# Frojdholm/rayrs

Measured on AMD Instinct MI355X. Metric: Mray/s (primary+secondary) on 1M-tri scene @1024spp, higher is better.
Workload: dtype f64

## Files before the change

### rayrs_amd/_ffi.py

```python
import ctypes as C
import os

_HERE = os.path.dirname(os.path.abspath(__file__))
LIB_PATH = os.environ.get("RAYRS_HIP_LIB") or os.path.join(_HERE, "librayrs_hip.so")

SYMBOLS = [
    "rayrs_strerror", "rayrs_last_error",
    "rayrs_objects_create", "rayrs_objects_destroy", "rayrs_objects_len",
    "rayrs_object_sphere", "rayrs_object_plane", "rayrs_object_triangle",
    "rayrs_object_from_triangles_f32", "rayrs_object_from_triangles_f64",
    "rayrs_object_from_spheres", "rayrs_object_box_geom",
    "rayrs_scene_new", "rayrs_scene_destroy", "rayrs_scene_info", "rayrs_scene_export_bvh",
    "rayrs_scene_export_wide", "rayrs_scene_export_gate_tree", "rayrs_scene_export_hot_tree", "rayrs_scene_clone_to_device", "rayrs_scene_device", "rayrs_scene_set_tuning",
    "rayrs_camera_new",
    "rayrs_frame_sample_chunk", "rayrs_render", "rayrs_render_launch", "rayrs_render_finish", "rayrs_render_multi",
    "rayrs_film_create", "rayrs_film_destroy", "rayrs_film_render", "rayrs_film_read", "rayrs_film_status_get",
    "rayrs_film_state_bytes", "rayrs_film_state_get", "rayrs_film_state_set",
    "rayrs_film_render_adaptive", "rayrs_film_tile_samples",
    "rayrs_render_features", "rayrs_film_features", "rayrs_film_denoise", "rayrs_image_denoise",
    "rayrs_film_noise", "rayrs_film_denoise_guided", "rayrs_image_denoise_guided",
    "rayrs_abi_layout", "rayrs_abi_version",
    "rayrs_io_last_error", "rayrs_buffer_free", "rayrs_ply_load", "rayrs_ply_save", "rayrs_obj_load", "rayrs_obj_load_spheres",
    "rayrs_hdr_load", "rayrs_hdr_save", "rayrs_image_to_bytes", "rayrs_ppm_save", "rayrs_png_save",
]


PRIVATE_SYMBOLS = ["rayrs_test_math", "rayrs_test_rng", "rayrs_test_intersect", "rayrs_test_trace", "rayrs_test_path_trace", "rayrs_test_material", "rayrs_test_background",
                   "rayrs_lab_set", "rayrs_lab_round_ms", "rayrs_lab_multi_rehearse"]


class MaterialDesc(C.Structure):
    _fields_ = [("kind", C.c_int32), ("metallic", C.c_int32), ("color", C.c_double * 3),
                ("spec_color", C.c_double * 3), ("alpha", C.c_double), ("ior", C.c_double),
                ("r0", C.c_double * 3)]


class EmissionDesc(C.Structure):
    _fields_ = [("emissive", C.c_int32), ("pad", C.c_int32), ("strength", C.c_double),
                ("color", C.c_double * 3)]


class CameraDesc(C.Structure):
    _fields_ = [("origin", C.c_double * 3), ("e_x", C.c_double * 3), ("e_y", C.c_double * 3),
                ("z", C.c_double * 3), ("width", C.c_double), ("height", C.c_double),
                ("ppc", C.c_uint32), ("x_pixels", C.c_uint32), ("y_pixels", C.c_uint32)]


class SceneInfo(C.Structure):
    _fields_ = [("n_objects", C.c_uint64), ("n_interior", C.c_uint32), ("n_prims", C.c_uint32),
                ("root_ref", C.c_uint32), ("depth", C.c_uint32), ("compact", C.c_uint32),
                ("n_surfaces", C.c_uint32), ("node_bytes", C.c_uint32), ("prim_bytes", C.c_uint32),
                ("device_bytes", C.c_uint64), ("root_box", C.c_double * 6),
                ("build_seconds", C.c_double), ("n_wide", C.c_uint32), ("wide_root_ref", C.c_uint32),
                ("wide_depth", C.c_uint32), ("local_pool", C.c_uint32), ("gate_n_wide", C.c_uint32),
                ("gate_root_ref", C.c_uint32), ("gate_depth", C.c_uint32),
                ("hot_n_wide", C.c_uint32), ("hot_root_ref", C.c_uint32), ("hot_depth", C.c_uint32),
                ("hot_first", C.c_uint32), ("hot_count", C.c_uint32), ("hot_pad", C.c_uint32),
                ("hot_box", C.c_double * 6)]


class RenderParams(C.Structure):
    _fields_ = [("spp", C.c_uint32), ("max_bounces", C.c_uint32), ("seed", C.c_uint64),
                ("sample_chunk", C.c_uint32), ("tile_rank", C.c_uint32), ("tile_ranks", C.c_uint32),
                ("out_format", C.c_uint32), ("count_work", C.c_uint32), ("fast_traversal", C.c_uint32)]


class RenderStats(C.Structure):
    _fields_ = [("rays", C.c_uint64), ("paths", C.c_uint64), ("nan_pixels", C.c_uint64),
                ("neg_pixels", C.c_uint64), ("interior_visits", C.c_uint64), ("tri_tests", C.c_uint64),
                ("sphere_tests", C.c_uint64), ("plane_tests", C.c_uint64), ("escaped_paths", C.c_uint64),
                ("step_wave", C.c_uint64), ("step_lane", C.c_uint64), ("inner_wave", C.c_uint64),
                ("leaf_wave", C.c_uint64), ("interior_ticks", C.c_uint64), ("leaf_ticks", C.c_uint64),
                ("kernel_ms", C.c_double), ("total_ms", C.c_double), ("kernel_launches", C.c_uint64),
                ("trace_ms", C.c_double), ("refill_ticks", C.c_uint64),
                ("surface_hits", C.c_uint64 * 8), ("direct_rays", C.c_uint64), ("hit_ms", C.c_double), ("miss_ms", C.c_double),
                ("local_pool", C.c_uint32), ("exact_walk", C.c_uint32), ("hot_group", C.c_uint32),
                ("stats_pad", C.c_uint32), ("pre_rays", C.c_uint64), ("pre_root_records", C.c_uint64), ("hot_lane", C.c_uint64),
                ("hot_prim_tests", C.c_uint64), ("hot_tri_divided", C.c_uint64)]

    def as_dict(self):
        d = {n: getattr(self, n) for n, _ in self._fields_}
        d["surface_hits"] = list(self.surface_hits)
        return d


class Tuning(C.Structure):
    _fields_ = [("pool_slots", C.c_uint32), ("local_pool", C.c_uint32)]


class FilmParams(C.Structure):
    _fields_ = [("sample_chunk", C.c_uint32), ("max_bounces", C.c_uint32), ("seed", C.c_uint64),
                ("tile_rank", C.c_uint32), ("tile_ranks", C.c_uint32), ("fast_traversal", C.c_uint32), ("pad", C.c_uint32)]


class FilmStatus(C.Structure):
    _fields_ = [("samples", C.c_uint64), ("full_chunks", C.c_uint64), ("rays", C.c_uint64), ("paths", C.c_uint64),
                ("nan_pixels", C.c_uint64), ("neg_pixels", C.c_uint64), ("unconverged", C.c_uint64),
                ("nonfinite", C.c_uint64), ("closed", C.c_uint32), ("pad", C.c_uint32)]

    def as_dict(self):
        return {n: getattr(self, n) for n, _ in self._fields_ if n != "pad"}


class LabTuning(C.Structure):
    _fields_ = [("refill_min", C.c_uint32), ("leaf_min", C.c_uint32), ("static_pct", C.c_uint32),
                ("stack_lds", C.c_uint32), ("hot_records", C.c_uint32), ("trav_blocks_per_cu", C.c_uint32),
                ("eager_light", C.c_uint32), ("local_reserve", C.c_uint32), ("local_segment_items", C.c_uint32),
                ("force_rccl", C.c_uint32), ("gate_tree", C.c_uint32), ("hot_group", C.c_uint32), ("leaf_wait", C.c_uint32), ("flat_blocks_per_cu", C.c_uint32)]


ABI_VERSION = 7

ABI_STRUCTS = [MaterialDesc, EmissionDesc, CameraDesc, SceneInfo, RenderParams, RenderStats, Tuning, FilmParams, FilmStatus]

_lib = None


def lib():
    global _lib
    if _lib is not None:
        return _lib
    if not os.path.exists(LIB_PATH):
        raise RuntimeError(
            f"{LIB_PATH} is missing: build it with `python -c 'import __graft_entry__ as g; g.build()'` "
            "(make -C rayrs_amd/csrc). There is no CPU fallback.")
    L = C.CDLL(LIB_PATH)
    L.rayrs_abi_version.argtypes = []
    L.rayrs_abi_version.restype = C.c_uint32
    if L.rayrs_abi_version() != ABI_VERSION:
        raise RuntimeError(f"{LIB_PATH} has RAYRS_ABI_VERSION {L.rayrs_abi_version()}, this binding was written against "
                           f"{ABI_VERSION}: rebuild the library (make -C rayrs_amd/csrc)")
    dp = C.POINTER(C.c_double)
    vp = C.c_void_p
    L.rayrs_strerror.restype = C.c_char_p
    L.rayrs_strerror.argtypes = [C.c_int]
    L.rayrs_last_error.restype = C.c_char_p
    L.rayrs_objects_create.argtypes = [C.POINTER(vp)]
    L.rayrs_objects_destroy.argtypes = [vp]
    L.rayrs_objects_destroy.restype = None
    L.rayrs_objects_len.argtypes = [vp]
    L.rayrs_objects_len.restype = C.c_uint64
    mp, ep = C.POINTER(MaterialDesc), C.POINTER(EmissionDesc)
    L.rayrs_object_sphere.argtypes = [vp, C.c_double, dp, mp, ep]
    L.rayrs_object_plane.argtypes = [vp, C.c_int] + [C.c_double] * 5 + [mp, ep]
    L.rayrs_object_triangle.argtypes = [vp, dp, dp, dp, mp, ep]
    L.rayrs_object_from_triangles_f32.argtypes = [vp, vp, C.c_uint32, vp, C.c_uint32, mp, ep]
    L.rayrs_object_from_triangles_f64.argtypes = [vp, vp, C.c_uint32, vp, C.c_uint32, mp, ep]
    L.rayrs_object_from_spheres.argtypes = [vp, C.c_double, vp, C.c_uint32, mp, ep]
    L.rayrs_object_box_geom.argtypes = [vp, dp, dp, mp, ep]
    L.rayrs_scene_new.argtypes = [vp, C.c_double, C.c_double, C.c_int, C.c_uint32, C.c_uint32, C.c_uint32, vp,
                                  C.c_int, C.POINTER(vp)]
    L.rayrs_scene_destroy.argtypes = [vp]
    L.rayrs_scene_destroy.restype = None
    L.rayrs_scene_info.argtypes = [vp, C.POINTER(SceneInfo)]
    L.rayrs_scene_export_bvh.argtypes = [vp, vp, vp, vp]
    L.rayrs_scene_export_wide.argtypes = [vp, vp, vp]
    L.rayrs_scene_export_gate_tree.argtypes = [vp, vp, vp]
    L.rayrs_scene_export_hot_tree.argtypes = [vp, vp, vp]
    L.rayrs_scene_clone_to_device.argtypes = [vp, C.c_int, C.POINTER(vp)]
    L.rayrs_scene_device.argtypes = [vp]
    L.rayrs_scene_set_tuning.argtypes = [vp, C.POINTER(Tuning)]
    L.rayrs_lab_set.argtypes = [vp, C.POINTER(LabTuning)]
    L.rayrs_lab_set.restype = C.c_int
    L.rayrs_lab_multi_rehearse.argtypes = [vp, C.c_uint32, C.c_uint32, C.c_int, C.c_char_p, C.c_uint32]
    L.rayrs_lab_multi_rehearse.restype = C.c_int
    L.rayrs_frame_sample_chunk.argtypes = [C.c_uint32] * 4
    L.rayrs_frame_sample_chunk.restype = C.c_uint32
    L.rayrs_abi_layout.argtypes = [vp, C.c_uint32]
    L.rayrs_abi_layout.restype = C.c_uint32
    L.rayrs_abi_version.argtypes = []
    L.rayrs_abi_version.restype = C.c_uint32
    L.rayrs_render_multi.argtypes = [C.POINTER(vp), C.c_uint32, C.POINTER(CameraDesc), C.POINTER(RenderParams), vp,
                                     C.POINTER(RenderStats)]
    L.rayrs_camera_new.argtypes = [dp, dp, dp, C.c_double, C.c_double, C.c_double, C.c_uint32,
                                   C.POINTER(CameraDesc)]
    L.rayrs_render.argtypes = [vp, C.POINTER(CameraDesc), C.POINTER(RenderParams), vp, C.POINTER(RenderStats)]
    L.rayrs_render_launch.argtypes = [vp, C.POINTER(CameraDesc), C.POINTER(RenderParams), vp, vp]
    L.rayrs_render_finish.argtypes = [vp, C.POINTER(RenderStats)]
    L.rayrs_film_create.argtypes = [vp, C.POINTER(CameraDesc), C.POINTER(FilmParams), C.POINTER(vp)]
    L.rayrs_film_destroy.argtypes = [vp]
    L.rayrs_film_destroy.restype = None
    L.rayrs_film_render.argtypes = [vp, C.c_uint32, C.POINTER(RenderStats)]
    L.rayrs_film_read.argtypes = [vp, C.c_uint32, vp]
    L.rayrs_film_status_get.argtypes = [vp, C.c_double, C.POINTER(FilmStatus)]
    L.rayrs_film_state_bytes.argtypes = [vp]
    L.rayrs_film_state_bytes.restype = C.c_uint64
    L.rayrs_film_state_get.argtypes = [vp, vp, C.c_uint64]
    L.rayrs_film_state_set.argtypes = [vp, vp, C.c_uint64]
    L.rayrs_film_render_adaptive.argtypes = [vp, C.c_uint32, C.c_double, C.c_uint32, C.POINTER(C.c_uint64), C.POINTER(RenderStats)]
    L.rayrs_film_tile_samples.argtypes = [vp, vp, C.c_uint64]
    L.rayrs_film_tile_samples.restype = C.c_uint64
    for name, args in (("rayrs_render_features", [vp, C.POINTER(CameraDesc), C.c_uint32, C.c_uint64, C.c_uint32, C.c_uint32, C.c_uint32,
                                                  vp, vp, vp, vp, vp]),
                       ("rayrs_film_features", [vp, C.c_uint32, vp, vp, vp, vp, vp]),
                       ("rayrs_film_denoise", [vp, C.c_uint32, C.c_uint32] + [C.c_double] * 4 + [C.c_uint32, vp]),
                       ("rayrs_image_denoise", [C.c_int, C.c_uint32, C.c_uint32, vp, vp, vp, vp, C.c_uint32] + [C.c_double] * 4 + [vp]),
                       ("rayrs_film_noise", [vp, vp]),
                       ("rayrs_film_denoise_guided", [vp, C.c_uint32, C.c_uint32] + [C.c_double] * 4 + [C.c_uint32, vp, vp]),
                       ("rayrs_image_denoise_guided", [C.c_int, C.c_uint32, C.c_uint32, vp, vp, vp, vp, vp, C.c_uint32] + [C.c_double] * 4
                        + [vp, vp])):
        if hasattr(L, name) or "RAYRS_HIP_LIB" not in os.environ:
            getattr(L, name).argtypes = args
    L.rayrs_test_math.argtypes = [C.c_int, C.c_int, vp, vp, C.c_uint64, vp]
    L.rayrs_test_rng.argtypes = [C.c_int, C.c_uint64, vp, vp, vp, C.c_uint64, vp]
    L.rayrs_test_intersect.argtypes = [vp, vp, vp, C.c_uint64, C.c_int, vp, vp]
    L.rayrs_test_trace.argtypes = [vp, vp, vp, C.c_uint64, C.c_int, vp, vp, vp]
    L.rayrs_test_path_trace.argtypes = [vp, C.POINTER(CameraDesc), C.c_uint64, C.c_uint32, vp, vp, C.c_uint64, C.c_int, C.c_uint32,
                                        vp, vp, vp, vp, vp, vp]
    L.rayrs_test_material.argtypes = [C.c_int, mp, vp, vp, vp, C.c_uint64, vp, vp, vp, vp]
    L.rayrs_test_background.argtypes = [vp, vp, C.c_uint64, vp]
    L.rayrs_io_last_error.restype = C.c_char_p
    L.rayrs_buffer_free.argtypes = [vp]
    L.rayrs_buffer_free.restype = None
    u32p = C.POINTER(C.c_uint32)
    L.rayrs_ply_load.argtypes = [C.c_char_p, C.POINTER(vp), u32p, C.POINTER(vp), u32p]
    L.rayrs_ply_save.argtypes = [C.c_char_p, vp, C.c_uint32, vp, C.c_uint32, C.c_int]
    L.rayrs_obj_load.argtypes = [C.c_char_p, C.POINTER(vp), u32p, C.POINTER(vp), u32p]
    L.rayrs_obj_load_spheres.argtypes = [C.c_char_p, C.POINTER(vp), u32p]
    L.rayrs_hdr_load.argtypes = [C.c_char_p, C.POINTER(vp), u32p, u32p]
    L.rayrs_hdr_save.argtypes = [C.c_char_p, vp, C.c_uint32, C.c_uint32]
    L.rayrs_image_to_bytes.argtypes = [vp, C.c_uint32, C.c_uint32, C.c_double, vp, C.POINTER(C.c_uint64)]
    L.rayrs_ppm_save.argtypes = [C.c_char_p, vp, C.c_uint32, C.c_uint32]
    L.rayrs_png_save.argtypes = [C.c_char_p, vp, C.c_uint32, C.c_uint32]
    for name in SYMBOLS:
        if not hasattr(L, name) and "RAYRS_HIP_LIB" in os.environ:
            continue
        fn = getattr(L, name)
        if fn.restype is C.c_int and name not in ("rayrs_strerror",):
            fn.restype = C.c_int
    _lib = L
    return L


class RayrsError(RuntimeError):
    def __init__(self, status, where):
        L = lib()
        msg = L.rayrs_strerror(status).decode()
        extra = L.rayrs_last_error().decode() if status != -6 else L.rayrs_io_last_error().decode()
        super().__init__(f"{where}: {msg} ({status})" + (f" [{extra}]" if extra else ""))
        self.status = status


def check(status, where):
    if status != 0:
        raise RayrsError(status, where)
```

### rayrs_amd/api.py

```python
import ctypes as C
from dataclasses import dataclass, field
from typing import List, Optional, Sequence, Tuple

import numpy as np

from . import _ffi

Vec = Tuple[float, float, float]


class Axis:
    X, XRev, Y, YRev, Z, ZRev = range(6)


class BvhHeuristic:
    Midpoint = ("midpoint", 0)

    @staticmethod
    def Sah(splits: int):
        return ("sah", int(splits))


MAT_LAMBERTIAN, MAT_REFLECT, MAT_REFRACT, MAT_GLASS, MAT_COOK_TORRANCE, MAT_COOK_TORRANCE_REFRACT, \
    MAT_COOK_TORRANCE_GLASS, MAT_PLASTIC, MAT_NO_REFLECT = range(9)
# ... 191 lines not shown
        return int(self.desc.x_pixels)

    def y_pixels(self) -> int:
        return int(self.desc.y_pixels)


class Scene:

    def __init__(self, objects, z_near, z_far, heuristic, hdri, device: int = 0):
        L = _ffi.lib()
        self._L = L
        self._h = None
        objs = C.c_void_p()
        _ffi.check(L.rayrs_objects_create(C.byref(objs)), "rayrs_objects_create")
        try:
            for o in flatten_objects(objects):
                m, e = o.mat.desc(), o.emission.desc()
                if o.kind == "sphere":
                    st = L.rayrs_object_sphere(objs, o.radius, _d3(o.origin), C.byref(m), C.byref(e))
                elif o.kind == "plane":
                    st = L.rayrs_object_plane(objs, o.axis, o.umin, o.umax, o.vmin, o.vmax, o.pos, C.byref(m),
                                              C.byref(e))
                elif o.kind == "triangle":
                    st = L.rayrs_object_triangle(objs, _d3(o.p[0]), _d3(o.p[1]), _d3(o.p[2]), C.byref(m),
                                                 C.byref(e))
                elif o.kind == "mesh":
                    fn = (L.rayrs_object_from_triangles_f32 if o.verts.dtype == np.float32
                          else L.rayrs_object_from_triangles_f64)
                    st = fn(objs, o.verts.ctypes.data, o.verts.shape[0], o.idx.ctypes.data, o.idx.shape[0],
                            C.byref(m), C.byref(e))
                else:
                    raise ValueError(f"unknown object kind {o.kind}")
                if st == -1:
                    raise ValueError(f"Object::{o.kind}: invalid argument (a reference assert! would fire)")
                _ffi.check(st, f"rayrs_object_{o.kind}")
            hdri = np.ascontiguousarray(hdri, dtype=np.float32)
            if hdri.ndim != 3 or hdri.shape[2] != 3:
                raise ValueError("hdri must be (H, W, 3)")
            kind, splits = heuristic
            h = C.c_void_p()
            st = L.rayrs_scene_new(objs, float(z_near), float(z_far), 1 if kind == "sah" else 0, int(splits),
                                   hdri.shape[1], hdri.shape[0], hdri.ctypes.data, int(device), C.byref(h))
            if st == -1:
                raise ValueError("Scene::new: invalid argument (lib.rs:234-235, bvh.rs:229)")
            _ffi.check(st, "rayrs_scene_new")
            self._h = h
            self.device = int(device)
        finally:
            L.rayrs_objects_destroy(objs)

    @classmethod
    def _from_handle(cls, L, h, device):
        self = cls.__new__(cls)
        self._L, self._h, self.device = L, h, int(device)
        return self

    def clone_to_device(self, device: int) -> "Scene":
        h = C.c_void_p()
        _ffi.check(self._L.rayrs_scene_clone_to_device(self._h, int(device), C.byref(h)), "rayrs_scene_clone_to_device")
        return Scene._from_handle(self._L, h, device)

    def set_tuning(self, **kw):
        t = _ffi.Tuning()
        for k, v in kw.items():
            if k not in dict(_ffi.Tuning._fields_):
                raise ValueError(f"unknown tuning field {k}")
            setattr(t, k, int(v))
        _ffi.check(self._L.rayrs_scene_set_tuning(self._h, C.byref(t)), "rayrs_scene_set_tuning")

    def lab_set(self, **kw):
        t = _ffi.LabTuning()
        for k, v in kw.items():
            if k not in dict(_ffi.LabTuning._fields_):
                raise ValueError(f"unknown lab field {k}")
            setattr(t, k, int(v))
        _ffi.check(self._L.rayrs_lab_set(self._h, C.byref(t)), "rayrs_lab_set")

    def info(self) -> dict:
        i = _ffi.SceneInfo()
        _ffi.check(self._L.rayrs_scene_info(self._h, C.byref(i)), "rayrs_scene_info")
        d = {n: getattr(i, n) for n, _ in i._fields_ if n not in ("root_box", "hot_box")}
        d["root_box"] = list(i.root_box)
        d["hot_box"] = list(i.hot_box)
        return d

    def export_bvh(self):
        i = self.info()
        box = np.zeros((max(i["n_interior"], 1), 2, 6), dtype=np.float64)
        ref = np.zeros((max(i["n_interior"], 1), 2), dtype=np.uint32)
        prim = np.zeros(max(i["n_prims"], 1), dtype=np.uint32)
        _ffi.check(self._L.rayrs_scene_export_bvh(self._h, box.ctypes.data, ref.ctypes.data, prim.ctypes.data),
                   "rayrs_scene_export_bvh")
        return box[:i["n_interior"]], ref[:i["n_interior"]], prim[:i["n_prims"]]

    def export_wide(self):
        i = self.info()
        box = np.zeros((max(i["n_wide"], 1), 4, 6), dtype=np.float64)
        ref = np.zeros((max(i["n_wide"], 1), 4), dtype=np.uint32)
        _ffi.check(self._L.rayrs_scene_export_wide(self._h, box.ctypes.data, ref.ctypes.data),
                   "rayrs_scene_export_wide")
        return box[:i["n_wide"]], ref[:i["n_wide"]]

    def export_gate_tree(self):
        i = self.info()
        box = np.zeros((max(i["gate_n_wide"], 1), 4, 6), dtype=np.float64)
        ref = np.zeros((max(i["gate_n_wide"], 1), 4), dtype=np.uint32)
        _ffi.check(self._L.rayrs_scene_export_gate_tree(self._h, box.ctypes.data, ref.ctypes.data),
                   "rayrs_scene_export_gate_tree")
        return box[:i["gate_n_wide"]], ref[:i["gate_n_wide"]]

    def export_hot_tree(self):
        i = self.info()
        box = np.zeros((max(i["hot_n_wide"], 1), 4, 6), dtype=np.float64)
        ref = np.zeros((max(i["hot_n_wide"], 1), 4), dtype=np.uint32)
        _ffi.check(self._L.rayrs_scene_export_hot_tree(self._h, box.ctypes.data, ref.ctypes.data),
                   "rayrs_scene_export_hot_tree")
        return box[:i["hot_n_wide"]], ref[:i["hot_n_wide"]]

    def close(self):
        if self._h is not None:
            self._L.rayrs_scene_destroy(self._h)
            self._h = None

    def __del__(self):
        try:
            self.close()
        except Exception:
            pass


def frame_sample_chunk(width: int, height: int, spp: int, requested: int = 4) -> int:
    return int(_ffi.lib().rayrs_frame_sample_chunk(int(width), int(height), int(spp), int(requested)))


def make_params(spp, max_bounces=50, seed=0x5EED, sample_chunk=0, tile_rank=0, tile_ranks=1, out_f64=False,
                count_work=False, exact_traversal=True, fast_traversal=None) -> _ffi.RenderParams:
    p = _ffi.RenderParams()
    p.spp, p.max_bounces, p.seed = int(spp), int(max_bounces), int(seed)
    p.sample_chunk, p.tile_rank, p.tile_ranks = int(sample_chunk), int(tile_rank), int(tile_ranks)
    p.out_format = 1 if out_f64 else 0
    p.count_work = 1 if count_work else 0
    fast = (not exact_traversal) if fast_traversal is None else bool(fast_traversal)
    p.fast_traversal = 1 if fast else 0
    return p


def render(scene: Scene, camera: Camera, spp: int, max_bounces: int = 50, seed: int = 0x5EED, sample_chunk: int = 0,
           tile_rank: int = 0, tile_ranks: int = 1, out_f64: bool = False, count_work: bool = False, out=None,
           exact_traversal: bool = True, fast_traversal=None):
    L = scene._L
    H, W = camera.y_pixels(), camera.x_pixels()
    dt = np.float64 if out_f64 else np.float32
    if out is None:
        out = np.zeros((H, W, 3), dtype=dt)
    assert out.shape == (H, W, 3) and out.dtype == dt and out.flags.c_contiguous
    p = make_params(spp, max_bounces, seed, sample_chunk, tile_rank, tile_ranks, out_f64, count_work, exact_traversal,
                    fast_traversal)
    st = _ffi.RenderStats()
    _ffi.check(L.rayrs_render(scene._h, C.byref(camera.desc), C.byref(p), out.ctypes.data, C.byref(st)),
               "rayrs_render")
    return out, st.as_dict()


def render_multi(scene_list, camera: Camera, spp: int, max_bounces: int = 50, seed: int = 0x5EED,
                 sample_chunk: int = 0, out_f64: bool = False):
    L = scene_list[0]._L
    H, W = camera.y_pixels(), camera.x_pixels()
# ... 268 lines not shown
```

### rayrs_amd/csrc/abi.cpp

```cpp
#include <hip/hip_runtime.h>

#include <cmath>
#include <cstddef>
#include <cstdlib>
#include <cstring>
#include <memory>
#include <new>
#include <stdexcept>
#include <string>
#include <vector>

#include "../../include/rayrs_hip.h"
#include "film.h"
#include "kernels.h"
#include "local_pool.h"
#include "rayrs_lab.h"
#include "scene_host.hpp"
#include "scene_internal.hpp"
#include "wavefront.h"

using namespace rayrs;

namespace {
thread_local std::string g_last_error;
// ... 103 lines not shown
    RAYRS_GUARDED({
    if (!objs) return RAYRS_INVALID_ARG;
    if (!(umin < umax && vmin < vmax)) return RAYRS_INVALID_ARG;
    if (axis < 0 || axis > 5) return RAYRS_INVALID_ARG;
    const int surf = objs->list.add_surface(mat, emission);
    if (surf < 0) return surf;
    Object o;
    std::memset(&o, 0, sizeof(o));
    o.geom.kind = PRIM_PLANE;
    o.geom.axis = (uint32_t)axis;
    o.geom.u0 = umin, o.geom.u1 = umax, o.geom.v0 = vmin, o.geom.v1 = vmax, o.geom.pos = pos;
    o.surface = (uint32_t)surf;
    objs->list.objs.push_back(o);
    return RAYRS_OK;
    })
}

int rayrs_object_triangle(rayrs_objects* objs, const double p1[3], const double p2[3], const double p3[3],
                          const rayrs_material* mat, const rayrs_emission* emission) {
    RAYRS_GUARDED({
    if (!objs || !p1 || !p2 || !p3) return RAYRS_INVALID_ARG;
    const int surf = objs->list.add_surface(mat, emission);
    if (surf < 0) return surf;
    push_triangle(objs->list, {p1[0], p1[1], p1[2]}, {p2[0], p2[1], p2[2]}, {p3[0], p3[1], p3[2]}, (uint32_t)surf);
    return RAYRS_OK;
    })
}

int rayrs_object_from_triangles_f32(rayrs_objects* objs, const float* verts, uint32_t nverts, const uint32_t* idx,
                                    uint32_t ntris, const rayrs_material* mat, const rayrs_emission* emission) {
    RAYRS_GUARDED({
    return from_triangles<float>(objs, verts, nverts, idx, ntris, mat, emission);
    })
}

int rayrs_object_from_triangles_f64(rayrs_objects* objs, const double* verts, uint32_t nverts, const uint32_t* idx,
                                    uint32_t ntris, const rayrs_material* mat, const rayrs_emission* emission) {
    RAYRS_GUARDED({
    return from_triangles<double>(objs, verts, nverts, idx, ntris, mat, emission);
    })
}

int rayrs_object_from_spheres(rayrs_objects* objs, double radius, const double* centers, uint32_t n,
                              const rayrs_material* mat, const rayrs_emission* emission) {
    if (!objs || (!centers && n)) return RAYRS_INVALID_ARG;
    for (uint32_t i = 0; i < n; i++) RAYRS_TRY(rayrs_object_sphere(objs, radius, centers + 3 * (size_t)i, mat, emission));
    return RAYRS_OK;
}

int rayrs_object_box_geom(rayrs_objects* objs, const double ll[3], const double ur[3], const rayrs_material* mat,
                          const rayrs_emission* emission) {
    if (!objs || !ll || !ur) return RAYRS_INVALID_ARG;
    const struct {
        int axis;
        double u0, u1, v0, v1, pos;
    } faces[6] = {
        {RAYRS_AXIS_X, ll[1], ur[1], ll[2], ur[2], ll[0]},    {RAYRS_AXIS_XREV, ll[1], ur[1], ll[2], ur[2], ur[0]},
        {RAYRS_AXIS_ZREV, ll[0], ur[0], ll[1], ur[1], ll[2]}, {RAYRS_AXIS_Z, ll[0], ur[0], ll[1], ur[1], ur[2]},
        {RAYRS_AXIS_YREV, ll[0], ur[0], ll[2], ur[2], ll[1]}, {RAYRS_AXIS_Y, ll[0], ur[0], ll[2], ur[2], ll[1]},
    };
    for (const auto& f : faces) RAYRS_TRY(rayrs_object_plane(objs, f.axis, f.u0, f.u1, f.v0, f.v1, f.pos, mat, emission));
    return RAYRS_OK;
}


void rayrs_scene_destroy(rayrs_scene* scene) { delete scene; }

static int scene_configure_traversal(rayrs_scene* s) {
    const FlatScene& f = s->flat;
    for (int x = 0; x < 3; x++) {
        if (x == 2 && !f.has_hot) continue;
        const WalkTree& t = s->tree(x);
        rayrs_scene::Walk& w = s->trav[x];
        const uint32_t depth = t.depth ? t.depth : 1;
        w.leafq = x == 0 ? 0u : TRAV_LEAFQ;
        uint32_t want = s->lab.stack_lds ? s->lab.stack_lds : (w.leafq ? TRAV_STACK_LDS_DEFER : TRAV_STACK_LDS);
        w.stack_lds = want < depth ? want : depth;
        const uint32_t rec_bytes = f.compact ? (uint32_t)sizeof(Node4F32) + 16u : (uint32_t)sizeof(Node4F64) + 16u;
        uint32_t hot = (w.leafq ? TRAV_HOT_BYTES_DEFER : TRAV_HOT_BYTES) / rec_bytes;
        if (s->lab.hot_records == 0xffffffffu) hot = 0;
        else if (s->lab.hot_records) hot = s->lab.hot_records < WIDE_FRONT ? s->lab.hot_records : WIDE_FRONT;
        w.hot_records = hot < t.n() ? hot : t.n();
        const uint32_t lds = wf_trav_lds_bytes(f.compact, w.stack_lds, w.leafq, w.hot_records);
        HIP_TRY(wf_trav_raise_lds(f.compact, lds));
        HIP_TRY(wf_trav_occupancy(f.compact, lds, &w.blocks_per_cu));
        if (w.blocks_per_cu < 1) w.blocks_per_cu = 1;
    }
    return RAYRS_OK;
}

constexpr uint32_t LOCAL_SEGMENT_ITEMS = 1u << 27;
constexpr uint32_t LOCAL_MAX_SEGMENTS = 64;
static void scene_configure_local(rayrs_scene* s) {
    const FlatScene& f = s->flat;
    LocalScene& ls = s->local;
    std::memset(&ls, 0, sizeof(ls));
    s->local_ok = false;
    const WalkTree& t = f.gate;
    if (t.n() > 1 || f.n_prims() == 0 || f.n_prims() > LP_MAX_PRIMS || s->surfaces.size() > LP_MAX_PRIMS) return;
    auto add_gate = [&](const double* box, uint32_t ref) {
        if ((ref >> 30) != REF_RANGE) return false;
        const uint32_t g = ls.n_gates++;
        for (int i = 0; i < 6; i++) ls.box[g][i] = box[i];
        ls.first[g] = (ref & 0x3fffffffu) >> 2;
        ls.count[g] = (ref & 3u) + 1u;
        return true;
    };
    if (t.n() == 0) {
        if (!add_gate(f.root_box, t.root_ref)) return;
    } else {
        if ((t.root_ref >> 30) != REF_INTERIOR) return;
        for (uint32_t k = 0; k < 4; k++) {
            const uint32_t ref = t.ref[k];
            if ((ref >> 30) == REF_NONE) continue;
            if (!add_gate(&t.box[(size_t)k * 6], ref)) return;
        }
    }
    uint32_t covered = 0;
    for (uint32_t g = 0; g < ls.n_gates; g++) covered += ls.count[g];
    if (covered != f.n_prims()) return;
    ls.n_records = t.n();
    ls.n_prims = f.n_prims();
    for (const SurfaceDev& sf : s->surfaces) ls.kind_mask |= 1u << (uint32_t)sf.kind;
    s->local_ok = true;
}

extern "C++" int rayrs::scene_upload(rayrs_scene* s) {
    HIP_TRY(hipSetDevice(s->device));
    hipDeviceProp_t prop;
    HIP_TRY(hipGetDeviceProperties(&prop, s->device));
    s->cu_count = prop.multiProcessorCount;
    const FlatScene& f = s->flat;
    for (int x = 0; x < 3; x++) {
        const WalkTree& t = s->tree(x);
        if (x == 2 && !f.has_hot) continue;
        HIP_TRY(s->trav[x].d_nodes.upload(t.node_bytes.data(), t.node_bytes.size()));
    }
    if (f.has_hot) HIP_TRY(s->d_hot.upload(&f.hot, sizeof(HotGroupDev)));
    HIP_TRY(s->d_prims.upload(f.prim_bytes.data(), f.prim_bytes.size()));
    HIP_TRY(s->d_surfaces.upload(s->surfaces.data(), s->surfaces.size() * sizeof(SurfaceDev)));
    HIP_TRY(s->d_hdri.upload(f.hdri_quads.data(), f.hdri_quads.size() * sizeof(float)));
    HIP_TRY(s->d_counters.reserve(sizeof(Counters)));
    for (auto& e : s->ev) HIP_TRY(e.create());
    s->device_bytes = f.walk.node_bytes.size() + f.gate.node_bytes.size() + (f.has_hot ? f.gate_hot.node_bytes.size() : 0) + f.prim_bytes.size() + s->surfaces.size() * sizeof(SurfaceDev) +
                      f.hdri_quads.size() * sizeof(float);
    RAYRS_TRY(scene_configure_traversal(s));
    HIP_TRY(s->pool.d_ctl.reserve(sizeof(WfCtl)));
    HIP_TRY(s->pool.h_live.alloc(2 * sizeof(uint32_t)));
    for (auto& e : s->pool.ev_batch) HIP_TRY(e.create());
    HIP_TRY(s->d_next_item.reserve(sizeof(unsigned long long)));
    if (s->local_ok) {
        HIP_TRY(lp_configure());
        HIP_TRY(lp_occupancy(s->flat.compact, s->local.n_prims, (uint32_t)s->surfaces.size(), &s->local_blocks_per_cu));
        if (s->local_blocks_per_cu < 1) s->local_blocks_per_cu = 1;
        if (s->local_blocks_per_cu > (int)LP_WPS) s->local_blocks_per_cu = (int)LP_WPS;
        HIP_TRY(s->d_local_items.reserve(LOCAL_MAX_SEGMENTS * sizeof(unsigned long long)));
    }
    return RAYRS_OK;
}

int rayrs_scene_new(const rayrs_objects* objs, double z_near, double z_far, int heuristic, uint32_t splits,
                    uint32_t hdri_w, uint32_t hdri_h, const float* hdri_rgb, int device, rayrs_scene** out) {
    RAYRS_GUARDED({
    if (!objs || !out) return RAYRS_INVALID_ARG;
    *out = nullptr;
    std::unique_ptr<rayrs_scene> s(new rayrs_scene());
    RAYRS_TRY(build_flat_scene(objs->list, z_near, z_far, heuristic, splits, hdri_w, hdri_h, hdri_rgb, &s->flat));
    if (std::max(s->flat.walk.depth, s->flat.gate.depth) > 4096u) {
        g_last_error = "walk tree needs " + std::to_string(std::max(s->flat.walk.depth, s->flat.gate.depth)) + " stack entries (limit 4096)";
        return RAYRS_UNSUPPORTED;
    }
    s->surfaces = objs->list.surfaces;
    s->n_objects = objs->list.objs.size();
    s->device = device;
    scene_configure_local(s.get());
    if (device >= 0) RAYRS_TRY(scene_upload(s.get()));
    *out = s.release();
    return RAYRS_OK;
    })
}

int rayrs_scene_info(const rayrs_scene* scene, rayrs_scene_info_t* info) {
    if (!scene || !info) return RAYRS_INVALID_ARG;
    const FlatScene& f = scene->flat;
    std::memset(info, 0, sizeof(*info));
    info->n_objects = scene->n_objects;
    info->n_interior = f.n_interior();
    info->n_prims = f.n_prims();
    info->root_ref = f.root_ref;
    info->depth = f.depth;
    info->compact = f.compact ? 1u : 0u;
    info->n_surfaces = (uint32_t)scene->surfaces.size();
    info->node_bytes = f.compact ? (uint32_t)sizeof(Node4F32) : (uint32_t)sizeof(Node4F64);
    info->n_wide = f.walk.n();
    info->wide_root_ref = f.walk.root_ref;
    info->wide_depth = f.walk.depth;
    info->gate_n_wide = f.gate.n();
    info->gate_root_ref = f.gate.root_ref;
    info->gate_depth = f.gate.depth;
    if (f.has_hot) {
        info->hot_n_wide = f.gate_hot.n();
        info->hot_root_ref = f.gate_hot.root_ref;
        info->hot_depth = f.gate_hot.depth;
        info->hot_first = f.hot.first;
        info->hot_count = f.hot.count;
        for (int i = 0; i < 6; i++) info->hot_box[i] = f.hot.box[i];
    }
    info->local_pool = (scene->local_ok && scene->tuning.local_pool != 1u) ? 1u : 0u;
    info->prim_bytes = 4u * (f.compact ? PRIM_DWORDS_COMPACT : PRIM_DWORDS_FULL);
    info->device_bytes = scene->device_bytes;
    for (int i = 0; i < 6; i++) info->root_box[i] = f.root_box[i];
    info->build_seconds = f.build_seconds;
    return RAYRS_OK;
}

int rayrs_scene_export_bvh(const rayrs_scene* scene, double* child_box, uint32_t* child_ref, uint32_t* prim_object) {
    if (!scene) return RAYRS_INVALID_ARG;
    const FlatScene& f = scene->flat;
    if (child_box && !f.child_box.empty()) std::memcpy(child_box, f.child_box.data(), f.child_box.size() * 8);
    if (child_ref && !f.child_ref.empty()) std::memcpy(child_ref, f.child_ref.data(), f.child_ref.size() * 4);
    if (prim_object && !f.prim_object.empty())
        std::memcpy(prim_object, f.prim_object.data(), f.prim_object.size() * 4);
    return RAYRS_OK;
}

static int export_tree(const WalkTree& t, double* wide_box, uint32_t* wide_ref) {
    if (wide_box && !t.box.empty()) std::memcpy(wide_box, t.box.data(), t.box.size() * 8);
    if (wide_ref && !t.ref.empty()) std::memcpy(wide_ref, t.ref.data(), t.ref.size() * 4);
// ... 12 lines not shown
    return scene && scene->flat.has_hot ? export_tree(scene->flat.gate_hot, wide_box, wide_ref) : RAYRS_INVALID_ARG;
}

int rayrs_scene_clone_to_device(const rayrs_scene* scene, int device, rayrs_scene** out) {
    RAYRS_GUARDED({
        if (!scene || !out || device < 0) return RAYRS_INVALID_ARG;
        *out = nullptr;
        std::unique_ptr<rayrs_scene> s(new rayrs_scene());
        s->flat = scene->flat;
        s->surfaces = scene->surfaces;
        s->n_objects = scene->n_objects;
        s->tuning = scene->tuning;
        s->lab = scene->lab;
        s->device = device;
        scene_configure_local(s.get());
        RAYRS_TRY(scene_upload(s.get()));
        *out = s.release();
        return RAYRS_OK;
    })
}

int rayrs_scene_device(const rayrs_scene* scene) { return scene ? scene->device : -1; }

static int scene_quiesce(rayrs_scene* scene) {
    return scene->device >= 0 ? scene_settle(scene) : RAYRS_OK;
}

rayrs_scene::~rayrs_scene() {
    if (device < 0) return;
    (void)hipSetDevice(device);
    if (pending && last_stream) (void)hipStreamSynchronize(last_stream);
}

int rayrs_scene_set_tuning(rayrs_scene* scene, const rayrs_tuning* tuning) {
    if (!scene || !tuning) return RAYRS_INVALID_ARG;
    if (tuning->local_pool > 1u) return RAYRS_INVALID_ARG;
    RAYRS_TRY(scene_quiesce(scene));
    scene->tuning = *tuning;
    return RAYRS_OK;
}

#ifdef RAYRS_LAB_TICKS
extern "C" int rayrs_lab_ticks(rayrs_scene* scene, uint64_t out[16]) {
    if (!scene || !out || scene->device < 0) return RAYRS_INVALID_ARG;
    HIP_TRY(hipSetDevice(scene->device));
    Counters c;
    HIP_TRY(scene->d_counters.download(&c, sizeof(c)));
    for (int i = 0; i < 16; i++) out[i] = c.lab_ticks[i];
    return RAYRS_OK;
}
#endif

static int round_event(rayrs_scene::Pool& pl, uint32_t r, uint32_t k, hipStream_t stream) {
    while (pl.ev_round.size() < 4 * (size_t)(r + 1)) {
        Event e;
        HIP_TRY(e.create());
        pl.ev_round.push_back(std::move(e));
    }
    HIP_TRY(hipEventRecord(pl.ev_round[4 * (size_t)r + k], stream));
    return RAYRS_OK;
}

static int round_ms(const rayrs_scene* scene, uint32_t r, float ms[3]) {
    const Event* e = &scene->pool.ev_round[4 * (size_t)r];
    ms[1] = ms[2] = 0.f;
    HIP_TRY(hipEventElapsedTime(&ms[0], e[0], e[1]));
    if (scene->last_local) return RAYRS_OK;
    HIP_TRY(hipEventElapsedTime(&ms[1], e[1], e[2]));
    HIP_TRY(hipEventElapsedTime(&ms[2], e[2], e[3]));
    return RAYRS_OK;
}

extern "C" int rayrs_lab_round_ms(rayrs_scene* scene, float* out, uint32_t cap_rounds) {
    if (!scene || scene->device < 0 || scene->pending) return RAYRS_INVALID_ARG;
    HIP_TRY(hipSetDevice(scene->device));
    for (uint32_t r = 0; r < scene->pool.timed_rounds && r < cap_rounds && out; r++) RAYRS_TRY(round_ms(scene, r, out + 3 * r));
    return (int)scene->pool.timed_rounds;
}

int rayrs_lab_set(rayrs_scene* scene, const rayrs_lab_tuning* lab) {
    if (!scene || !lab) return RAYRS_INVALID_ARG;
    if (lab->stack_lds > 64u) return RAYRS_INVALID_ARG;
    if (lab->hot_group != 0u && lab->hot_group != 0xffffffffu) return RAYRS_INVALID_ARG;
    if (lab->static_pct > 100u || lab->refill_min > 64u || lab->leaf_min > 64u || lab->leaf_wait > 64u || lab->flat_blocks_per_cu > 64u || lab->eager_light > 1u || lab->force_rccl > 1u || lab->gate_tree > 1u)
        return RAYRS_INVALID_ARG;
    if (lab->local_reserve != 0u && (lab->local_reserve < 8u || lab->local_reserve > 4096u)) return RAYRS_INVALID_ARG;
    if (lab->local_segment_items != 0u && lab->local_segment_items < 65536u) return RAYRS_INVALID_ARG;
    RAYRS_TRY(scene_quiesce(scene));
    scene->lab = *lab;
    if (scene->device >= 0) return scene_configure_traversal(scene);
    return RAYRS_OK;
}

uint32_t rayrs_frame_sample_chunk(uint32_t x_pixels, uint32_t y_pixels, uint32_t spp, uint32_t requested) {
    if (spp == 0) return 0;
    uint64_t chunk = requested ? requested : 4u;
    const uint64_t pixels = (uint64_t)((x_pixels + 7u) / 8u) * ((y_pixels + 7u) / 8u) * 64u;
    while (chunk < spp && pixels * ((spp + chunk - 1) / chunk) > (1ull << 30)) chunk *= 2;
    return chunk >= spp ? 0u : (uint32_t)chunk;
}

uint32_t rayrs_abi_version(void) { return RAYRS_ABI_VERSION; }

uint32_t rayrs_abi_layout(uint32_t* out, uint32_t cap) {
    std::vector<uint32_t> t;
    t.push_back(RAYRS_ABI_VERSION);
#define RAYRS_STRUCT(T, N) t.push_back((uint32_t)sizeof(T)), t.push_back(N)
#define RAYRS_FIELD(T, F) t.push_back((uint32_t)offsetof(T, F))
    RAYRS_STRUCT(rayrs_material, 7);
    RAYRS_FIELD(rayrs_material, kind), RAYRS_FIELD(rayrs_material, metallic), RAYRS_FIELD(rayrs_material, color);
    RAYRS_FIELD(rayrs_material, spec_color), RAYRS_FIELD(rayrs_material, alpha), RAYRS_FIELD(rayrs_material, ior);
    RAYRS_FIELD(rayrs_material, r0);
    RAYRS_STRUCT(rayrs_emission, 4);
    RAYRS_FIELD(rayrs_emission, emissive), RAYRS_FIELD(rayrs_emission, pad), RAYRS_FIELD(rayrs_emission, strength);
    RAYRS_FIELD(rayrs_emission, color);
    RAYRS_STRUCT(rayrs_camera, 9);
    RAYRS_FIELD(rayrs_camera, origin), RAYRS_FIELD(rayrs_camera, e_x), RAYRS_FIELD(rayrs_camera, e_y);
    RAYRS_FIELD(rayrs_camera, z), RAYRS_FIELD(rayrs_camera, width), RAYRS_FIELD(rayrs_camera, height);
    RAYRS_FIELD(rayrs_camera, ppc), RAYRS_FIELD(rayrs_camera, x_pixels), RAYRS_FIELD(rayrs_camera, y_pixels);
    RAYRS_STRUCT(rayrs_scene_info_t, 26);
    RAYRS_FIELD(rayrs_scene_info_t, n_objects), RAYRS_FIELD(rayrs_scene_info_t, n_interior);
    RAYRS_FIELD(rayrs_scene_info_t, n_prims), RAYRS_FIELD(rayrs_scene_info_t, root_ref);
    RAYRS_FIELD(rayrs_scene_info_t, depth), RAYRS_FIELD(rayrs_scene_info_t, compact);
    RAYRS_FIELD(rayrs_scene_info_t, n_surfaces), RAYRS_FIELD(rayrs_scene_info_t, node_bytes);
    RAYRS_FIELD(rayrs_scene_info_t, prim_bytes), RAYRS_FIELD(rayrs_scene_info_t, device_bytes);
    RAYRS_FIELD(rayrs_scene_info_t, root_box), RAYRS_FIELD(rayrs_scene_info_t, build_seconds);
    RAYRS_FIELD(rayrs_scene_info_t, n_wide), RAYRS_FIELD(rayrs_scene_info_t, wide_root_ref);
    RAYRS_FIELD(rayrs_scene_info_t, wide_depth), RAYRS_FIELD(rayrs_scene_info_t, local_pool);
    RAYRS_FIELD(rayrs_scene_info_t, gate_n_wide), RAYRS_FIELD(rayrs_scene_info_t, gate_root_ref);
    RAYRS_FIELD(rayrs_scene_info_t, gate_depth);
    RAYRS_FIELD(rayrs_scene_info_t, hot_n_wide), RAYRS_FIELD(rayrs_scene_info_t, hot_root_ref);
    RAYRS_FIELD(rayrs_scene_info_t, hot_depth), RAYRS_FIELD(rayrs_scene_info_t, hot_first);
    RAYRS_FIELD(rayrs_scene_info_t, hot_count), RAYRS_FIELD(rayrs_scene_info_t, hot_pad);
    RAYRS_FIELD(rayrs_scene_info_t, hot_box);
    RAYRS_STRUCT(rayrs_render_params, 9);
    RAYRS_FIELD(rayrs_render_params, spp), RAYRS_FIELD(rayrs_render_params, max_bounces);
    RAYRS_FIELD(rayrs_render_params, seed), RAYRS_FIELD(rayrs_render_params, sample_chunk);
    RAYRS_FIELD(rayrs_render_params, tile_rank), RAYRS_FIELD(rayrs_render_params, tile_ranks);
    RAYRS_FIELD(rayrs_render_params, out_format), RAYRS_FIELD(rayrs_render_params, count_work);
    RAYRS_FIELD(rayrs_render_params, fast_traversal);
    RAYRS_STRUCT(rayrs_render_stats, 33);
    RAYRS_FIELD(rayrs_render_stats, rays), RAYRS_FIELD(rayrs_render_stats, paths);
    RAYRS_FIELD(rayrs_render_stats, nan_pixels), RAYRS_FIELD(rayrs_render_stats, neg_pixels);
    RAYRS_FIELD(rayrs_render_stats, interior_visits), RAYRS_FIELD(rayrs_render_stats, tri_tests);
    RAYRS_FIELD(rayrs_render_stats, sphere_tests), RAYRS_FIELD(rayrs_render_stats, plane_tests);
    RAYRS_FIELD(rayrs_render_stats, escaped_paths), RAYRS_FIELD(rayrs_render_stats, step_wave);
    RAYRS_FIELD(rayrs_render_stats, step_lane), RAYRS_FIELD(rayrs_render_stats, inner_wave);
    RAYRS_FIELD(rayrs_render_stats, leaf_wave), RAYRS_FIELD(rayrs_render_stats, interior_ticks);
    RAYRS_FIELD(rayrs_render_stats, leaf_ticks), RAYRS_FIELD(rayrs_render_stats, kernel_ms);
    RAYRS_FIELD(rayrs_render_stats, total_ms), RAYRS_FIELD(rayrs_render_stats, kernel_launches);
    RAYRS_FIELD(rayrs_render_stats, trace_ms), RAYRS_FIELD(rayrs_render_stats, refill_ticks);
    RAYRS_FIELD(rayrs_render_stats, surface_hits), RAYRS_FIELD(rayrs_render_stats, direct_rays);
    RAYRS_FIELD(rayrs_render_stats, hit_ms), RAYRS_FIELD(rayrs_render_stats, miss_ms);
    RAYRS_FIELD(rayrs_render_stats, local_pool), RAYRS_FIELD(rayrs_render_stats, exact_walk);
    RAYRS_FIELD(rayrs_render_stats, hot_group), RAYRS_FIELD(rayrs_render_stats, stats_pad);
    RAYRS_FIELD(rayrs_render_stats, pre_rays), RAYRS_FIELD(rayrs_render_stats, pre_root_records);
    RAYRS_FIELD(rayrs_render_stats, hot_lane);
    RAYRS_FIELD(rayrs_render_stats, hot_prim_tests), RAYRS_FIELD(rayrs_render_stats, hot_tri_divided);
    RAYRS_STRUCT(rayrs_tuning, 2);
    RAYRS_FIELD(rayrs_tuning, pool_slots), RAYRS_FIELD(rayrs_tuning, local_pool);
    RAYRS_STRUCT(rayrs_film_params, 7);
    RAYRS_FIELD(rayrs_film_params, sample_chunk), RAYRS_FIELD(rayrs_film_params, max_bounces);
    RAYRS_FIELD(rayrs_film_params, seed), RAYRS_FIELD(rayrs_film_params, tile_rank);
    RAYRS_FIELD(rayrs_film_params, tile_ranks), RAYRS_FIELD(rayrs_film_params, fast_traversal);
    RAYRS_FIELD(rayrs_film_params, pad);
    RAYRS_STRUCT(rayrs_film_status, 10);
    RAYRS_FIELD(rayrs_film_status, samples), RAYRS_FIELD(rayrs_film_status, full_chunks);
    RAYRS_FIELD(rayrs_film_status, rays), RAYRS_FIELD(rayrs_film_status, paths);
    RAYRS_FIELD(rayrs_film_status, nan_pixels), RAYRS_FIELD(rayrs_film_status, neg_pixels);
    RAYRS_FIELD(rayrs_film_status, unconverged), RAYRS_FIELD(rayrs_film_status, nonfinite);
    RAYRS_FIELD(rayrs_film_status, closed), RAYRS_FIELD(rayrs_film_status, pad);
#undef RAYRS_STRUCT
#undef RAYRS_FIELD
    for (uint32_t i = 0; i < cap && i < t.size(); i++) out[i] = t[i];
    return (uint32_t)t.size();
}


int rayrs_camera_new(const double origin[3], const double up[3], const double lookat[3], double fov, double width,
                     double height, uint32_t ppi, rayrs_camera* out) {
    return camera_new(origin, up, lookat, fov, width, height, ppi, out);
}


extern "C++" SceneDev rayrs::make_scene_dev(const rayrs_scene* s, bool exact) {
    SceneDev sc;
    std::memset(&sc, 0, sizeof(sc));
    const int which = s->walk_index(exact);
    const WalkTree& t = s->tree(which);
    const rayrs_scene::Walk& w = s->trav[which];
    sc.hot = which == 2 ? s->d_hot.as<HotGroupDev>() : nullptr;
    sc.nodes = w.d_nodes.as<>();
    sc.prims = s->d_prims.as<>();
    sc.surfaces = s->d_surfaces.as<SurfaceDev>();
    sc.hdri = s->d_hdri.as<float>();
    sc.hdri_w = s->flat.hdri_w;
    sc.hdri_h = s->flat.hdri_h;
    sc.hdri_wm1 = (double)(s->flat.hdri_w - 1u);
    sc.hdri_hm1 = (double)(s->flat.hdri_h - 1u);
    sc.root_ref = t.root_ref;
    sc.stack_depth = t.depth ? t.depth : 1;
    sc.stack_lds = w.stack_lds;
    sc.hot_records = w.hot_records;
    sc.leafq = w.leafq;
    sc.n_surfaces = (uint32_t)s->surfaces.size();
    for (int i = 0; i < 6; i++) sc.root_box[i] = s->flat.root_box[i];
    sc.t0 = s->flat.t0;
    sc.t1 = s->flat.t1;
    sc.exact = exact ? 1u : 0u;
    return sc;
}

constexpr double RAYRS_FAR_DIAGONALS = 8.0;
constexpr double RAYRS_FAR_PRIMITIVES = 4096.0;
extern "C++" bool rayrs::camera_is_far(const rayrs_scene* s, const rayrs_camera* c) {
    const double* b = s->flat.root_box;
    double d2 = 0.0, e2 = 0.0;
    for (int a = 0; a < 3; a++) {
        const double lo = b[2 * a], hi = b[2 * a + 1], o = c->origin[a];
        const double out = o < lo ? lo - o : (o > hi ? o - hi : 0.0);
        d2 += out * out;
        e2 += (hi - lo) * (hi - lo);
    }
    const double small = s->flat.small_extent;
    return d2 > RAYRS_FAR_DIAGONALS * RAYRS_FAR_DIAGONALS * e2 || (small > 0.0 && d2 > RAYRS_FAR_PRIMITIVES * RAYRS_FAR_PRIMITIVES * small * small);
}

extern "C++" CameraDev rayrs::make_camera_dev(const rayrs_camera* c) {
    CameraDev cam;
    std::memset(&cam, 0, sizeof(cam));
    for (int i = 0; i < 3; i++) {
        cam.origin[i] = c->origin[i];
        cam.e_x[i] = c->e_x[i];
        cam.e_y[i] = c->e_y[i];
        cam.z[i] = c->z[i];
    }
    cam.width = c->width;
    cam.height = c->height;
    cam.ppc = (double)c->ppc;
    cam.W = c->x_pixels;
    cam.H = c->y_pixels;
    return cam;
}

extern "C++" uint32_t rayrs::trav_settings(const rayrs_scene* s, bool exact, uint32_t np, RenderDev& rp) {
    const rayrs_lab_tuning& lab = s->lab;
    rp.refill_min = lab.refill_min ? lab.refill_min : 52u;
    rp.leaf_min = lab.leaf_min ? lab.leaf_min : (exact ? 48u : lab.gate_tree ? 32u : 24u);
    rp.leaf_wait = lab.leaf_wait ? lab.leaf_wait : 16u;
    uint32_t trav_bpc = (uint32_t)s->trav[s->walk_index(exact)].blocks_per_cu;
    if (lab.trav_blocks_per_cu && lab.trav_blocks_per_cu < trav_bpc) trav_bpc = lab.trav_blocks_per_cu;
    const uint32_t blocks = (uint32_t)s->cu_count * trav_bpc;
    const uint32_t static_pct = lab.static_pct ? lab.static_pct : 50u;
    const uint64_t n_waves = (uint64_t)blocks * 4u;
    rp.static_windows = (uint32_t)((uint64_t)(np / wf_window_slots()) * static_pct / 100u / n_waves * n_waves);
    return blocks;
}

extern "C++" WfDev rayrs::pool_wf(const DevBuf& block, uint32_t np, const DevBuf& ctl, uint32_t trav_blocks, const DevBuf& spill) {
    WfDev wf;
    std::memset(&wf, 0, sizeof(wf));
    wf.slots = block.as<PathSlot>();
    wf.light = reinterpret_cast<double*>(wf.slots + np);
    wf.state = reinterpret_cast<uint8_t*>(wf.light + (size_t)np * 4u);
    wf.ctl = ctl.as<WfCtl>();
    wf.np = np;
    wf.trav_threads = trav_blocks * 256u;
    wf.stack_spill = spill.as<uint32_t>();
    return wf;
}

struct FramePlan {
    SceneDev sc;
    CameraDev cam;
    RenderDev rp;
    bool exact, eager_light, use_local;
    uint64_t partial_need;
    uint64_t tile_items, seg_tiles, seg_items;
    uint32_t local_blocks;
    uint64_t live_total;
    uint32_t np, trav_blocks, flat_blocks;
    size_t spill_words;
    bool is_film;
    FilmPassDev film;
};

static RenderDev make_render_dev(const rayrs_scene* scene, const rayrs_camera* camera, const rayrs_render_params* params, uint32_t sample0,
                                 const FilmPassDev* film, void* out_device) {
    RenderDev rp;
    std::memset(&rp, 0, sizeof(rp));
    rp.spp = params->spp;
    rp.sample0 = sample0;
    rp.max_bounces = params->max_bounces;
    rp.seed = params->seed;
    rp.chunk = (params->sample_chunk == 0 || params->sample_chunk >= params->spp) ? params->spp : params->sample_chunk;
// ... 36 lines not shown
    p.local_blocks = (uint32_t)scene->cu_count * (uint32_t)scene->local_blocks_per_cu;
    const uint64_t most_items = rp.total_items < p.seg_items ? rp.total_items : p.seg_items;
    const uint64_t want_blocks = (most_items + 4u * LP_PATHS_PER_WAVE - 1) / (4u * LP_PATHS_PER_WAVE);
    if (want_blocks < p.local_blocks) p.local_blocks = (uint32_t)(want_blocks ? want_blocks : 1);
    if (!p.use_local || rp.total_items == 0) p.local_blocks = 0;

    p.exact = params->fast_traversal == 0u || camera_is_far(scene, camera);
    p.sc = make_scene_dev(scene, p.exact);
    p.cam = make_camera_dev(camera);

    constexpr uint64_t POOL_MAX_SLOTS = 1ull << 28;
    uint64_t np64 = rp.total_items;
    if (np64 > POOL_MAX_SLOTS) np64 = POOL_MAX_SLOTS;
    {
        const uint64_t samples = rp.n_local_tiles * 64ull * rp.spp;
        const uint64_t by_work = samples / 12u > (1ull << 20) ? samples / 12u : (1ull << 20);
        if (np64 > by_work) np64 = by_work;
    }
    if (scene->tuning.pool_slots) np64 = scene->tuning.pool_slots;
    if (np64 > rp.total_items) np64 = rp.total_items;
    p.live_total = np64;
    const bool streaming = !p.use_local && rp.total_items > 0;
    p.np = streaming ? (uint32_t)((p.live_total + 1023ull) & ~1023ull) : 0u;
    p.trav_blocks = trav_settings(scene, p.exact, p.np, rp);
    p.spill_words = streaming ? (size_t)(p.sc.stack_depth - p.sc.stack_lds) * p.trav_blocks * 256u : 0;

    p.eager_light = lab.eager_light != 0u;
    for (const SurfaceDev& sf : scene->surfaces)
        if (sf.emit[0] != 0.0 || sf.emit[1] != 0.0 || sf.emit[2] != 0.0) p.eager_light = true;

    const uint32_t n_windows = p.np / wf_window_slots();
    p.flat_blocks = (n_windows + 3u) / 4u;
    uint32_t per_cu = lab.flat_blocks_per_cu;
    if (!per_cu) {
        per_cu = n_windows / (36u * (uint32_t)scene->cu_count);
        per_cu = per_cu < FLAT_BLOCKS_PER_CU_MIN ? FLAT_BLOCKS_PER_CU_MIN : per_cu > FLAT_BLOCKS_PER_CU_MAX ? FLAT_BLOCKS_PER_CU_MAX : per_cu;
    }
    const uint32_t flat_cap = (uint32_t)scene->cu_count * per_cu;
    if (p.flat_blocks > flat_cap) p.flat_blocks = flat_cap;
    return RAYRS_OK;
}

static int enqueue_local(rayrs_scene* scene, const FramePlan& p, hipStream_t stream) {
    rayrs_scene::Pool& pl = scene->pool;
    const RenderDev& rp = p.rp;
    const uint64_t n_seg = (rp.total_items + p.seg_items - 1) / p.seg_items;
    for (uint64_t seg = 0; seg < n_seg; seg++) {
        LocalDev lp;
        lp.light = scene->d_local_light.as<double>();
        lp.next_item = scene->d_local_items.as<unsigned long long>() + seg;
        lp.item_base = seg * p.seg_items;
        lp.item_count = rp.total_items - lp.item_base < p.seg_items ? rp.total_items - lp.item_base : p.seg_items;
        RenderDev rseg = rp;
        rseg.partial_item0 = lp.item_base;
        const uint64_t share = lp.item_count / ((uint64_t)p.local_blocks * 4u * 16u);
        lp.reserve = (uint32_t)(share < 8u ? 8u : share > 256u ? 256u : share);
        if (scene->lab.local_reserve) lp.reserve = scene->lab.local_reserve;
        lp.pad = 0;
        RAYRS_TRY(round_event(pl, (uint32_t)seg, 0, stream));
        HIP_TRY(lp_launch(scene->flat.compact, rp.count_work != 0u, p.sc, scene->local, p.cam, rseg, lp, p.local_blocks, stream));
        RAYRS_TRY(round_event(pl, (uint32_t)seg, 1, stream));
        const uint32_t seg_lt0 = (uint32_t)(seg * p.seg_tiles), seg_n_lt = (uint32_t)(lp.item_count / p.tile_items);
        HIP_TRY(p.is_film ? launch_film_accumulate(p.cam, rseg, p.film, seg_lt0, seg_n_lt, stream) : launch_resolve(p.cam, rseg, seg_lt0, seg_n_lt, stream));
        pl.timed_rounds = (uint32_t)seg + 1;
    }
    scene->rounds = (uint32_t)n_seg;
    return RAYRS_OK;
}

static int enqueue_streaming(rayrs_scene* scene, const FramePlan& p, const WfDev& wf, hipStream_t stream) {
    rayrs_scene::Pool& pl = scene->pool;
    const RenderDev& rp = p.rp;
    uint32_t* h_live = pl.h_live.as<uint32_t>();
    HIP_TRY(wf_launch_init(wf, (uint32_t)p.live_total, stream));
    HIP_TRY(wf_launch_gen(scene->flat.compact, p.sc, p.cam, rp, wf, p.flat_blocks, stream));
    h_live[0] = h_live[1] = (uint32_t)p.live_total;
    constexpr uint32_t MAX_TIMED = 8192;
    uint32_t it = 0;
    uint32_t batch = 16;
    for (uint32_t b = 0;; b++) {
        for (uint32_t k = 0; k < batch; k++, it++) {
            const bool timed = it < MAX_TIMED;
            if (timed) RAYRS_TRY(round_event(pl, it, 0, stream));
            HIP_TRY(wf_launch_trav(scene->flat.compact, rp.count_work != 0u, p.sc, rp, wf, p.trav_blocks, stream));
            if (timed) RAYRS_TRY(round_event(pl, it, 1, stream));
            HIP_TRY(wf_launch_hit(scene->flat.compact, p.eager_light, p.sc, p.cam, rp, wf, p.flat_blocks, stream));
            if (timed) RAYRS_TRY(round_event(pl, it, 2, stream));
            HIP_TRY(wf_launch_miss(scene->flat.compact, p.eager_light, p.sc, p.cam, rp, wf, p.flat_blocks, stream));
            if (timed) {
                RAYRS_TRY(round_event(pl, it, 3, stream));
                pl.timed_rounds = it + 1;
            }
        }
        HIP_TRY(hipMemcpyAsync(&h_live[b & 1u], &wf.ctl->live_slots, sizeof(uint32_t), hipMemcpyDeviceToHost, stream));
        HIP_TRY(hipEventRecord(pl.ev_batch[b & 1u], stream));
        if (b > 0) {
            HIP_TRY(hipEventSynchronize(pl.ev_batch[(b - 1u) & 1u]));
            const uint64_t seen = h_live[(b - 1u) & 1u];
            if (seen == 0u) break;
            batch = seen * 8u < p.live_total ? 4u : 16u;
        }
        if (it > (1u << 26)) {
            g_last_error = "path rounds did not terminate";
            return RAYRS_HIP_ERROR;
        }
    }
    scene->rounds = it;
    return RAYRS_OK;
}

extern "C++" int rayrs::render_enqueue(rayrs_scene* scene, const rayrs_camera* camera, const rayrs_render_params* params, uint32_t sample0,
                                       const FilmPassDev* film, void* out_device, void* hip_stream) {
    RAYRS_GUARDED({
    if (!scene || !camera || !params || (!out_device && !film)) return RAYRS_INVALID_ARG;
    if (scene->device < 0) return RAYRS_NO_DEVICE;
    if (params->spp == 0 || camera->x_pixels == 0 || camera->y_pixels == 0) return RAYRS_INVALID_ARG;
    if (camera->x_pixels > 65535u || camera->y_pixels > 65535u) return RAYRS_UNSUPPORTED;
    if (params->max_bounces > 8000u) return RAYRS_UNSUPPORTED;
    if (params->spp > SLOT_SAMPLE_MASK || sample0 > SLOT_SAMPLE_MASK - params->spp) return RAYRS_UNSUPPORTED;
    if (params->tile_ranks == 0 || params->tile_rank >= params->tile_ranks) return RAYRS_INVALID_ARG;
    if (params->out_format != RAYRS_OUT_F32 && params->out_format != RAYRS_OUT_F64) return RAYRS_INVALID_ARG;
    if (params->fast_traversal > 1u) return RAYRS_INVALID_ARG;
    HIP_TRY(hipSetDevice(scene->device));
    hipStream_t stream = reinterpret_cast<hipStream_t>(hip_stream);
    if (scene->pending) {
        HIP_TRY(hipStreamSynchronize(scene->last_stream));
        scene->pending = false;
    }

    FramePlan p;
    RAYRS_TRY(plan_frame(scene, camera, params, sample0, film, out_device, p));
    p.is_film = film != nullptr;
    p.film = film ? *film : FilmPassDev{};
    scene->last_exact = p.exact;

    rayrs_scene::Pool& pl = scene->pool;
    HIP_TRY(scene->d_partial.reserve((size_t)p.partial_need * 3 * sizeof(double)));
    p.rp.partial = scene->d_partial.as<double>();
    HIP_TRY(scene->d_local_light.reserve((size_t)p.local_blocks * 4u * LP_PATHS_PER_WAVE * 4 * sizeof(double)));
    HIP_TRY(pl.block.reserve((size_t)p.np * POOL_SLOT_BYTES));
    HIP_TRY(pl.d_wave_items.reserve((size_t)p.flat_blocks * 4u * 2 * sizeof(unsigned long long)));
    HIP_TRY(pl.d_stack_spill.reserve(p.spill_words * sizeof(uint32_t)));
    WfDev wf = pool_wf(pl.block, p.np, pl.d_ctl, p.trav_blocks, pl.d_stack_spill);
    wf.n_flat_waves = p.flat_blocks * 4u;
    wf.wave_items = pl.d_wave_items.as<unsigned long long>();

    pl.timed_rounds = 0;
    HIP_TRY(hipMemsetAsync(p.rp.counters, 0, sizeof(Counters), stream));
    HIP_TRY(hipMemsetAsync(p.rp.next_item, 0, sizeof(unsigned long long), stream));
    if (p.use_local) HIP_TRY(hipMemsetAsync(scene->d_local_items.as<>(), 0, LOCAL_MAX_SEGMENTS * sizeof(unsigned long long), stream));
    HIP_TRY(hipEventRecord(scene->ev[0], stream));
    scene->rounds = 0;
    scene->last_local = p.use_local;
    if (p.rp.total_items > 0) RAYRS_TRY(p.use_local ? enqueue_local(scene, p, stream) : enqueue_streaming(scene, p, wf, stream));
    HIP_TRY(hipEventRecord(scene->ev[1], stream));
    if (!p.use_local) HIP_TRY(p.is_film ? launch_film_accumulate(p.cam, p.rp, p.film, 0u, p.rp.n_local_tiles, stream) : launch_resolve(p.cam, p.rp, 0u, p.rp.n_local_tiles, stream));
    HIP_TRY(hipEventRecord(scene->ev[2], stream));
    scene->last_stream = stream;
    scene->pending = true;
    return RAYRS_OK;
    })
}

int rayrs_render_launch(rayrs_scene* scene, const rayrs_camera* camera, const rayrs_render_params* params,
                        void* out_device, void* hip_stream) {
    if (!out_device) return RAYRS_INVALID_ARG;
    return render_enqueue(scene, camera, params, 0u, nullptr, out_device, hip_stream);
// ... 71 lines not shown
```

### rayrs_amd/csrc/rayrs_lab.h

```cpp
#ifndef RAYRS_LAB_H
#define RAYRS_LAB_H

#include <stdint.h>

#include "../../include/rayrs_hip.h"

#ifdef __cplusplus
extern "C" {
#endif

typedef struct {
    uint32_t refill_min;
    uint32_t leaf_min;
    uint32_t static_pct;
    uint32_t stack_lds;
    uint32_t hot_records;
    uint32_t trav_blocks_per_cu;
    uint32_t eager_light;
    uint32_t local_reserve;
    uint32_t local_segment_items;
    uint32_t force_rccl;
    uint32_t gate_tree;
    uint32_t hot_group;
    uint32_t leaf_wait;
    uint32_t flat_blocks_per_cu;
} rayrs_lab_tuning;

int rayrs_lab_set(rayrs_scene* scene, const rayrs_lab_tuning* lab);

int rayrs_lab_round_ms(rayrs_scene* scene, float* out, uint32_t cap_rounds);

int rayrs_lab_multi_rehearse(const int* rank_devices, uint32_t n, uint32_t rounds, int fail_reduce_at, char* log, uint32_t cap);

#ifdef __cplusplus
}
#endif
#endif
```

### rayrs_amd/csrc/rayrs_selftest.h

```cpp
#ifndef RAYRS_SELFTEST_H
#define RAYRS_SELFTEST_H

#include <stdint.h>

#include "../../include/rayrs_hip.h"

#ifdef __cplusplus
extern "C" {
#endif

int rayrs_test_math(int device, int fn, const double* x, const double* y, uint64_t n, double* out);
int rayrs_test_rng(int device, uint64_t seed, const uint64_t* pixel, const uint64_t* sample, const uint32_t* draw,
                   uint64_t n, uint64_t* out_bits);
int rayrs_test_intersect(rayrs_scene* scene, const double* o, const double* d, uint64_t n, int exact, double* t,
                         int64_t* object);
int rayrs_test_trace(rayrs_scene* scene, const double* o, const double* d, uint64_t n, int exact, double* t, int64_t* object,
                     uint64_t* pre_answered);
int rayrs_test_path_trace(rayrs_scene* scene, const rayrs_camera* camera, uint64_t seed, uint32_t max_bounces,
                          const uint32_t* pixel, const uint32_t* sample, uint64_t n, int exact, uint32_t cap,
                          uint32_t* n_queries, int64_t* object, double* t, double* throughput, uint32_t* draw, double* rgb);
int rayrs_test_material(int device, const rayrs_material* mat, const double* normal, const double* view,
                        const uint64_t* key, uint64_t n, int32_t* scattered, double* color, double* dir,
                        uint32_t* draws);
int rayrs_test_background(rayrs_scene* scene, const double* dir, uint64_t n, double* rgb);

#ifdef __cplusplus
}
#endif
#endif
```

### rayrs_amd/csrc/scene_host.cpp

```cpp
#include "scene_host.hpp"

#include <algorithm>
#include <chrono>
#include <cmath>
#include <cstddef>
#include <cstdlib>
#include <cstring>
#include <limits>

#include "../../include/rayrs_numeric.h"

namespace rayrs {


static bool in01(const double* c) {
    return c[0] >= 0.0 && c[0] <= 1.0 && c[1] >= 0.0 && c[1] <= 1.0 && c[2] >= 0.0 && c[2] <= 1.0;
}

int ObjectList::add_surface(const rayrs_material* m, const rayrs_emission* e) {
    if (!m) return RAYRS_INVALID_ARG;
    SurfaceDev s;
    std::memset(&s, 0, sizeof(s));
    s.kind = m->kind;
    if (m->kind < 0 || m->kind > RAYRS_MAT_NO_REFLECT) return RAYRS_INVALID_ARG;
    if (m->kind != RAYRS_MAT_NO_REFLECT) {
        if (!in01(m->color)) return RAYRS_INVALID_ARG;
        for (int i = 0; i < 3; i++) s.color[i] = m->color[i];
        const bool needs_ior = m->kind == RAYRS_MAT_REFRACT || m->kind == RAYRS_MAT_GLASS ||
                               m->kind == RAYRS_MAT_COOK_TORRANCE_REFRACT ||
                               m->kind == RAYRS_MAT_COOK_TORRANCE_GLASS || m->kind == RAYRS_MAT_PLASTIC;
        if (needs_ior && !(m->ior > 0.0 && std::isfinite(m->ior))) return RAYRS_INVALID_ARG;
        s.ior = m->ior;
        if (m->kind >= RAYRS_MAT_COOK_TORRANCE && m->kind <= RAYRS_MAT_PLASTIC) {
            if (!(m->alpha > 0.0 && std::isfinite(m->alpha))) return RAYRS_INVALID_ARG;
            s.ct_alpha2 = m->alpha * m->alpha;
            for (int i = 0; i < 3; i++) s.ct_color[i] = m->color[i];
            if (m->kind == RAYRS_MAT_COOK_TORRANCE) {
                s.metallic = m->metallic ? 1 : 0;
                if (s.metallic) {
                    for (int i = 0; i < 3; i++) s.ct_r0[i] = m->r0[i];
                } else {
                    s.ct_ior = m->ior;
                }
            } else {
                s.metallic = 0;
                s.ct_ior = m->ior;
                if (m->kind == RAYRS_MAT_PLASTIC) {
                    if (!in01(m->spec_color)) return RAYRS_INVALID_ARG;
                    for (int i = 0; i < 3; i++) s.ct_color[i] = m->spec_color[i];
                }
            }
        }
    }
    if (e && e->emissive) {
        if (!(e->strength >= 0.0) || !in01(e->color)) return RAYRS_INVALID_ARG;
        s.emissive = 1;
        for (int i = 0; i < 3; i++) s.emit[i] = e->strength * e->color[i];
    }
    for (size_t i = 0; i < surfaces.size(); i++)
        if (std::memcmp(&surfaces[i], &s, sizeof(s)) == 0) return (int)i;
    surfaces.push_back(s);
    return (int)surfaces.size() - 1;
}


Aabb shape_bbox(const Shape& s) {
    Aabb b;
    if (s.kind == PRIM_SPHERE) {
        const double radius = rr_sqrt(s.radius2);
        b.xmin = s.origin.x - radius;
        b.xmax = s.origin.x + radius;
        b.ymin = s.origin.y - radius;
        b.ymax = s.origin.y + radius;
        b.zmin = s.origin.z - radius;
        b.zmax = s.origin.z + radius;
    } else if (s.kind == PRIM_PLANE) {
        if (s.axis == RAYRS_AXIS_X || s.axis == RAYRS_AXIS_XREV) {
            b = {s.pos, s.pos, s.u0, s.u1, s.v0, s.v1};
        } else if (s.axis == RAYRS_AXIS_Y || s.axis == RAYRS_AXIS_YREV) {
            b = {s.u0, s.u1, s.pos, s.pos, s.v0, s.v1};
        } else {
            b = {s.u0, s.u1, s.v0, s.v1, s.pos, s.pos};
        }
    } else {
        b.xmin = rr_min(s.p1.x, rr_min(s.p2.x, s.p3.x));
        b.ymin = rr_min(s.p1.y, rr_min(s.p2.y, s.p3.y));
        b.zmin = rr_min(s.p1.z, rr_min(s.p2.z, s.p3.z));
        b.xmax = rr_max(s.p1.x, rr_max(s.p2.x, s.p3.x));
        b.ymax = rr_max(s.p1.y, rr_max(s.p2.y, s.p3.y));
        b.zmax = rr_max(s.p1.z, rr_max(s.p2.z, s.p3.z));
    }
    return b;
}
// ... 436 lines not shown
void tight_box(const Aabb& b, const double* gate, double* out) {
    const double pb[6] = {b.xmin, b.xmax, b.ymin, b.ymax, b.zmin, b.zmax};
    double ext = 0.0;
    for (int a = 0; a < 3; a++) ext = std::max(ext, pb[2 * a + 1] - pb[2 * a]);
    const double m = ext * LEAF_MARGIN;
    for (int a = 0; a < 3; a++) {
        double lo = pb[2 * a] - m, hi = pb[2 * a + 1] + m;
        float lf = (float)lo, hf = (float)hi;
        if ((double)lf > lo) lf = std::nextafterf(lf, -std::numeric_limits<float>::infinity());
        if ((double)hf < hi) hf = std::nextafterf(hf, std::numeric_limits<float>::infinity());
        lo = (double)lf, hi = (double)hf;
        out[2 * a] = lo > gate[2 * a] ? lo : gate[2 * a];
        out[2 * a + 1] = hi < gate[2 * a + 1] ? hi : gate[2 * a + 1];
    }
}

void split_groups(const std::vector<WalkGroup>& groups, const std::vector<Aabb>& prim_box, std::vector<WalkGroup>& out) {
    out.reserve(groups.size() * 3);
    for (const WalkGroup& g : groups) {
        const uint32_t first = (g.ref & 0x3fffffffu) >> 2, count = (g.ref & 3u) + 1u;
        for (uint32_t i = 0; i < count; i++) {
            WalkGroup r;
            tight_box(prim_box[first + i], g.box, r.box);
            r.ref = (REF_RANGE << 30) | ((first + i) << 2);
            out.push_back(r);
        }
    }
}

void build_tree_over(const std::vector<WalkGroup>& leaves, WalkTree& t) {
    WalkBuilder b(leaves);
    b.build();
    t.box.reserve(leaves.size() * 12);
    t.ref.reserve(leaves.size() * 2);
    const WideCollapse wc(b.nodes);
    t.root_ref = emit_wide(t, wc, 0, &t.depth);
    front_largest(t);
}

constexpr double HOT_MIN_AREA = 0.25;
constexpr size_t HOT_MIN_GROUPS = 8;

void pick_hot_group(FlatScene& f, const std::vector<WalkGroup>& groups) {
    f.has_hot = false;
    f.gate_hot = WalkTree();
    std::memset(&f.hot, 0, sizeof(f.hot));
    if (groups.size() < HOT_MIN_GROUPS) return;
    size_t best = 0;
    double best_area = -1.0;
    for (size_t i = 0; i < groups.size(); i++) {
        const double a = box_area(groups[i].box);
        if (a > best_area) best_area = a, best = i;
    }
    const double root_area = box_area(f.root_box);
    if (!(best_area >= HOT_MIN_AREA * root_area) || !std::isfinite(best_area)) return;
    std::vector<WalkGroup> rest;
    rest.reserve(groups.size() - 1);
    for (size_t i = 0; i < groups.size(); i++)
        if (i != best) rest.push_back(groups[i]);
    build_tree_over(rest, f.gate_hot);
    const WalkGroup& g = groups[best];
    for (int k = 0; k < 6; k++) f.hot.box[k] = g.box[k];
    f.hot.first = (g.ref & 0x3fffffffu) >> 2;
    f.hot.count = (g.ref & 3u) + 1u;
    f.has_hot = true;
}

void build_walk_trees(FlatScene& f, const std::vector<Aabb>& prim_box) {
    f.walk = WalkTree();
    f.gate = WalkTree();
    if ((f.root_ref >> 30) != REF_INTERIOR) {
        f.walk.root_ref = f.gate.root_ref = f.root_ref;
        return;
    }
    std::vector<WalkGroup> groups;
    collect_groups(f, f.root_ref & 0x3fffffffu, f.root_box, groups);
    build_tree_over(groups, f.gate);
    pick_hot_group(f, groups);
    std::vector<WalkGroup> singles;
    split_groups(groups, prim_box, singles);
    build_tree_over(singles, f.walk);
}

inline bool boxes_f32_exact(const WalkTree& t) {
    for (size_t r = 0; r < t.ref.size(); r++) {
        if ((t.ref[r] >> 30) == REF_NONE) continue;
        for (int k = 0; k < 6; k++)
            if (!f32_exact(t.box[r * 6 + k])) return false;
    }
    return true;
}

template <typename NODE, typename F>
void fill_nodes(WalkTree& t) {
    const uint32_t n = t.n();
    const double inf = std::numeric_limits<double>::infinity();
    t.node_bytes.assign((size_t)std::max(n, 1u) * sizeof(NODE), 0);
    NODE* nodes = reinterpret_cast<NODE*>(t.node_bytes.data());
    for (uint32_t r = 0; r < n; r++)
        for (int ch = 0; ch < 4; ch++) {
            const uint32_t ref = t.ref[(size_t)r * 4 + ch];
            nodes[r].ref[ch] = ref;
            for (int k = 0; k < 6; k++)
                nodes[r].box[ch][k] = (ref >> 30) == REF_NONE ? ((k & 1) ? (F)-inf : (F)inf) : (F)t.box[((size_t)r * 4 + ch) * 6 + k];
        }
}

void put_f64(uint32_t* dst, double v) { std::memcpy(dst, &v, 8); }
void put_f32(uint32_t* dst, float v) { std::memcpy(dst, &v, 4); }

}

int build_flat_scene(const ObjectList& objs, double z_near, double z_far, int heuristic, uint32_t splits,
                     uint32_t hdri_w, uint32_t hdri_h, const float* hdri_rgb, FlatScene* out) {
    if (!(z_near >= 0.0) || !(z_far > z_near)) return RAYRS_INVALID_ARG;
    if (objs.objs.empty()) return RAYRS_INVALID_ARG;
    if (heuristic != RAYRS_BVH_MIDPOINT && heuristic != RAYRS_BVH_SAH) return RAYRS_INVALID_ARG;
    if (heuristic == RAYRS_BVH_SAH && splits < 2) return RAYRS_INVALID_ARG;
    if (hdri_w < 2 || hdri_h < 2 || !hdri_rgb) return RAYRS_INVALID_ARG;
    if (objs.objs.size() >= (1u << 28)) return RAYRS_UNSUPPORTED;

    const auto t_begin = std::chrono::steady_clock::now();
    FlatScene& f = *out;
    f = FlatScene();
    f.t0 = z_near;
    f.t1 = z_far;

    Builder b(objs, f, heuristic == RAYRS_BVH_SAH, splits);
    Aabb root;
    const size_t n = objs.objs.size();
    if (n == 1) {
        root = b.boxes[0];
        f.prim_object[0] = 0;
        b.next_prim = 1;
        f.root_ref = (REF_RANGE << 30) | 0u;
    } else {
        f.root_ref = b.build(0, n, 0, &root);
    }
    f.root_box[0] = root.xmin, f.root_box[1] = root.xmax, f.root_box[2] = root.ymin;
    f.root_box[3] = root.ymax, f.root_box[4] = root.zmin, f.root_box[5] = root.zmax;

    {
        std::vector<Aabb> prim_box(n);
        for (size_t p = 0; p < n; p++) prim_box[p] = b.boxes[f.prim_object[p]];
        build_walk_trees(f, prim_box);
        std::vector<double> ext(n);
        for (size_t p = 0; p < n; p++) {
            const Aabb& pb = prim_box[p];
            const double e = std::max(pb.xmax - pb.xmin, std::max(pb.ymax - pb.ymin, pb.zmax - pb.zmin));
            ext[p] = e > 0.0 ? e : std::numeric_limits<double>::infinity();
        }
        std::nth_element(ext.begin(), ext.begin() + (std::ptrdiff_t)(n / 20), ext.end());
        f.small_extent = std::isfinite(ext[n / 20]) ? ext[n / 20] : 0.0;
    }

    bool compact = boxes_f32_exact(f.gate) && boxes_f32_exact(f.walk) && boxes_f32_exact(f.gate_hot);
    for (size_t i = 0; i < n && compact; i++) {
        const Shape& s = objs.objs[i].geom;
        if (s.kind != PRIM_TRIANGLE) continue;
        const double v[9] = {s.p1.x, s.p1.y, s.p1.z, s.p2.x, s.p2.y, s.p2.z, s.p3.x, s.p3.y, s.p3.z};
        for (double c : v)
            if (!f32_exact(c)) {
                compact = false;
                break;
            }
    }
    f.compact = compact;
    for (WalkTree* t : {&f.gate, &f.walk, &f.gate_hot}) {
        if (compact) fill_nodes<Node4F32, float>(*t);
        else fill_nodes<Node4F64, double>(*t);
    }

    const uint32_t dw = compact ? PRIM_DWORDS_COMPACT : PRIM_DWORDS_FULL;
    f.prim_bytes.assign((size_t)n * dw * 4, 0);
    uint32_t* prims = reinterpret_cast<uint32_t*>(f.prim_bytes.data());
    for (size_t p = 0; p < n; p++) {
        const Object& o = objs.objs[f.prim_object[p]];
        const Shape& s = o.geom;
        uint32_t* rec = prims + p * dw;
        if (s.kind == PRIM_SPHERE) {
            put_f64(rec + 0, s.radius2);
            put_f64(rec + 2, s.origin.x);
            put_f64(rec + 4, s.origin.y);
            put_f64(rec + 6, s.origin.z);
        } else if (s.kind == PRIM_PLANE) {
            put_f64(rec + 0, s.u0);
            put_f64(rec + 2, s.u1);
            put_f64(rec + 4, s.v0);
            put_f64(rec + 6, s.v1);
            put_f64(rec + 8, s.pos);
        } else {
            const double v[9] = {s.p1.x, s.p1.y, s.p1.z, s.p2.x, s.p2.y, s.p2.z, s.p3.x, s.p3.y, s.p3.z};
            for (int k = 0; k < 9; k++) {
                if (compact)
                    put_f32(rec + k, (float)v[k]);
                else
                    put_f64(rec + 2 * k, v[k]);
            }
        }
        rec[dw - 1] = s.kind | (s.axis << 2) | (o.surface << 8);
    }

    if (f.has_hot) {
        for (uint32_t k = 0; k < f.hot.count; k++) {
            const Object& o = objs.objs[f.prim_object[f.hot.first + k]];
            const Shape& s = o.geom;
            HotPrim& hp = f.hot.prim[k];
            if (s.kind == PRIM_SPHERE) {
                hp.v[0] = s.radius2, hp.v[1] = s.origin.x, hp.v[2] = s.origin.y, hp.v[3] = s.origin.z;
            } else if (s.kind == PRIM_PLANE) {
                hp.v[0] = s.u0, hp.v[1] = s.u1, hp.v[2] = s.v0, hp.v[3] = s.v1, hp.v[4] = s.pos;
            } else {
                hp.v[0] = s.p1.x, hp.v[1] = s.p1.y, hp.v[2] = s.p1.z;
                hp.v[3] = s.p2.x - s.p1.x, hp.v[4] = s.p2.y - s.p1.y, hp.v[5] = s.p2.z - s.p1.z;
                hp.v[6] = s.p3.x - s.p1.x, hp.v[7] = s.p3.y - s.p1.y, hp.v[8] = s.p3.z - s.p1.z;
            }
            hp.tag = s.kind | (s.axis << 2) | (o.surface << 8);
            if (s.kind == PRIM_SPHERE) f.hot.n_sphere++;
            else if (s.kind == PRIM_PLANE) f.hot.n_plane++;
            else f.hot.n_tri++;
        }
        const WalkTree& t = f.gate_hot;
        const uint32_t r = t.root_ref & 0x3fffffffu;
        const double inf = std::numeric_limits<double>::infinity();
        for (int ch = 0; ch < 4; ch++) {
            const uint32_t ref = t.ref[(size_t)r * 4 + ch];
            f.hot.root_ref[ch] = ref;
            for (int k = 0; k < 6; k++)
                f.hot.root_box[ch][k] = (ref >> 30) == REF_NONE ? ((k & 1) ? -inf : inf) : t.box[((size_t)r * 4 + ch) * 6 + k];
        }
    }

    f.hdri_w = hdri_w;
    f.hdri_h = hdri_h;
    {
        std::vector<float> rgb((size_t)hdri_w * hdri_h * 3);
        for (size_t t = 0; t < rgb.size(); t++) {
            const double v = rr_max(rr_min((double)hdri_rgb[t], 3.0), 0.0);
            rgb[t] = (float)v;
        }
        f.hdri_quads.assign((size_t)hdri_w * hdri_h * 16, 0.f);
        for (uint32_t i = 0; i < hdri_h; i++) {
            const uint32_t i1 = i + 1 < hdri_h ? i + 1 : hdri_h - 1;
            for (uint32_t j = 0; j < hdri_w; j++) {
                const uint32_t j1 = j + 1 < hdri_w ? j + 1 : hdri_w - 1;
                const size_t src[4] = {(size_t)i * hdri_w + j, (size_t)i1 * hdri_w + j, (size_t)i * hdri_w + j1,
                                       (size_t)i1 * hdri_w + j1};
                float* q = &f.hdri_quads[((size_t)i * hdri_w + j) * 16];
                for (int k = 0; k < 4; k++)
                    for (int c = 0; c < 3; c++) q[k * 4 + c] = rgb[src[k] * 3 + c];
            }
        }
    }

    f.build_seconds = std::chrono::duration<double>(std::chrono::steady_clock::now() - t_begin).count();
    return RAYRS_OK;
}


static inline Vec3 sub(Vec3 a, Vec3 b) { return {a.x - b.x, a.y - b.y, a.z - b.z}; }
static inline Vec3 cross(Vec3 a, Vec3 b) {
    return {a.y * b.z - a.z * b.y, a.z * b.x - a.x * b.z, a.x * b.y - a.y * b.x};
}
static inline Vec3 unit(Vec3 a) {
    const double inv = 1.0 / rr_sqrt(a.x * a.x + a.y * a.y + a.z * a.z);
    return {a.x * inv, a.y * inv, a.z * inv};
}

int camera_new(const double origin[3], const double up[3], const double lookat[3], double fov, double width,
               double height, uint32_t ppi, rayrs_camera* out) {
    if (!origin || !up || !lookat || !out) return RAYRS_INVALID_ARG;
    if (!(fov > 0. && fov < 180.)) return RAYRS_INVALID_ARG;
    if (!(width > 0.) || !(height > 0.)) return RAYRS_INVALID_ARG;
    const Vec3 o{origin[0], origin[1], origin[2]}, u{up[0], up[1], up[2]}, la{lookat[0], lookat[1], lookat[2]};
    if (o.x == la.x && o.y == la.y && o.z == la.z) return RAYRS_INVALID_ARG;
    const uint32_t ppc = (uint32_t)std::round((double)ppi * 2.54);
    const Vec3 z = unit(sub(la, o));
    const Vec3 x = unit(cross(u, z));
    const Vec3 y = unit(cross(z, x));
    const double rad = fov * (RR_PI / 180.0);
    const double focal = width / rr_tan(rad / 2.);
    out->origin[0] = o.x, out->origin[1] = o.y, out->origin[2] = o.z;
    out->e_x[0] = x.x, out->e_x[1] = x.y, out->e_x[2] = x.z;
    out->e_y[0] = y.x, out->e_y[1] = y.y, out->e_y[2] = y.z;
    out->z[0] = focal * z.x, out->z[1] = focal * z.y, out->z[2] = focal * z.z;
    out->width = width;
    out->height = height;
    out->ppc = ppc;
    out->x_pixels = (uint32_t)std::round(width * (double)ppc);
    out->y_pixels = (uint32_t)std::round(height * (double)ppc);
    return RAYRS_OK;
}

}
```

### rayrs_amd/csrc/scene_host.hpp

```cpp
#pragma once
#include <cstdint>
#include <string>
#include <vector>

#include "../../include/rayrs_hip.h"
#include "layout.h"

namespace rayrs {

struct Vec3 {
    double x, y, z;
};

struct Aabb {
    double xmin, xmax, ymin, ymax, zmin, zmax;
};

struct Shape {
    uint32_t kind;
    uint32_t axis;
    double radius2;
    Vec3 origin;
    double u0, u1, v0, v1, pos;
    Vec3 p1, p2, p3;
};

struct Object {
    Shape geom;
    uint32_t surface;
};

struct ObjectList {
    std::vector<Object> objs;
    std::vector<SurfaceDev> surfaces;

    int add_surface(const rayrs_material* m, const rayrs_emission* e);
};

Aabb shape_bbox(const Shape& s);

struct WalkTree {
    std::vector<double> box;
    std::vector<uint32_t> ref;
    uint32_t root_ref = 0;
    uint32_t depth = 0;
    std::vector<uint8_t> node_bytes;
    uint32_t n() const { return (uint32_t)(ref.size() / 4); }
};

struct FlatScene {
    std::vector<double> child_box;
    std::vector<uint32_t> child_ref;
    std::vector<uint32_t> prim_object;
    uint32_t root_ref = 0;
    uint32_t depth = 0;
    WalkTree walk, gate, gate_hot;
    bool has_hot = false;
    HotGroupDev hot = {};
    double root_box[6] = {0, 0, 0, 0, 0, 0};
    bool compact = false;
    std::vector<uint8_t> prim_bytes;
    std::vector<float> hdri_quads;
    uint32_t hdri_w = 0, hdri_h = 0;
    double t0 = 0, t1 = 0;
    double build_seconds = 0;
    double small_extent = 0;
    uint32_t n_interior() const { return (uint32_t)(child_ref.size() / 2); }
    uint32_t n_prims() const { return (uint32_t)prim_object.size(); }
};

int build_flat_scene(const ObjectList& objs, double z_near, double z_far, int heuristic, uint32_t splits,
                     uint32_t hdri_w, uint32_t hdri_h, const float* hdri_rgb, FlatScene* out);

int camera_new(const double origin[3], const double up[3], const double lookat[3], double fov, double width,
               double height, uint32_t ppi, rayrs_camera* out);

}
```

### rayrs_amd/csrc/scene_internal.hpp

```cpp
#pragma once
#include <hip/hip_runtime.h>

#include <cstdint>
#include <string>
#include <vector>

#include "../../include/rayrs_hip.h"
#include "device_mem.hpp"
#include "film.h"
#include "local_pool.h"
#include "rayrs_lab.h"
#include "scene_host.hpp"
#include "wavefront.h"

struct rayrs_objects {
    rayrs::ObjectList list;
};

struct rayrs_scene {
    rayrs::FlatScene flat;
    std::vector<rayrs::SurfaceDev> surfaces;
    uint64_t n_objects = 0;
    int device = -1;
    ~rayrs_scene();
    rayrs::DevBuf d_prims, d_surfaces, d_hdri, d_counters;
    rayrs::DevBuf d_partial;
    rayrs::Event ev[3];
    hipStream_t last_stream = nullptr;
    bool pending = false;
    int cu_count = 0;
    struct Walk {
        rayrs::DevBuf d_nodes;
        int blocks_per_cu = 0;
        uint32_t stack_lds = 1;
        uint32_t hot_records = 0;
        uint32_t leafq = 0;
    };
    Walk trav[3];
    const rayrs::WalkTree& tree(int which) const { return which == 2 ? flat.gate_hot : which == 1 ? flat.gate : flat.walk; }
    rayrs::DevBuf d_hot;
    int walk_index(bool exact) const {
        if (!exact) return lab.gate_tree ? 1 : 0;
        return (flat.has_hot && lab.hot_group != 0xffffffffu) ? 2 : 1;
    }
    uint64_t device_bytes = 0;
    struct Pool {
        rayrs::DevBuf block;
        rayrs::DevBuf d_ctl;
        rayrs::DevBuf d_wave_items;
        rayrs::DevBuf d_stack_spill;
        rayrs::PinnedBuf h_live;
        rayrs::Event ev_batch[2];
        std::vector<rayrs::Event> ev_round;
        uint32_t timed_rounds = 0;
    };
    Pool pool;
    rayrs::DevBuf d_next_item;
    uint32_t rounds = 0;
    bool local_ok = false;
    bool last_local = false;
    bool last_exact = false;
    rayrs::LocalScene local = {};
    int local_blocks_per_cu = 1;
    rayrs::DevBuf d_local_light;
    rayrs::DevBuf d_local_items;
    rayrs::Stream multi_stream;
    rayrs::DevBuf multi_out;
    rayrs_tuning tuning = {};
    rayrs_lab_tuning lab = {};
};

namespace rayrs {
void set_last_error(const std::string& text);
int hip_fail(hipError_t e, const char* what);
int scene_settle(rayrs_scene* s);
inline uint32_t rank_tiles(uint64_t n_tiles, uint32_t rank, uint32_t ranks) {
    return n_tiles > rank ? (uint32_t)((n_tiles - rank + ranks - 1) / ranks) : 0u;
}
inline size_t frame_bytes(uint32_t w, uint32_t h, uint32_t out_format) {
    return (size_t)w * h * 3 * (out_format == RAYRS_OUT_F64 ? 8 : 4);
}
int scene_upload(rayrs_scene* s);
SceneDev make_scene_dev(const rayrs_scene* s, bool exact);
CameraDev make_camera_dev(const rayrs_camera* c);
bool camera_is_far(const rayrs_scene* s, const rayrs_camera* c);
uint32_t trav_settings(const rayrs_scene* s, bool exact, uint32_t np, RenderDev& rp);
constexpr size_t POOL_SLOT_BYTES = sizeof(PathSlot) + 4 * sizeof(double) + 1u;
WfDev pool_wf(const DevBuf& block, uint32_t np, const DevBuf& ctl, uint32_t trav_blocks, const DevBuf& spill);
int render_enqueue(rayrs_scene* scene, const rayrs_camera* camera, const rayrs_render_params* params, uint32_t sample0,
                   const FilmPassDev* film, void* out_device, void* hip_stream);
}

#define HIP_TRY(expr)                                       \
    do {                                                    \
        hipError_t _e = (expr);                             \
        if (_e != hipSuccess) return rayrs::hip_fail(_e, #expr); \
    } while (0)

#define RAYRS_TRY(expr)                \
    do {                               \
        const int _s = (expr);         \
        if (_s != RAYRS_OK) return _s; \
    } while (0)

#define RAYRS_GUARDED(...)                                   \
    try {                                                    \
        __VA_ARGS__                                          \
    } catch (const std::bad_alloc&) {                        \
        rayrs::set_last_error("out of host memory");         \
        return RAYRS_OOM;                                    \
    } catch (const std::exception& e) {                      \
        rayrs::set_last_error(e.what());                     \
        return RAYRS_INVALID_ARG;                            \
    } catch (...) {                                          \
        rayrs::set_last_error("unknown exception");          \
        return RAYRS_INVALID_ARG;                            \
    }
```

### rayrs_amd/csrc/selftest.cpp

```cpp
#include <cstring>
#include <vector>

#include "kernels.h"
#include "rayrs_selftest.h"
#include "scene_internal.hpp"

using namespace rayrs;

static hipError_t alloc(DevBuf& b, size_t bytes) { return b.reserve(bytes ? bytes : 8); }

extern "C" {

int rayrs_test_math(int device, int fn, const double* x, const double* y, uint64_t n, double* out) {
    if (!x || !out) return RAYRS_INVALID_ARG;
    HIP_TRY(hipSetDevice(device));
    DevBuf dx, dy, dout;
    HIP_TRY(dx.upload(x, n * 8));
    if (y) HIP_TRY(dy.upload(y, n * 8));
    HIP_TRY(alloc(dout, n * 8));
    if (n) HIP_TRY(launch_test_math(fn, dx.as<const double>(), y ? dy.as<const double>() : nullptr, n, dout.as<double>(), nullptr));
    HIP_TRY(hipDeviceSynchronize());
    HIP_TRY(dout.download(out, n * 8));
    return RAYRS_OK;
}

int rayrs_test_rng(int device, uint64_t seed, const uint64_t* pixel, const uint64_t* sample, const uint32_t* draw,
                   uint64_t n, uint64_t* out_bits) {
    if (!pixel || !sample || !draw || !out_bits) return RAYRS_INVALID_ARG;
    HIP_TRY(hipSetDevice(device));
    DevBuf dp, ds, dd, dout;
    HIP_TRY(dp.upload(pixel, n * 8));
    HIP_TRY(ds.upload(sample, n * 8));
    HIP_TRY(dd.upload(draw, n * 4));
    HIP_TRY(alloc(dout, n * 8));
    if (n)
        HIP_TRY(launch_test_rng(seed, dp.as<const uint64_t>(), ds.as<const uint64_t>(), dd.as<const uint32_t>(), n,
                                dout.as<uint64_t>(), nullptr));
    HIP_TRY(hipDeviceSynchronize());
    HIP_TRY(dout.download(out_bits, n * 8));
    return RAYRS_OK;
}

int rayrs_test_intersect(rayrs_scene* scene, const double* o, const double* d, uint64_t n, int exact, double* t,
                         int64_t* object) {
    if (!scene || !o || !d || !t || !object) return RAYRS_INVALID_ARG;
    if (scene->device < 0) return RAYRS_NO_DEVICE;
    HIP_TRY(hipSetDevice(scene->device));
    DevBuf dorg, ddir, dt, dprim;
    HIP_TRY(dorg.upload(o, n * 24));
    HIP_TRY(ddir.upload(d, n * 24));
    HIP_TRY(alloc(dt, n * 8));
    HIP_TRY(alloc(dprim, n * 8));
    const SceneDev sc = make_scene_dev(scene, exact != 0);
    DevBuf dspill;
    const uint64_t threads = (n + 255) / 256 * 256;
    if (sc.stack_depth > sc.stack_lds) HIP_TRY(alloc(dspill, (size_t)(sc.stack_depth - sc.stack_lds) * threads * 4));
    if (n)
        HIP_TRY(launch_test_intersect(scene->flat.compact, sc, dorg.as<const double>(), ddir.as<const double>(), n,
                                      dt.as<double>(), dprim.as<long long>(), dspill.as<uint32_t>(), nullptr));
    HIP_TRY(hipDeviceSynchronize());
    HIP_TRY(dt.download(t, n * 8));
    HIP_TRY(dprim.download(object, n * 8));
    for (uint64_t i = 0; i < n; i++)
        if (object[i] >= 0) object[i] = (int64_t)scene->flat.prim_object[(size_t)object[i]];
    return RAYRS_OK;
}

int rayrs_test_trace(rayrs_scene* scene, const double* o, const double* d, uint64_t n, int exact, double* t, int64_t* object,
                     uint64_t* pre_answered) {
    if (!scene || !o || !d || !t || !object) return RAYRS_INVALID_ARG;
    if (scene->device < 0) return RAYRS_NO_DEVICE;
    HIP_TRY(hipSetDevice(scene->device));
    const bool ex = exact != 0;
    const SceneDev sc = make_scene_dev(scene, ex);
    uint64_t np64 = scene->tuning.pool_slots ? scene->tuning.pool_slots : (n < (1u << 20) ? n : (1u << 20));
    np64 = np64 < 1024u ? 1024u : (np64 + 1023u) & ~1023ull;
    const uint32_t np = (uint32_t)np64;
    RenderDev rp;
    std::memset(&rp, 0, sizeof(rp));
    const uint32_t trav_blocks = trav_settings(scene, ex, np, rp);
    DevBuf dblock, dctl, dspill, dcount, dans, dorg, ddir;
    HIP_TRY(alloc(dblock, (size_t)np * POOL_SLOT_BYTES));
    HIP_TRY(alloc(dctl, sizeof(WfCtl)));
    HIP_TRY(alloc(dspill, (size_t)(sc.stack_depth - sc.stack_lds) * trav_blocks * 256u * 4u));
    HIP_TRY(alloc(dcount, sizeof(Counters)));
    HIP_TRY(alloc(dans, sizeof(unsigned long long)));
    HIP_TRY(alloc(dorg, (size_t)np * 24));
    HIP_TRY(alloc(ddir, (size_t)np * 24));
    HIP_TRY(hipMemset(dcount.as<>(), 0, sizeof(Counters)));
    HIP_TRY(hipMemset(dans.as<>(), 0, sizeof(unsigned long long)));
    const WfDev wf = pool_wf(dblock, np, dctl, trav_blocks, dspill);
    rp.counters = dcount.as<Counters>();
    std::vector<uint8_t> state(np);
    std::vector<PathSlot> slots(np);
    constexpr uint32_t MAX_ROUNDS = 64;
    for (uint64_t base = 0; base < n; base += np) {
        const uint32_t m = (uint32_t)(n - base < np ? n - base : np);
        HIP_TRY(hipMemcpy(dorg.as<>(), o + 3 * base, (size_t)m * 24, hipMemcpyHostToDevice));
        HIP_TRY(hipMemcpy(ddir.as<>(), d + 3 * base, (size_t)m * 24, hipMemcpyHostToDevice));
        HIP_TRY(wf_launch_intake(sc, wf, dorg.as<const double>(), ddir.as<const double>(), m, dans.as<unsigned long long>(), nullptr));
        uint32_t round = 0;
        for (;; round++) {
            WfCtl ctl;
            std::memset(&ctl, 0, sizeof(ctl));
            ctl.live_slots = m;
            HIP_TRY(hipMemcpy(dctl.as<>(), &ctl, sizeof(ctl), hipMemcpyHostToDevice));
            HIP_TRY(wf_launch_trav(scene->flat.compact, false, sc, rp, wf, trav_blocks, nullptr));
            HIP_TRY(hipDeviceSynchronize());
            HIP_TRY(hipMemcpy(state.data(), wf.state, np, hipMemcpyDeviceToHost));
            bool ready = false;
            for (uint32_t i = 0; i < m; i++) ready |= (state[i] & 7u) == WF_READY;
            if (!ready) break;
            if (round + 1 >= MAX_ROUNDS) {
                set_last_error("rayrs_test_trace: slots still READY after the traversal rounds");
                return RAYRS_HIP_ERROR;
            }
        }
        HIP_TRY(dblock.download(slots.data(), (size_t)m * sizeof(PathSlot)));
        for (uint32_t i = 0; i < m; i++) {
            if (state[i] == WF_HIT) {
                if (slots[i].ray.prim >= scene->flat.prim_object.size()) {
                    set_last_error("rayrs_test_trace: a HIT slot names no primitive");
                    return RAYRS_HIP_ERROR;
                }
                t[base + i] = slots[i].ray.t;
                object[base + i] = (int64_t)scene->flat.prim_object[slots[i].ray.prim];
            } else if (state[i] == WF_MISS) {
                t[base + i] = 0.0;
                object[base + i] = -1;
            } else {
                set_last_error("rayrs_test_trace: a slot left neither HIT nor MISS");
                return RAYRS_HIP_ERROR;
            }
        }
    }
    unsigned long long answered = 0;
    HIP_TRY(dans.download(&answered, sizeof(answered)));
    if (pre_answered) *pre_answered = answered;
    return RAYRS_OK;
}

int rayrs_test_path_trace(rayrs_scene* scene, const rayrs_camera* camera, uint64_t seed, uint32_t max_bounces,
                          const uint32_t* pixel, const uint32_t* sample, uint64_t n, int exact, uint32_t cap,
                          uint32_t* n_queries, int64_t* object, double* t, double* throughput, uint32_t* draw, double* rgb) {
    if (!scene || !camera || !pixel || !sample || !n_queries || !object || !t || !throughput || !draw || !rgb || cap == 0)
        return RAYRS_INVALID_ARG;
    if (scene->device < 0) return RAYRS_NO_DEVICE;
    for (uint64_t i = 0; i < n; i++)
        if ((pixel[i] >> 16) >= camera->y_pixels || (pixel[i] & 0xffffu) >= camera->x_pixels) return RAYRS_INVALID_ARG;
    HIP_TRY(hipSetDevice(scene->device));
    DevBuf dpix, dsam, dn, dprim, dt, dthr, ddraw, drgb, dspill;
    HIP_TRY(dpix.upload(pixel, n * 4));
    HIP_TRY(dsam.upload(sample, n * 4));
    HIP_TRY(alloc(dn, n * 4));
    HIP_TRY(alloc(dprim, n * cap * 4));
    HIP_TRY(alloc(dt, n * cap * 8));
    HIP_TRY(alloc(dthr, n * cap * 24));
    HIP_TRY(alloc(ddraw, n * cap * 4));
    HIP_TRY(alloc(drgb, n * 24));
    HIP_TRY(hipMemset(dprim.as<>(), 0xff, n * cap * 4));
    HIP_TRY(hipMemset(dt.as<>(), 0, n * cap * 8));
    HIP_TRY(hipMemset(dthr.as<>(), 0, n * cap * 24));
    HIP_TRY(hipMemset(ddraw.as<>(), 0, n * cap * 4));
    const SceneDev sc = make_scene_dev(scene, exact != 0);
    const CameraDev cam = make_camera_dev(camera);
    const uint64_t threads = (n + 255) / 256 * 256;
    if (sc.stack_depth > sc.stack_lds) HIP_TRY(alloc(dspill, (size_t)(sc.stack_depth - sc.stack_lds) * threads * 4));
    if (n)
        HIP_TRY(launch_test_path_trace(scene->flat.compact, sc, cam, seed, max_bounces, dpix.as<const uint32_t>(),
                                       dsam.as<const uint32_t>(), n, cap, dn.as<uint32_t>(), dprim.as<uint32_t>(), dt.as<double>(),
                                       dthr.as<double>(), ddraw.as<uint32_t>(), drgb.as<double>(), dspill.as<uint32_t>(), nullptr));
    HIP_TRY(hipDeviceSynchronize());
    std::vector<uint32_t> prim(n * cap);
    HIP_TRY(dn.download(n_queries, n * 4));
    HIP_TRY(dprim.download(prim.data(), n * cap * 4));
    HIP_TRY(dt.download(t, n * cap * 8));
    HIP_TRY(dthr.download(throughput, n * cap * 24));
    HIP_TRY(ddraw.download(draw, n * cap * 4));
    HIP_TRY(drgb.download(rgb, n * 24));
    for (uint64_t k = 0; k < n * cap; k++)
        object[k] = prim[k] == 0xffffffffu ? -1 : (int64_t)scene->flat.prim_object[prim[k]];
    return RAYRS_OK;
}

int rayrs_test_material(int device, const rayrs_material* mat, const double* normal, const double* view,
                        const uint64_t* key, uint64_t n, int32_t* scattered, double* color, double* dir,
                        uint32_t* draws) {
    RAYRS_GUARDED({
    if (!mat || !normal || !view || !key || !scattered || !color || !dir || !draws) return RAYRS_INVALID_ARG;
    ObjectList tmp;
    const int surf = tmp.add_surface(mat, nullptr);
    if (surf < 0) return surf;
    HIP_TRY(hipSetDevice(device));
    DevBuf ds, dn, dv, dk, dsc, dc, dd, ddr;
    HIP_TRY(ds.upload(&tmp.surfaces[0], sizeof(SurfaceDev)));
    HIP_TRY(dn.upload(normal, n * 24));
    HIP_TRY(dv.upload(view, n * 24));
    HIP_TRY(dk.upload(key, n * 8));
    HIP_TRY(alloc(dsc, n * 4));
    HIP_TRY(alloc(dc, n * 24));
    HIP_TRY(alloc(dd, n * 24));
    HIP_TRY(alloc(ddr, n * 4));
    if (n)
        HIP_TRY(launch_test_material(ds.as<const SurfaceDev>(), dn.as<const double>(), dv.as<const double>(),
                                     dk.as<const uint64_t>(), n, dsc.as<int32_t>(), dc.as<double>(), dd.as<double>(),
                                     ddr.as<uint32_t>(), nullptr));
    HIP_TRY(hipDeviceSynchronize());
    HIP_TRY(dsc.download(scattered, n * 4));
    HIP_TRY(dc.download(color, n * 24));
    HIP_TRY(dd.download(dir, n * 24));
    HIP_TRY(ddr.download(draws, n * 4));
    return RAYRS_OK;
    })
}

int rayrs_test_background(rayrs_scene* scene, const double* dir, uint64_t n, double* rgb) {
    if (!scene || !dir || !rgb) return RAYRS_INVALID_ARG;
    if (scene->device < 0) return RAYRS_NO_DEVICE;
    HIP_TRY(hipSetDevice(scene->device));
    DevBuf dd, dout;
    HIP_TRY(dd.upload(dir, n * 24));
    HIP_TRY(alloc(dout, n * 24));
    const SceneDev sc = make_scene_dev(scene, false);
    if (n) HIP_TRY(launch_test_background(sc, dd.as<const double>(), n, dout.as<double>(), nullptr));
// ... 7 lines not shown
```

### rayrs_amd/csrc/wavefront.h

```cpp
#pragma once
#include <hip/hip_runtime.h>

#include <cstddef>

#include "layout.h"

namespace rayrs {


struct RaySlot {
    double o[3];
    double d[3];
    double t;
    uint32_t prim;
    uint32_t bd;
};
static_assert(sizeof(RaySlot) == 64, "RaySlot");

struct TailSlot {
    double thr[3];
    double acc[3];
    uint32_t item;
    uint32_t s_cur;
    uint32_t s_end;
    uint32_t pix;
};
static_assert(sizeof(TailSlot) == 64, "TailSlot");

struct PathSlot {
    RaySlot ray;
    TailSlot tail;
};
static_assert(sizeof(PathSlot) == 128, "PathSlot");
constexpr uint32_t SLOT_ITEM_BIT = 1u << 31;
constexpr uint32_t SLOT_LIGHT_BIT = 1u << 30;
constexpr uint32_t SLOT_SAMPLE_MASK = (1u << 30) - 1u;

constexpr uint8_t WF_IDLE = 0;
constexpr uint8_t WF_READY = 1;
constexpr uint8_t WF_HIT = 2;
constexpr uint8_t WF_MISS = 3;
constexpr uint8_t WF_DEAD = 4;

struct alignas(128) WfCtl {
    uint32_t next_window;
    uint32_t pad0[31];
    uint32_t live_slots;
    uint32_t pad1[31];
};
static_assert(offsetof(WfCtl, live_slots) == 128 && sizeof(WfCtl) == 256, "WfCtl lines");

struct WfDev {
    PathSlot* slots;
    double* light;
    uint8_t* state;
    WfCtl* ctl;
    uint32_t np;
    unsigned long long* wave_items;
    uint32_t n_flat_waves;
    uint32_t trav_threads;
    uint32_t* stack_spill;
};

uint32_t wf_window_slots();
hipError_t wf_launch_init(const WfDev& wf, uint32_t live, hipStream_t stream);
hipError_t wf_launch_gen(bool compact, const SceneDev& sc, const CameraDev& cam, const RenderDev& rp, const WfDev& wf,
                         uint32_t blocks, hipStream_t stream);
hipError_t wf_launch_trav(bool compact, bool count, const SceneDev& sc, const RenderDev& rp, const WfDev& wf,
                          uint32_t blocks, hipStream_t stream);
uint32_t wf_trav_lds_bytes(bool compact, uint32_t stack_lds, uint32_t leafq, uint32_t hot_records);
hipError_t wf_trav_occupancy(bool compact, uint32_t lds, int* blocks_per_cu);
hipError_t wf_trav_raise_lds(bool compact, uint32_t lds);
hipError_t wf_launch_hit(bool compact, bool eager_light, const SceneDev& sc, const CameraDev& cam, const RenderDev& rp, const WfDev& wf,
                         uint32_t blocks, hipStream_t stream);
hipError_t wf_launch_miss(bool compact, bool eager_light, const SceneDev& sc, const CameraDev& cam, const RenderDev& rp, const WfDev& wf,
                          uint32_t blocks, hipStream_t stream);
hipError_t wf_launch_intake(const SceneDev& sc, const WfDev& wf, const double* o, const double* d, uint32_t n,
                            unsigned long long* answered, hipStream_t stream);

}
```

### rayrs_amd/csrc/wavefront.hip

```cpp
#include <hip/hip_runtime.h>

#include <map>
#include <mutex>

#include "device_path.h"
#include "kernels.h"
#include "lab_ticks.h"
#include "launch_dispatch.h"
#include "wavefront.h"

namespace rayrs {

constexpr uint32_t SPL = 8;
constexpr uint32_t WINDOW = 64 * SPL;
constexpr uint32_t HIT_SURFACES_LDS = 32;

static_assert(SPL == 8, "StateWords/BatchFeed assume two words per lane");
struct StateWords {
    uint32_t w[SPL / 4];
};

RR_DEV StateWords load_state_words(const WfDev& wf, uint32_t win) {
    const uint32_t* src = reinterpret_cast<const uint32_t*>(wf.state + win * WINDOW) + (threadIdx.x & 63u) * (SPL / 4);
    StateWords r;
#pragma unroll
    for (uint32_t k = 0; k < SPL / 4; k++) r.w[k] = src[k];
    return r;
}

RR_DEV uint32_t compact_words(const StateWords& sw, uint8_t want, uint16_t* list) {
    const uint32_t lane = threadIdx.x & 63u;
    const unsigned long long lanemask_lt = (1ull << lane) - 1ull;
    const uint32_t* words = sw.w;
    uint32_t count = 0;
#pragma unroll
    for (int j = 0; j < (int)SPL; j++) {
        const uint32_t s = (words[j >> 2] >> ((j & 3) * 8)) & 0xffu;
        const bool m = s == (uint32_t)want;
        const unsigned long long mask = __ballot(m);
        if (m) list[count + (uint32_t)__popcll(mask & lanemask_lt)] = (uint16_t)(lane * SPL + (uint32_t)j);
        count += (uint32_t)__popcll(mask);
    }
    return count;
}

RR_DEV uint32_t compact_window(const WfDev& wf, uint32_t win, uint8_t want, uint16_t* list) {
    return compact_words(load_state_words(wf, win), want, list);
}

RR_DEV uint8_t ready_state(V3 d) {
    const uint32_t key = (d.x < 0.0 ? 1u : 0u) | (d.y < 0.0 ? 2u : 0u) | (d.z < 0.0 ? 4u : 0u);
    return (uint8_t)(WF_READY | (key << 4));
}
RR_DEV uint32_t compact_window_ready(const WfDev& wf, uint32_t win, uint16_t* list) {
    const StateWords sw = load_state_words(wf, win);
    uint32_t count = 0;
#pragma nounroll
    for (uint32_t key = 0; key < 8u; key++) count += compact_words(sw, (uint8_t)(WF_READY | (key << 4)), list + count);
    return count;
}

RR_DEV uint8_t ready_state_pre(uint32_t mask) { return (uint8_t)(WF_READY | (mask << 3)); }
RR_DEV uint32_t compact_window_ready_pre(const WfDev& wf, uint32_t win, uint16_t* list) {
    const StateWords sw = load_state_words(wf, win);
    const uint32_t lane = threadIdx.x & 63u;
    const unsigned long long lanemask_lt = (1ull << lane) - 1ull;
    uint32_t count = 0;
#pragma nounroll
    for (uint32_t key = 0; key < 4u; key++) {
#pragma unroll
        for (int j = 0; j < (int)SPL; j++) {
            const uint32_t s = (sw.w[j >> 2] >> ((j & 3) * 8)) & 0xffu;
            const uint32_t m = (s >> 3) & 15u;
            const bool hit = (s & 7u) == (uint32_t)WF_READY && (m & (0u - m)) == (1u << key);
            const unsigned long long mask = __ballot(hit);
            if (hit) list[count + (uint32_t)__popcll(mask & lanemask_lt)] = (uint16_t)((lane * SPL + (uint32_t)j) | (m << 9));
            count += (uint32_t)__popcll(mask);
        }
    }
    return count;
}

constexpr uint32_t FEED_LIST = WINDOW + 64;

struct BatchFeed {
    uint32_t next_win, n_waves, n_windows, count, k, total;
    StateWords ahead;
    uint8_t want;
    uint32_t* list;
};

RR_DEV uint32_t compact_words_abs(const StateWords& sw, uint8_t want, uint32_t base, uint32_t* list) {
    const uint32_t lane = threadIdx.x & 63u;
    const uint32_t* words = sw.w;
    uint32_t count = 0;
#pragma unroll
    for (int j = 0; j < (int)SPL; j++) {
        const uint32_t s = (words[j >> 2] >> ((j & 3) * 8)) & 0xffu;
        const bool m = s == (uint32_t)want;
        const unsigned long long mask = __ballot(m);
        if (m) list[count + lanes_below(mask)] = base + lane * SPL + (uint32_t)j;
        count += (uint32_t)__popcll(mask);
    }
    return count;
}

RR_DEV void feed_init(BatchFeed& f, const WfDev& wf, uint32_t wave, uint32_t n_waves, uint8_t want, uint32_t* list) {
    f.next_win = wave, f.n_waves = n_waves, f.n_windows = wf.np / WINDOW;
    f.count = 0, f.k = 0, f.total = 0, f.want = want, f.list = list;
    f.ahead.w[0] = f.ahead.w[1] = 0;
    if (f.next_win < f.n_windows) f.ahead = load_state_words(wf, f.next_win);
}

RR_DEV bool feed_next(BatchFeed& f, const WfDev& wf, uint32_t& slot, bool& valid) {
    const uint32_t lane = threadIdx.x & 63u;
    while (f.count - f.k < 64u && f.next_win < f.n_windows) {
        const uint32_t left = f.count - f.k;
        const uint32_t carry = lane < left ? f.list[f.k + lane] : 0u;
        if (lane < left) f.list[lane] = carry;
        const uint32_t fresh = compact_words_abs(f.ahead, f.want, f.next_win * WINDOW, f.list + left);
        f.total += fresh;
        f.count = left + fresh;
        f.k = 0;
        f.next_win += f.n_waves;
        if (f.next_win < f.n_windows) f.ahead = load_state_words(wf, f.next_win);
    }
    if (f.k >= f.count) return false;
    valid = f.k + lane < f.count;
    slot = valid ? f.list[f.k + lane] : 0u;
    f.k += 64u;
    return true;
}

RR_DEV unsigned long long wave_sum(unsigned long long v) {
#pragma unroll
    for (int off = 32; off > 0; off >>= 1) {
        const uint32_t lo = (uint32_t)__shfl_xor((int)(uint32_t)v, off);
        const uint32_t hi = (uint32_t)__shfl_xor((int)(uint32_t)(v >> 32), off);
        v += ((unsigned long long)hi << 32) | lo;
    }
    return v;
}

RR_DEV void wave_atomic_add(unsigned long long* dst, unsigned long long v) {
    const unsigned long long s = wave_sum(v);
    if ((threadIdx.x & 63u) == 0 && s) atomicAdd(dst, s);
}

constexpr uint32_t ka_up(uint32_t off, uint32_t a) { return (off + a - 1u) / a * a; }
constexpr uint32_t KA_SC = 0;
constexpr uint32_t KA_CAM = ka_up(KA_SC + (uint32_t)sizeof(SceneDev), (uint32_t)alignof(CameraDev));
constexpr uint32_t KA_RP = ka_up(KA_CAM + (uint32_t)sizeof(CameraDev), (uint32_t)alignof(RenderDev));
constexpr uint32_t KA_WF = ka_up(KA_RP + (uint32_t)sizeof(RenderDev), (uint32_t)alignof(WfDev));
template <class T, uint32_t OFF>
RR_DEV const T& karg() {
    typedef const __attribute__((address_space(4))) char* KPtr;
    KPtr p = (KPtr)__builtin_amdgcn_kernarg_segment_ptr() + OFF;
    asm volatile("" : "+s"(p));
    return *(const T*)p;
}

RR_DEV RaySlot* ray_slot(const WfDev& wf, uint32_t slot) { return &wf.slots[slot].ray; }
RR_DEV TailSlot* tail_slot(const WfDev& wf, uint32_t slot) { return &wf.slots[slot].tail; }
RR_DEV double* light_slot(const WfDev& wf, uint32_t slot) { return wf.light + (size_t)slot * 4u; }


__global__ void __launch_bounds__(256) wf_init_kernel(WfDev wf, uint32_t live) {
    const uint32_t i = blockIdx.x * blockDim.x + threadIdx.x;
    if (i == 0) {
        WfCtl* c = wf.ctl;
        c->next_window = 0;
        c->live_slots = live;
    }
    if (i < 2u * wf.n_flat_waves) wf.wave_items[i] = 0ull;
    if (i >= wf.np) return;
    wf.state[i] = i < live ? WF_IDLE : WF_DEAD;
}


struct ItemRegs {
    double acc[3];
    uint32_t item, s_end, pix;
    uint32_t word;
    RR_DEV uint32_t cursor() const { return word & SLOT_SAMPLE_MASK; }
    RR_DEV bool has_item() const { return (word >> 31) != 0u; }
    RR_DEV bool has_light() const { return ((word >> 30) & 1u) != 0u; }
};

RR_DEV ItemRegs load_item(const WfDev& wf, uint32_t slot) {
    const TailSlot* t = tail_slot(wf, slot);
    ItemRegs r;
    r.acc[0] = t->acc[0], r.acc[1] = t->acc[1], r.acc[2] = t->acc[2];
    r.word = t->s_cur;
    r.item = t->item, r.s_end = t->s_end, r.pix = t->pix;
    return r;
}

RR_DEV uint64_t sample_key(const RenderDev& rp, const CameraDev& cam, const ItemRegs& ir) {
    return rr_path_key(rp.seed, (uint64_t)(ir.pix >> 16) * cam.W + (ir.pix & 0xffffu), (uint64_t)(ir.cursor() - 1u));
}

constexpr uint32_t ITEM_RESERVE = 256;
constexpr unsigned long long ITEMS_GONE = ~0ull;

struct ItemRange {
    unsigned long long next, end;
};

RR_DEV unsigned long long wave_uniform64(unsigned long long v) {
    const uint32_t lo = __builtin_amdgcn_readfirstlane((uint32_t)v), hi = __builtin_amdgcn_readfirstlane((uint32_t)(v >> 32));
    return ((unsigned long long)hi << 32) | lo;
}
template <bool SCALAR = false>
RR_DEV ItemRange load_item_range(const WfDev& wf, uint32_t wave) {
    ItemRange r;
    r.next = wf.wave_items[2 * (size_t)wave];
    r.end = wf.wave_items[2 * (size_t)wave + 1];
    if (SCALAR) r.next = wave_uniform64(r.next), r.end = wave_uniform64(r.end);
    return r;
}
RR_DEV void store_item_range(const WfDev& wf, uint32_t wave, const ItemRange& r) {
    if ((threadIdx.x & 63u) == 0) {
        wf.wave_items[2 * (size_t)wave] = r.next;
        wf.wave_items[2 * (size_t)wave + 1] = r.end;
    }
}

RR_DEV bool refill_item_range(const RenderDev& rp, ItemRange& range) {
    unsigned long long first = ITEMS_GONE;
    if (range.end != ITEMS_GONE) {
        if ((threadIdx.x & 63u) == 0) first = atomicAdd(rp.next_item, (unsigned long long)ITEM_RESERVE);
        const uint32_t flo = __builtin_amdgcn_readfirstlane((uint32_t)first);
        const uint32_t fhi = __builtin_amdgcn_readfirstlane((uint32_t)(first >> 32));
        first = ((unsigned long long)fhi << 32) | flo;
    }
    if (first >= rp.total_items) {
        range.next = range.end = ITEMS_GONE;
        return false;
    }
    range.next = first;
    range.end = first + ITEM_RESERVE < rp.total_items ? first + ITEM_RESERVE : rp.total_items;
    return true;
}

struct SampleCount {
    unsigned long long paths;
    unsigned long long direct;
// ... 146 lines not shown
    bool enters = nr.enters;
    const V3 o = nr.o, d = nr.d;
    V3 inv = nr.inv;
    const uint32_t bd = nr.bd;
    const bool pre = karg<SceneDev, KA_SC>().hot != nullptr;
    if (__ballot(got) == 0ull) return;
    const bool primary = got && !carry;
    if (pre) {
        if (DEFER) {
            inv = mk(1.0 / d.x, 1.0 / d.y, 1.0 / d.z);
            enters = root_box_hit(karg<SceneDev, KA_SC>(), o, inv);
        }
        if (primary && !enters) sn.deferred++;
        finish_rays(got, enters, primary, slot, o, d, inv, bd, sn);
    } else if (got) {
        const WfDev& wf = karg<WfDev, KA_WF>();
        RaySlot* rs = ray_slot(wf, slot);
        rs->o[0] = o.x, rs->o[1] = o.y, rs->o[2] = o.z;
        rs->d[0] = d.x, rs->d[1] = d.y, rs->d[2] = d.z;
        rs->bd = bd;
        if (primary && !enters) {
            wf.state[slot] = WF_MISS;
            sn.deferred++;
        } else {
            wf.state[slot] = ready_state(d);
        }
    }
}

RR_DEV void store_sample_count(const SceneDev& sc, const RenderDev& rp, const WfDev& wf, const SampleCount& sn) {
    wave_atomic_add(&rp.counters->paths, sn.paths);
    const unsigned long long direct = wave_sum(sn.direct), deferred = wave_sum(sn.deferred);
    const unsigned long long pre = (unsigned long long)sn.pre_miss + sn.pre_done;
    if ((threadIdx.x & 63u) == 0 && (direct | deferred | pre)) {
        atomicAdd(&rp.counters->rays, direct + deferred + pre);
        if (direct) atomicAdd(&rp.counters->escaped_paths, direct);
        if (direct | deferred) atomicAdd(&rp.counters->direct_rays, direct + deferred);
    }
    if (rp.count_work && sc.hot != nullptr && (threadIdx.x & 63u) == 0) {
        Counters* c = rp.counters;
        const HotPtr h = hot_ptr(sc);
        const unsigned long long e = sn.hot.entered;
        atomicAdd(&c->pre_rays, pre);
        atomicAdd(&c->interior_visits, (unsigned long long)sn.pre_root);
        atomicAdd(&c->pre_root_records, (unsigned long long)sn.pre_root);
        atomicAdd(&c->hot_lane, (unsigned long long)sn.hot.owed);
        atomicAdd(&c->hot_prim_tests, e * h->count);
        atomicAdd(&c->hot_tri_divided, (unsigned long long)sn.hot.divided);
        if (h->n_tri) atomicAdd(&c->tri_tests, e * h->n_tri);
        if (h->n_sphere) atomicAdd(&c->sphere_tests, e * h->n_sphere);
        if (h->n_plane) atomicAdd(&c->plane_tests, e * h->n_plane);
    }
    const uint32_t r = (uint32_t)wave_sum(sn.retired);
    if ((threadIdx.x & 63u) == 0 && r) atomicSub(&wf.ctl->live_slots, r);
}

template <bool COMPACT>
__global__ void __launch_bounds__(256) wf_gen_kernel(SceneDev sc, CameraDev cam, RenderDev rp, WfDev wf) {
    __shared__ uint16_t lists[4][WINDOW];
    const uint32_t lane = threadIdx.x & 63u;
    uint16_t* list = lists[threadIdx.x >> 6];
    const uint32_t wave = (blockIdx.x * blockDim.x + threadIdx.x) >> 6;
    const uint32_t n_waves = (gridDim.x * blockDim.x) >> 6;
    const uint32_t n_windows = wf.np / WINDOW;
    SampleCount sn{0, 0, 0, 0, HotTally{0, 0, 0}, 0, 0, 0};
    ItemRange range = load_item_range(wf, wave);
    for (uint32_t win = wave; win < n_windows; win += n_waves) {
        const uint32_t count = compact_window(wf, win, WF_IDLE, list);
        for (uint32_t k = 0; k < count; k += 64u) {
            const bool valid = k + lane < count;
            const uint32_t slot = win * WINDOW + (valid ? (uint32_t)list[k + lane] : 0u);
            ItemRegs ir;
            ir.acc[0] = ir.acc[1] = ir.acc[2] = 0.0;
            ir.item = ir.s_end = ir.pix = ir.word = 0u;
            const NewRays nr = next_sample<COMPACT>(valid, slot, ir, false, range, sn);
            emit_rays<false>(slot, nr, sn);
        }
    }
    store_item_range(wf, wave, range);
    store_sample_count(sc, rp, wf, sn);
}



template <bool COMPACT, bool COUNT, bool EXACT, bool PRE>
__global__ void __launch_bounds__(256, 5) wf_trav_kernel(SceneDev sc, RenderDev rp, WfDev wf) {
    static_assert(EXACT || !PRE, "pre-tested rays are the default walk's");
    extern __shared__ uint32_t lds_dyn[];
    WfCtl* ctl = wf.ctl;
    if (ctl->live_slots == 0u) return;
    const uint32_t lane = threadIdx.x & 63u;
    const uint32_t wave = threadIdx.x >> 6;
    const uint32_t stack_words = (sc.stack_lds + 1u + sc.leafq) * 64u;
    const LaneStack stack{lds_dyn + (size_t)wave * stack_words + lane,
                          wf.stack_spill + ((size_t)blockIdx.x * 256u + threadIdx.x), sc.stack_lds, wf.trav_threads};
    uint16_t* list = reinterpret_cast<uint16_t*>(lds_dyn + 4u * (size_t)stack_words) + wave * WINDOW;
    uint4* hot_lds = reinterpret_cast<uint4*>(lds_dyn + 4u * (size_t)stack_words + 4u * WINDOW / 2u);
    {
        constexpr uint32_t G = COMPACT ? 8u : 16u;
        const uint4* src = reinterpret_cast<const uint4*>(sc.nodes);
        for (uint32_t i = threadIdx.x; i < sc.hot_records * G; i += 256u)
            hot_lds[(i / G) * HotNodes::stride<COMPACT>() + i % G] = src[i];
        __syncthreads();
    }
    const HotNodes hot{hot_lds, sc.hot_records};
    const unsigned long long lanemask_lt = (1ull << lane) - 1ull;
    uint32_t root_ref0 = 0, root_ref1 = 0, root_ref2 = 0, root_ref3 = 0;
    if (PRE) {
        const HotPtr h = hot_ptr(sc);
        root_ref0 = h->root_ref[0], root_ref1 = h->root_ref[1], root_ref2 = h->root_ref[2], root_ref3 = h->root_ref[3];
    }
    const uint32_t root_leaves = (root_ref0 >= REF_LEAF_BASE ? 1u : 0u) | (root_ref1 >= REF_LEAF_BASE ? 2u : 0u) |
                                 (root_ref2 >= REF_LEAF_BASE ? 4u : 0u) | (root_ref3 >= REF_LEAF_BASE ? 8u : 0u);

    const uint32_t n_windows = wf.np / WINDOW;
    const uint32_t n_waves = gridDim.x * 4u;
    const uint32_t static_windows = ctl->live_slots < wf.np / 4u ? n_windows : rp.static_windows;
    uint32_t static_next = blockIdx.x * 4u + wave;
    uint32_t list_pos = 0, list_len = 0, list_base = 0;
    bool no_more = false;

    bool active = false, pending = false;
    uint32_t slot = 0;
    V3 o = mk(0, 0, 0), d = mk(0, 0, 1);
    Trav tv;
    tv.inv = mk(0, 0, 0), tv.best_t = 0, tv.best_prim = 0xffffffffu, tv.cur = TRAV_DONE, tv.sp = 0;
    WorkCount wc{0, 0, 0, 0, 0};
    unsigned long long n_rays = 0;
    unsigned long long u_int_wave = 0, u_int_lane = 0, u_leaf_wave = 0, u_leaf_lane = 0;
    unsigned long long tk_int = 0, tk_leaf = 0, tk_refill = 0, tk_last = COUNT ? clock64() : 0ull;

    for (;;) {
        const bool at_int = EXACT ? (active && tv.cur != TRAV_DONE && defer_has_room(tv)) : (active && trav_at_interior(tv));
        const bool at_leaf = EXACT ? (active && defer_has_leaf(tv)) : (active && !trav_at_interior(tv));
        const int n_int = __popcll(__ballot(at_int));
        const int n_leaf = __popcll(__ballot(at_leaf));
        const int n_work = EXACT ? __popcll(__ballot(active)) : n_int + n_leaf;
        if ((n_work < (int)rp.refill_min && !no_more) || n_work == 0) {
            if (pending) {
                const bool hit = tv.best_prim != 0xffffffffu;
                if (hit) {
                    RaySlot* rs = ray_slot(wf, slot);
                    rs->t = tv.best_t;
                    rs->prim = tv.best_prim;
                }
                wf.state[slot] = hit ? WF_HIT : WF_MISS;
                pending = false;
            }
            if (no_more) break;
            bool need = !active;
            unsigned long long need_mask = __ballot(need);
            while (need_mask != 0ull) {
                if (list_pos >= list_len) {
                    uint32_t w = static_next;
                    if (w < static_windows) {
                        static_next += n_waves;
                    } else {
                        if (lane == 0) w = static_windows + atomicAdd(&ctl->next_window, 1u);
                        w = (uint32_t)__builtin_amdgcn_readfirstlane((int)w);
                    }
                    if (w >= n_windows) {
                        no_more = true;
                        break;
                    }
                    list_base = w * WINDOW;
                    list_len = PRE ? compact_window_ready_pre(wf, w, list) : compact_window_ready(wf, w, list);
                    list_pos = 0;
                    continue;
                }
                const uint32_t avail = list_len - list_pos;
                const uint32_t rank = (uint32_t)__popcll(need_mask & lanemask_lt);
                if (need && rank < avail) {
                    const uint32_t entry = (uint32_t)list[list_pos + rank];
                    slot = list_base + (PRE ? (entry & 511u) : entry);
                    const RaySlot* rs = ray_slot(wf, slot);
                    o = mk(rs->o[0], rs->o[1], rs->o[2]);
                    d = mk(rs->d[0], rs->d[1], rs->d[2]);
                    n_rays++;
                    if (PRE) {
                        tv.inv = mk(1.0 / d.x, 1.0 / d.y, 1.0 / d.z);
                        tv.best_t = rs->t;
                        tv.best_prim = rs->prim;
                        const uint32_t m = entry >> 9;
                        uint32_t r1 = root_ref1, r2 = root_ref2, r3 = root_ref3;
                        asm volatile("" : "+s"(r1), "+s"(r2), "+s"(r3));
                        const uint32_t mi = m & ~root_leaves, ml = m & root_leaves;
                        const int n = (int)__popc(mi);
                        const uint32_t low = mi & (0u - mi);
                        tv.cur = mi == 0u ? TRAV_DONE : (low & 1u) ? root_ref0 : (low & 2u) ? r1 : (low & 4u) ? r2 : r3;
                        tv.sp = n > 0 ? n - 1 : 0;
                        if ((mi & 2u) && low != 2u) stack.put(n - 1 - (int)__popc(mi & 1u), r1);
                        if ((mi & 4u) && low != 4u) stack.put(n - 1 - (int)__popc(mi & 3u), r2);
                        if ((mi & 8u) && low != 8u) stack.put(n - 1 - (int)__popc(mi & 7u), r3);
                        if (ml != 0u) {
                            if (ml & 1u) defer_take_ref(stack, tv, root_ref0);
                            if (ml & 2u) defer_take_ref(stack, tv, r1);
                            if (ml & 4u) defer_take_ref(stack, tv, r2);
                            if (ml & 8u) defer_take_ref(stack, tv, r3);
                        }
                        active = true;
                    } else {
                        trav_init(sc, o, d, tv);
                        if (tv.cur == TRAV_DONE) {
                            pending = true;
                        } else {
                            active = true;
                            if (EXACT && tv.cur >= REF_LEAF_BASE) {
                                const uint32_t ref = tv.cur;
                                tv.cur = TRAV_DONE;
                                defer_take_ref(stack, tv, ref);
                            }
                        }
                    }
                    need = false;
                }
                const uint32_t wanted = (uint32_t)__popcll(need_mask);
                list_pos += wanted < avail ? wanted : avail;
                need_mask = __ballot(need);
            }
            if (COUNT) {
                const unsigned long long now = clock64();
                tk_refill += now - tk_last, tk_last = now;
            }
            if (__ballot(active || pending) == 0ull && no_more) break;
            continue;
        }
        const bool leaf_phase = n_leaf >= (int)rp.leaf_min || n_int == 0 ||
                                (EXACT && __popcll(__ballot(at_leaf && !at_int)) >= (int)rp.leaf_wait);
        if (leaf_phase) {
            if (COUNT) u_leaf_wave += 1, u_leaf_lane += at_leaf ? 1 : 0;
            if (at_leaf) {
                if (EXACT) {
                    trav_leaf_step_defer<COMPACT, COUNT>(sc, o, d, stack, tv, wc);
                    if (defer_finished(tv)) active = false, pending = true;
                } else {
                    trav_leaf_step<COMPACT, COUNT>(sc, o, d, stack, tv, wc);
                    if (tv.cur == TRAV_DONE) active = false, pending = true;
                }
            }
            if (COUNT) {
                const unsigned long long now = clock64();
                tk_leaf += now - tk_last, tk_last = now;
            }
        } else {
            if (COUNT) u_int_wave += 1, u_int_lane += at_int ? 1 : 0;
            if (at_int) {
                if (EXACT) {
                    trav_interior_step_defer<COMPACT, COUNT>(sc, o, stack, hot, tv, wc);
                    if (defer_finished(tv)) active = false, pending = true;
                } else {
                    trav_interior_step<COMPACT, COUNT, false>(sc, o, stack, hot, tv, wc);
                    if (tv.cur == TRAV_DONE) active = false, pending = true;
                }
            }
            if (COUNT) {
                const unsigned long long now = clock64();
                tk_int += now - tk_last, tk_last = now;
            }
        }
    }

    Counters* c = rp.counters;
    wave_atomic_add(&c->rays, n_rays);
    if (COUNT) {
        wave_atomic_add(&c->interior_visits, wc.interior);
        wave_atomic_add(&c->tri_tests, wc.tri);
        wave_atomic_add(&c->sphere_tests, wc.sphere);
        wave_atomic_add(&c->plane_tests, wc.plane);
        wave_atomic_add(&c->step_wave, u_int_wave), wave_atomic_add(&c->step_lane, u_int_lane);
        wave_atomic_add(&c->inner_wave, u_leaf_lane), wave_atomic_add(&c->leaf_wave, u_leaf_wave);
        if (lane == 0) {
            atomicAdd(&c->interior_ticks, tk_int), atomicAdd(&c->leaf_ticks, tk_leaf);
            atomicAdd(&c->refill_ticks, tk_refill);
        }
    }
}


struct HitIn {
    uint32_t slot;
    bool valid;
    V3 o, d, thr, light;
    double t;
    uint32_t prim, bd;
    ItemRegs ir;
};

RR_DEV V3 load_light(const WfDev& wf, uint32_t slot) {
    const double* l = light_slot(wf, slot);
    return mk(l[0], l[1], l[2]);
}
RR_DEV bool light_is_plus_zero(V3 light) {
    return (rr_f64_bits(light.x) | rr_f64_bits(light.y) | rr_f64_bits(light.z)) == 0ull;
}

template <bool EAGER>
RR_DEV void load_hit_in(const WfDev& wf, HitIn& h) {
    const RaySlot* rs = ray_slot(wf, h.slot);
    h.o = mk(rs->o[0], rs->o[1], rs->o[2]);
    h.d = mk(rs->d[0], rs->d[1], rs->d[2]);
    h.t = rs->t;
    h.prim = rs->prim;
    h.bd = rs->bd;
    const TailSlot* t = tail_slot(wf, h.slot);
    h.thr = mk(t->thr[0], t->thr[1], t->thr[2]);
    h.light = EAGER ? load_light(wf, h.slot) : mk(0.0, 0.0, 0.0);
    h.ir = load_item(wf, h.slot);
}

template <bool COMPACT, bool EAGER>
__global__ void __launch_bounds__(256, 3) wf_hit_kernel(SceneDev sc, CameraDev cam, RenderDev rp, WfDev wf) {
    __shared__ uint32_t lists[4][FEED_LIST];
    __shared__ SurfaceDev s_surf[HIT_SURFACES_LDS];
    if (wf.ctl->live_slots == 0u) return;
    const uint32_t n_surf_lds = sc.n_surfaces < HIT_SURFACES_LDS ? sc.n_surfaces : HIT_SURFACES_LDS;
    for (uint32_t i = threadIdx.x; i < n_surf_lds * (uint32_t)(sizeof(SurfaceDev) / 4); i += 256u)
        reinterpret_cast<uint32_t*>(s_surf)[i] = reinterpret_cast<const uint32_t*>(sc.surfaces)[i];
    __syncthreads();
    uint32_t* list = lists[threadIdx.x >> 6];
    const uint32_t wave = (blockIdx.x * blockDim.x + threadIdx.x) >> 6;
    const uint32_t n_waves = (gridDim.x * blockDim.x) >> 6;
    SampleCount sn{0, 0, 0, 0, HotTally{0, 0, 0}, 0, 0, 0};
    if (blockIdx.x == 0 && threadIdx.x == 0) wf.ctl->next_window = 0;
    ItemRange range = load_item_range<true>(wf, wave);
    BatchFeed feed;
    feed_init(feed, wf, wave, n_waves, WF_HIT, list);
    HitIn cur;
    bool have = feed_next(feed, wf, cur.slot, cur.valid);
    PrimRec<COMPACT> rec_cur;
    if (have) {
        load_hit_in<EAGER>(wf, cur);
        rec_cur = load_prim<COMPACT>(sc.prims, cur.valid ? cur.prim : 0u);
    }
    RR_TICKS_BEGIN(7);
    while (have) {
        HitIn nxt;
        bool have_next = false;
        PrimRec<COMPACT> rec_nxt;
        {
            const uint32_t slot = cur.slot;
            const bool valid = cur.valid;
            bool ended = false, goes_on = false, acc_changed = false;
            uint32_t hit_sid = 8u;
            ItemRegs ir = cur.ir;
            V3 thr = mk(1.0, 1.0, 1.0), light = mk(0.0, 0.0, 0.0), position = mk(0.0, 0.0, 0.0), dir = mk(0.0, 0.0, 1.0);
            uint32_t bd_next = 0;
            if (valid) {
                RR_TICK_LOADS_ARRIVED(6)
                const SceneDev& sc = karg<SceneDev, KA_SC>();
                const RenderDev& rp = karg<RenderDev, KA_RP>();
                const WfDev& wf = karg<WfDev, KA_WF>();
                const V3 o = cur.o;
                const V3 d = cur.d;
                const double t = cur.t;
                const uint32_t bounce = cur.bd & 0xffffu;
                thr = bounce > 1u ? cur.thr : mk(1.0, 1.0, 1.0);
                light = mk(0.0, 0.0, 0.0);
                if (bounce > 1u && ir.has_light()) light = EAGER ? cur.light : load_light(wf, slot);
// ... 126 lines not shown
        ItemRegs ir = cur.ir;
        if (cur.valid) {
            const bool first = (cur.bd & 0xffffu) <= 1u;
            const V3 thr = first ? mk(1.0, 1.0, 1.0) : cur.thr;
            V3 light = mk(0.0, 0.0, 0.0);
            if (!first && ir.has_light()) light = EAGER ? cur.light : load_light(karg<WfDev, KA_WF>(), cur.slot);
            const V3 result = v_add(light, v_mul(thr, background(karg<SceneDev, KA_SC>(), cur.d)));
            ir.acc[0] += result.x;
            ir.acc[1] += result.y;
            ir.acc[2] += result.z;
        }
        RR_TICK(1)
        const NewRays nr = next_sample<COMPACT>(cur.valid, cur.slot, ir, true, range, sn);
        emit_rays<false>(cur.slot, nr, sn);
        RR_TICK(2)
        cur = nxt;
        have = have_next;
        RR_TICKS_BATCH();
    }
    RR_TICKS_END_MISS(rp)
    n_escaped = feed.total;
    store_item_range(wf, wave, range);
    if (lane == 0 && n_escaped) atomicAdd(&rp.counters->escaped_paths, n_escaped);
    store_sample_count(sc, rp, wf, sn);
}


__global__ void __launch_bounds__(256) wf_intake_kernel(SceneDev sc, CameraDev cam, RenderDev rp, WfDev wf, const double* o,
                                                        const double* d, uint32_t n, unsigned long long* answered) {
    const uint32_t slot = blockIdx.x * blockDim.x + threadIdx.x;
    const bool got = slot < n;
    const V3 ro = got ? mk(o[3 * slot], o[3 * slot + 1], o[3 * slot + 2]) : mk(0.0, 0.0, 0.0);
    const V3 rd = got ? mk(d[3 * slot], d[3 * slot + 1], d[3 * slot + 2]) : mk(0.0, 0.0, 1.0);
    const V3 inv = mk(1.0 / rd.x, 1.0 / rd.y, 1.0 / rd.z);
    const bool enters = got && root_box_hit(sc, ro, inv);
    if (sc.hot != nullptr) {
        SampleCount sn{0, 0, 0, 0, HotTally{0, 0, 0}, 0, 0, 0};
        finish_rays(got, enters, false, slot, ro, rd, inv, 1u, sn);
        if ((threadIdx.x & 63u) == 0 && sn.pre_done) atomicAdd(answered, (unsigned long long)sn.pre_done);
    } else if (got) {
        RaySlot* rs = ray_slot(wf, slot);
        rs->o[0] = ro.x, rs->o[1] = ro.y, rs->o[2] = ro.z;
        rs->d[0] = rd.x, rs->d[1] = rd.y, rs->d[2] = rd.z;
        rs->bd = 1u;
        wf.state[slot] = enters ? ready_state(rd) : WF_MISS;
    }
    if (!got && slot < wf.np) wf.state[slot] = WF_DEAD;
}


hipError_t wf_launch_intake(const SceneDev& sc, const WfDev& wf, const double* o, const double* d, uint32_t n,
                            unsigned long long* answered, hipStream_t stream) {
    const CameraDev cam{};
    const RenderDev rp{};
    hipLaunchKernelGGL(wf_intake_kernel, dim3(wf.np / 256u), dim3(256), 0, stream, sc, cam, rp, wf, o, d, n, answered);
    return hipGetLastError();
}

template <class F> struct ka_leading : std::false_type {};
template <class... Tail> struct ka_leading<void(SceneDev, CameraDev, RenderDev, WfDev, Tail...)> : std::true_type {};
static_assert(ka_leading<decltype(wf_gen_kernel<true>)>::value && ka_leading<decltype(wf_hit_kernel<true, true>)>::value &&
                  ka_leading<decltype(wf_miss_kernel<true, true>)>::value && ka_leading<decltype(wf_intake_kernel)>::value,
              "a kernel that calls karg() takes (SceneDev, CameraDev, RenderDev, WfDev) first");

uint32_t wf_trav_lds_bytes(bool compact, uint32_t stack_lds, uint32_t leafq, uint32_t hot_records) {
    return 4u * 64u * (stack_lds + 1u + leafq) * 4u + 4u * WINDOW * 2u + hot_records * (compact ? 144u : 272u);
}

uint32_t wf_window_slots() { return WINDOW; }

hipError_t wf_launch_init(const WfDev& wf, uint32_t live, hipStream_t stream) {
    hipLaunchKernelGGL(wf_init_kernel, dim3((wf.np + 255u) / 256u), dim3(256), 0, stream, wf, live);
    return hipGetLastError();
}

hipError_t wf_launch_gen(bool compact, const SceneDev& sc, const CameraDev& cam, const RenderDev& rp, const WfDev& wf,
                         uint32_t blocks, hipStream_t stream) {
    with_bools([&](auto C) {
        hipLaunchKernelGGL(wf_gen_kernel<C()>, dim3(blocks), dim3(256), 0, stream, sc, cam, rp, wf);
    }, compact);
    return hipGetLastError();
}

hipError_t wf_launch_trav(bool compact, bool count, const SceneDev& sc, const RenderDev& rp, const WfDev& wf,
                          uint32_t blocks, hipStream_t stream) {
    const uint32_t lds = wf_trav_lds_bytes(compact, sc.stack_lds, sc.leafq, sc.hot_records);
    with_bools([&](auto C, auto N, auto X, auto P) {
        hipLaunchKernelGGL((wf_trav_kernel<C(), N(), X(), X() && P()>), dim3(blocks), dim3(256), lds, stream, sc, rp, wf);
    }, compact, count, sc.exact != 0u, sc.hot != nullptr);
    return hipGetLastError();
}

hipError_t wf_trav_occupancy(bool compact, uint32_t lds, int* blocks_per_cu) {
    return with_bools([&](auto C) {
        return hipOccupancyMaxActiveBlocksPerMultiprocessor(blocks_per_cu, wf_trav_kernel<C(), false, false, false>, 256, lds);
    }, compact);
}

hipError_t wf_trav_raise_lds(bool compact, uint32_t lds) {
    static std::mutex mutex;
    static std::map<std::pair<int, bool>, uint32_t> raised;
    int device = 0;
    hipError_t e = hipGetDevice(&device);
    if (e != hipSuccess) return e;
    std::lock_guard<std::mutex> lock(mutex);
    uint32_t& set = raised[{device, compact}];
    if (lds <= set) return hipSuccess;
    e = with_bools([&](auto C) {
        const void* const instances[] = {
            reinterpret_cast<const void*>(&wf_trav_kernel<C(), false, false, false>), reinterpret_cast<const void*>(&wf_trav_kernel<C(), true, false, false>),
            reinterpret_cast<const void*>(&wf_trav_kernel<C(), false, true, false>), reinterpret_cast<const void*>(&wf_trav_kernel<C(), true, true, false>),
            reinterpret_cast<const void*>(&wf_trav_kernel<C(), false, true, true>), reinterpret_cast<const void*>(&wf_trav_kernel<C(), true, true, true>)};
        for (const void* k : instances) {
            const hipError_t ek = hipFuncSetAttribute(k, hipFuncAttributeMaxDynamicSharedMemorySize, (int)lds);
            if (ek != hipSuccess) return ek;
        }
        return hipSuccess;
    }, compact);
    if (e == hipSuccess) set = lds;
    return e;
}

hipError_t wf_launch_hit(bool compact, bool eager_light, const SceneDev& sc, const CameraDev& cam, const RenderDev& rp,
                         const WfDev& wf, uint32_t blocks, hipStream_t stream) {
    with_bools([&](auto C, auto E) {
        hipLaunchKernelGGL((wf_hit_kernel<C(), E()>), dim3(blocks), dim3(256), 0, stream, sc, cam, rp, wf);
    }, compact, eager_light);
    return hipGetLastError();
}

hipError_t wf_launch_miss(bool compact, bool eager_light, const SceneDev& sc, const CameraDev& cam, const RenderDev& rp,
                          const WfDev& wf, uint32_t blocks, hipStream_t stream) {
    with_bools([&](auto C, auto E) {
        hipLaunchKernelGGL((wf_miss_kernel<C(), E()>), dim3(blocks), dim3(256), 0, stream, sc, cam, rp, wf);
    }, compact, eager_light);
    return hipGetLastError();
}

}
```

Baseline: 5720.

## Pack BVH leaf triangle groups into deduplicated 128-byte cache lines

Builds a new per-leaf record layout where each group of up to four triangles is stored with shared vertices deduplicated into one or two 128-byte lines, with corner indices packed into spare words. A renumbered copy of the node tree and hot root points at these line records, and the traversal kernel gets a template variant whose leaf step reads the packed records. It targets the number of memory lines touched per leaf visit in exact compact traversal. The cost is extra device memory for the duplicated node tree and line buffers, plus another kernel instantiation.

```diff
diff --git a/rayrs_amd/_ffi.py b/rayrs_amd/_ffi.py
--- a/rayrs_amd/_ffi.py
+++ b/rayrs_amd/_ffi.py
@@ -26,7 +26,7 @@
 
 
 PRIVATE_SYMBOLS = ["rayrs_test_math", "rayrs_test_rng", "rayrs_test_intersect", "rayrs_test_trace", "rayrs_test_path_trace", "rayrs_test_material", "rayrs_test_background",
-                   "rayrs_lab_set", "rayrs_lab_round_ms", "rayrs_lab_multi_rehearse"]
+                   "rayrs_test_group_lines", "rayrs_lab_set", "rayrs_lab_group_lines", "rayrs_lab_round_ms", "rayrs_lab_multi_rehearse"]
 
 
 class MaterialDesc(C.Structure):
@@ -106,7 +106,8 @@
     _fields_ = [("refill_min", C.c_uint32), ("leaf_min", C.c_uint32), ("static_pct", C.c_uint32),
                 ("stack_lds", C.c_uint32), ("hot_records", C.c_uint32), ("trav_blocks_per_cu", C.c_uint32),
                 ("eager_light", C.c_uint32), ("local_reserve", C.c_uint32), ("local_segment_items", C.c_uint32),
-                ("force_rccl", C.c_uint32), ("gate_tree", C.c_uint32), ("hot_group", C.c_uint32), ("leaf_wait", C.c_uint32), ("flat_blocks_per_cu", C.c_uint32)]
+                ("force_rccl", C.c_uint32), ("gate_tree", C.c_uint32), ("hot_group", C.c_uint32), ("leaf_wait", C.c_uint32), ("flat_blocks_per_cu", C.c_uint32),
+                ("no_group_lines", C.c_uint32)]
 
 
 ABI_VERSION = 7
@@ -162,6 +163,11 @@
     L.rayrs_scene_set_tuning.argtypes = [vp, C.POINTER(Tuning)]
     L.rayrs_lab_set.argtypes = [vp, C.POINTER(LabTuning)]
     L.rayrs_lab_set.restype = C.c_int
+    if hasattr(L, "rayrs_lab_group_lines"):
+        L.rayrs_lab_group_lines.argtypes = [vp]
+        L.rayrs_lab_group_lines.restype = C.c_int
+        L.rayrs_test_group_lines.argtypes = [vp, C.POINTER(C.c_uint64), vp, vp, vp, vp]
+        L.rayrs_test_group_lines.restype = C.c_int
     L.rayrs_lab_multi_rehearse.argtypes = [vp, C.c_uint32, C.c_uint32, C.c_int, C.c_char_p, C.c_uint32]
     L.rayrs_lab_multi_rehearse.restype = C.c_int
     L.rayrs_frame_sample_chunk.argtypes = [C.c_uint32] * 4
diff --git a/rayrs_amd/api.py b/rayrs_amd/api.py
--- a/rayrs_amd/api.py
+++ b/rayrs_amd/api.py
@@ -297,7 +297,21 @@
         d = {n: getattr(i, n) for n, _ in i._fields_ if n not in ("root_box", "hot_box")}
         d["root_box"] = list(i.root_box)
         d["hot_box"] = list(i.hot_box)
+        route = self._L.rayrs_lab_group_lines(self._h) if hasattr(self._L, "rayrs_lab_group_lines") else 0
+        if route < 0:
+            _ffi.check(route, "rayrs_lab_group_lines")
+        d["group_lines"] = int(route)
         return d
+
+    def export_group_lines(self):
+        sizes = (C.c_uint64 * 8)()
+        _ffi.check(self._L.rayrs_test_group_lines(self._h, sizes, None, None, None, None), "rayrs_test_group_lines")
+        bufs = [np.zeros(max(int(sizes[k]) // 4, 1), dtype=np.uint32) for k in range(4)]
+        _ffi.check(self._L.rayrs_test_group_lines(self._h, sizes, *[b.ctypes.data for b in bufs]), "rayrs_test_group_lines")
+        lines, line_nodes, nodes, prims = [b[:int(sizes[k]) // 4] for k, b in enumerate(bufs)]
+        return {"lines": lines.reshape(-1, 32), "line_nodes": line_nodes.reshape(-1, 32), "nodes": nodes.reshape(-1, 32),
+                "prims": prims.reshape(-1, 12), "root_ref": int(sizes[4]), "hot": bool(sizes[5]), "groups": int(sizes[6]),
+                "two_line_groups": int(sizes[7])}
 
     def export_bvh(self):
         i = self.info()
diff --git a/rayrs_amd/csrc/abi.cpp b/rayrs_amd/csrc/abi.cpp
--- a/rayrs_amd/csrc/abi.cpp
+++ b/rayrs_amd/csrc/abi.cpp
@@ -209,8 +209,9 @@
         else if (s->lab.hot_records) hot = s->lab.hot_records < WIDE_FRONT ? s->lab.hot_records : WIDE_FRONT;
         w.hot_records = hot < t.n() ? hot : t.n();
         const uint32_t lds = wf_trav_lds_bytes(f.compact, w.stack_lds, w.leafq, w.hot_records);
-        HIP_TRY(wf_trav_raise_lds(f.compact, lds));
-        HIP_TRY(wf_trav_occupancy(f.compact, lds, &w.blocks_per_cu));
+        const bool lines = s->lines_route(true) && x == s->walk_index(true);
+        HIP_TRY(wf_trav_raise_lds(f.compact, lines, lds));
+        HIP_TRY(wf_trav_occupancy(f.compact, lines, lds, &w.blocks_per_cu));
         if (w.blocks_per_cu < 1) w.blocks_per_cu = 1;
     }
     return RAYRS_OK;
@@ -265,12 +266,24 @@
     }
     if (f.has_hot) HIP_TRY(s->d_hot.upload(&f.hot, sizeof(HotGroupDev)));
     HIP_TRY(s->d_prims.upload(f.prim_bytes.data(), f.prim_bytes.size()));
+    uint64_t lines_bytes = 0;
+    if (f.has_lines) {
+        HIP_TRY(s->d_lines.upload(f.line_bytes.data(), f.line_bytes.size()));
+        HIP_TRY(s->d_line_nodes.upload(f.line_node_bytes.data(), f.line_node_bytes.size()));
+        lines_bytes = f.line_bytes.size() + f.line_node_bytes.size();
+        if (f.has_hot) {
+            HotGroupDev hot = f.hot;
+            for (int ch = 0; ch < 4; ch++) hot.root_ref[ch] = f.line_hot_root_ref[ch];
+            HIP_TRY(s->d_hot_lines.upload(&hot, sizeof(HotGroupDev)));
+            lines_bytes += sizeof(HotGroupDev);
+        }
+    }
     HIP_TRY(s->d_surfaces.upload(s->surfaces.data(), s->surfaces.size() * sizeof(SurfaceDev)));
     HIP_TRY(s->d_hdri.upload(f.hdri_quads.data(), f.hdri_quads.size() * sizeof(float)));
     HIP_TRY(s->d_counters.reserve(sizeof(Counters)));
     for (auto& e : s->ev) HIP_TRY(e.create());
     s->device_bytes = f.walk.node_bytes.size() + f.gate.node_bytes.size() + (f.has_hot ? f.gate_hot.node_bytes.size() : 0) + f.prim_bytes.size() + s->surfaces.size() * sizeof(SurfaceDev) +
-                      f.hdri_quads.size() * sizeof(float);
+                      f.hdri_quads.size() * sizeof(float) + lines_bytes;
     RAYRS_TRY(scene_configure_traversal(s));
     HIP_TRY(s->pool.d_ctl.reserve(sizeof(WfCtl)));
     HIP_TRY(s->pool.h_live.alloc(2 * sizeof(uint32_t)));
@@ -449,6 +462,7 @@
     if (!scene || !lab) return RAYRS_INVALID_ARG;
     if (lab->stack_lds > 64u) return RAYRS_INVALID_ARG;
     if (lab->hot_group != 0u && lab->hot_group != 0xffffffffu) return RAYRS_INVALID_ARG;
+    if (lab->no_group_lines > 1u) return RAYRS_INVALID_ARG;
     if (lab->static_pct > 100u || lab->refill_min > 64u || lab->leaf_min > 64u || lab->leaf_wait > 64u || lab->flat_blocks_per_cu > 64u || lab->eager_light > 1u || lab->force_rccl > 1u || lab->gate_tree > 1u)
         return RAYRS_INVALID_ARG;
     if (lab->local_reserve != 0u && (lab->local_reserve < 8u || lab->local_reserve > 4096u)) return RAYRS_INVALID_ARG;
@@ -457,6 +471,11 @@
     scene->lab = *lab;
     if (scene->device >= 0) return scene_configure_traversal(scene);
     return RAYRS_OK;
+}
+
+extern "C" int rayrs_lab_group_lines(const rayrs_scene* scene) {
+    if (!scene) return RAYRS_INVALID_ARG;
+    return scene->lines_route(true) ? 1 : 0;
 }
 
 uint32_t rayrs_frame_sample_chunk(uint32_t x_pixels, uint32_t y_pixels, uint32_t spp, uint32_t requested) {
@@ -578,6 +597,20 @@
     return sc;
 }
 
+extern "C++" int rayrs::launch_trav(const rayrs_scene* s, bool exact, bool count, const SceneDev& sc, const RenderDev& rp,
+                                    const WfDev& wf, uint32_t blocks, hipStream_t stream) {
+    const bool lines = s->lines_route(exact);
+    SceneDev tsc = sc;
+    if (lines) {
+        tsc.nodes = s->d_line_nodes.as<>();
+        tsc.prims = s->d_lines.as<>();
+        tsc.root_ref = s->flat.line_root_ref;
+        if (sc.hot != nullptr) tsc.hot = s->d_hot_lines.as<HotGroupDev>();
+    }
+    HIP_TRY(wf_launch_trav(s->flat.compact, count, lines, tsc, rp, wf, blocks, stream));
+    return RAYRS_OK;
+}
+
 constexpr double RAYRS_FAR_DIAGONALS = 8.0;
 constexpr double RAYRS_FAR_PRIMITIVES = 4096.0;
 extern "C++" bool rayrs::camera_is_far(const rayrs_scene* s, const rayrs_camera* c) {
@@ -780,7 +813,7 @@
         for (uint32_t k = 0; k < batch; k++, it++) {
             const bool timed = it < MAX_TIMED;
             if (timed) RAYRS_TRY(round_event(pl, it, 0, stream));
-            HIP_TRY(wf_launch_trav(scene->flat.compact, rp.count_work != 0u, p.sc, rp, wf, p.trav_blocks, stream));
+            RAYRS_TRY(launch_trav(scene, p.exact, rp.count_work != 0u, p.sc, rp, wf, p.trav_blocks, stream));
             if (timed) RAYRS_TRY(round_event(pl, it, 1, stream));
             HIP_TRY(wf_launch_hit(scene->flat.compact, p.eager_light, p.sc, p.cam, rp, wf, p.flat_blocks, stream));
             if (timed) RAYRS_TRY(round_event(pl, it, 2, stream));
diff --git a/rayrs_amd/csrc/group_lines.h b/rayrs_amd/csrc/group_lines.h
--- /dev/null
+++ b/rayrs_amd/csrc/group_lines.h
@@ -0,0 +1,76 @@
+#pragma once
+#include <stdint.h>
+#include <string.h>
+
+namespace rayrs {
+
+constexpr uint32_t GL_LINE_BYTES = 128;
+constexpr uint32_t GL_GRANULES = GL_LINE_BYTES / 16;
+constexpr uint32_t GL_ONE_LINE_VERTS = GL_GRANULES;
+constexpr uint32_t GL_MAX_VERTS = 12;
+
+inline uint32_t group_line_encode(uint32_t first_prim, uint32_t count, const uint32_t (*tri)[9], uint8_t* out) {
+    uint32_t words[2 * GL_LINE_BYTES / 4];
+    memset(words, 0, sizeof(words));
+    uint32_t n_verts = 3;
+    for (uint32_t c = 0; c < 3; c++)
+        for (uint32_t a = 0; a < 3; a++) words[4 * c + a] = tri[0][3 * c + a];
+    uint32_t corners[2] = {0, 0};
+    for (uint32_t k = 1; k < count; k++)
+        for (uint32_t c = 0; c < 3; c++) {
+            const uint32_t* p = &tri[k][3 * c];
+            uint32_t v = 0;
+            while (v < n_verts && memcmp(&words[4 * v], p, 12) != 0) v++;
+            if (v == n_verts) {
+                memcpy(&words[4 * v], p, 12);
+                n_verts++;
+            }
+            if (k < 3) corners[0] |= v << (12 * (k - 1) + 4 * c);
+            else corners[1] |= v << (4 * c);
+        }
+    words[3] = first_prim, words[7] = corners[0], words[11] = corners[1], words[15] = n_verts | (count << 8);
+    memcpy(out, words, sizeof(words));
+    return n_verts > GL_ONE_LINE_VERTS ? 2u : 1u;
+}
+
+}
+
+#if defined(__HIPCC__) && defined(RR_DEV)
+namespace rayrs {
+
+RR_DEV void group_line_triangle(uint4 a, uint4 b, uint4 c, uint32_t p, V3 o, V3 d, double tmin, double tmax, Trav& tv) {
+    const V3 p1 = mk(f32bits_to_f64(a.x), f32bits_to_f64(a.y), f32bits_to_f64(a.z));
+    const V3 p2 = mk(f32bits_to_f64(b.x), f32bits_to_f64(b.y), f32bits_to_f64(b.z));
+    const V3 p3 = mk(f32bits_to_f64(c.x), f32bits_to_f64(c.y), f32bits_to_f64(c.z));
+    double t;
+    if (triangle_intersect(p1, p2, p3, o, d, t) && t > tmin && t < tmax) {
+        if (t < tv.best_t || (t == tv.best_t && p < tv.best_prim)) {
+            tv.best_t = t;
+            tv.best_prim = p;
+        }
+    }
+}
+
+template <bool COMPACT, bool COUNT>
+RR_DEV void trav_leaf_step_lines(const SceneDev& sc, V3 o, V3 d, const LaneStack& stack, Trav& tv, WorkCount& wc) {
+    static_assert(COMPACT, "group lines hold f32 vertices");
+    const double tmin = sc.t0, tmax = sc.t1;
+    tv.sp -= (int)LEAFQ_ONE;
+    const uint32_t ref = defer_queue(stack)[((uint32_t)tv.sp >> 16) * 64u];
+    const uint32_t count = (ref & 3u) + 1u;
+    const uint4* rec = reinterpret_cast<const uint4*>(sc.prims) + (size_t)((ref & 0x3fffffffu) >> 2) * GL_GRANULES;
+    if (COUNT) wc.leaf_prims = count, wc.tri += count;
+    const uint4 a = rec[0], b = rec[1], c = rec[2];
+    const uint32_t first = a.w;
+    group_line_triangle(a, b, c, first, o, d, tmin, tmax, tv);
+    uint32_t corners = b.w;
+    for (uint32_t k = 1; k < count; k++) {
+        if (k == 3u) corners = c.w;
+        const uint4 va = rec[corners & 15u], vb = rec[(corners >> 4) & 15u], vc = rec[(corners >> 8) & 15u];
+        corners >>= 12;
+        group_line_triangle(va, vb, vc, first + k, o, d, tmin, tmax, tv);
+    }
+}
+
+}
+#endif
diff --git a/rayrs_amd/csrc/rayrs_lab.h b/rayrs_amd/csrc/rayrs_lab.h
--- a/rayrs_amd/csrc/rayrs_lab.h
+++ b/rayrs_amd/csrc/rayrs_lab.h
@@ -24,9 +24,12 @@
     uint32_t hot_group;
     uint32_t leaf_wait;
     uint32_t flat_blocks_per_cu;
+    uint32_t no_group_lines;
 } rayrs_lab_tuning;
 
 int rayrs_lab_set(rayrs_scene* scene, const rayrs_lab_tuning* lab);
+
+int rayrs_lab_group_lines(const rayrs_scene* scene);
 
 int rayrs_lab_round_ms(rayrs_scene* scene, float* out, uint32_t cap_rounds);
 
diff --git a/rayrs_amd/csrc/rayrs_selftest.h b/rayrs_amd/csrc/rayrs_selftest.h
--- a/rayrs_amd/csrc/rayrs_selftest.h
+++ b/rayrs_amd/csrc/rayrs_selftest.h
@@ -24,6 +24,9 @@
                         uint32_t* draws);
 int rayrs_test_background(rayrs_scene* scene, const double* dir, uint64_t n, double* rgb);
 
+int rayrs_test_group_lines(const rayrs_scene* scene, uint64_t sizes[8], uint8_t* lines, uint8_t* line_nodes, uint8_t* nodes,
+                           uint8_t* prims);
+
 #ifdef __cplusplus
 }
 #endif
diff --git a/rayrs_amd/csrc/scene_host.cpp b/rayrs_amd/csrc/scene_host.cpp
--- a/rayrs_amd/csrc/scene_host.cpp
+++ b/rayrs_amd/csrc/scene_host.cpp
@@ -9,6 +9,7 @@
 #include <limits>
 
 #include "../../include/rayrs_numeric.h"
+#include "group_lines.h"
 
 namespace rayrs {
 
@@ -611,6 +612,51 @@
     build_tree_over(singles, f.walk);
 }
 
+void build_group_lines(FlatScene& f) {
+    f.has_lines = false;
+    f.line_bytes.clear(), f.line_node_bytes.clear();
+    f.n_line_groups = f.n_two_line_groups = 0;
+    if (!f.compact) return;
+    const WalkTree& t = f.lines_tree();
+    const uint32_t* prims = reinterpret_cast<const uint32_t*>(f.prim_bytes.data());
+    std::vector<uint32_t> groups;
+    if (t.n() == 0) {
+        if ((t.root_ref >> 30) != REF_RANGE) return;
+        groups.push_back(t.root_ref & 0x3fffffffu);
+    }
+    for (uint32_t ref : t.ref)
+        if ((ref >> 30) == REF_RANGE) groups.push_back(ref & 0x3fffffffu);
+    std::sort(groups.begin(), groups.end());
+    for (uint32_t g : groups)
+        for (uint32_t k = 0; k <= (g & 3u); k++) {
+            const uint32_t p = (g >> 2) + k;
+            if (p >= f.n_prims() || (prims[(size_t)p * PRIM_DWORDS_COMPACT + PRIM_DWORDS_COMPACT - 1] & 3u) != PRIM_TRIANGLE) return;
+        }
+    std::vector<uint32_t> line_of(f.n_prims(), 0u);
+    uint8_t rec[2 * GL_LINE_BYTES];
+    for (uint32_t g : groups) {
+        const uint32_t first = g >> 2, count = (g & 3u) + 1u;
+        uint32_t tri[4][9];
+        for (uint32_t k = 0; k < count; k++) std::memcpy(tri[k], prims + (size_t)(first + k) * PRIM_DWORDS_COMPACT, 36);
+        const uint32_t lines = group_line_encode(first, count, tri, rec);
+        line_of[first] = (uint32_t)(f.line_bytes.size() / GL_LINE_BYTES);
+        f.line_bytes.insert(f.line_bytes.end(), rec, rec + (size_t)lines * GL_LINE_BYTES);
+        f.n_line_groups++;
+        if (lines == 2u) f.n_two_line_groups++;
+    }
+    auto renumber = [&](uint32_t ref) {
+        if ((ref >> 30) != REF_RANGE) return ref;
+        return (REF_RANGE << 30) | (line_of[(ref & 0x3fffffffu) >> 2] << 2) | (ref & 3u);
+    };
+    f.line_node_bytes = t.node_bytes;
+    Node4F32* nodes = reinterpret_cast<Node4F32*>(f.line_node_bytes.data());
+    for (uint32_t r = 0; r < t.n(); r++)
+        for (int ch = 0; ch < 4; ch++) nodes[r].ref[ch] = renumber(nodes[r].ref[ch]);
+    f.line_root_ref = renumber(t.root_ref);
+    for (int ch = 0; ch < 4; ch++) f.line_hot_root_ref[ch] = f.has_hot ? renumber(f.hot.root_ref[ch]) : 0u;
+    f.has_lines = true;
+}
+
 inline bool boxes_f32_exact(const WalkTree& t) {
     for (size_t r = 0; r < t.ref.size(); r++) {
         if ((t.ref[r] >> 30) == REF_NONE) continue;
@@ -760,6 +806,8 @@
         }
     }
 
+    build_group_lines(f);
+
     f.hdri_w = hdri_w;
     f.hdri_h = hdri_h;
     {
diff --git a/rayrs_amd/csrc/scene_host.hpp b/rayrs_amd/csrc/scene_host.hpp
--- a/rayrs_amd/csrc/scene_host.hpp
+++ b/rayrs_amd/csrc/scene_host.hpp
@@ -59,6 +59,13 @@
     HotGroupDev hot = {};
     double root_box[6] = {0, 0, 0, 0, 0, 0};
     bool compact = false;
+    bool has_lines = false;
+    std::vector<uint8_t> line_bytes;
+    std::vector<uint8_t> line_node_bytes;
+    uint32_t line_root_ref = 0;
+    uint32_t line_hot_root_ref[4] = {0, 0, 0, 0};
+    uint32_t n_line_groups = 0, n_two_line_groups = 0;
+    const WalkTree& lines_tree() const { return has_hot ? gate_hot : gate; }
     std::vector<uint8_t> prim_bytes;
     std::vector<float> hdri_quads;
     uint32_t hdri_w = 0, hdri_h = 0;
diff --git a/rayrs_amd/csrc/scene_internal.hpp b/rayrs_amd/csrc/scene_internal.hpp
--- a/rayrs_amd/csrc/scene_internal.hpp
+++ b/rayrs_amd/csrc/scene_internal.hpp
@@ -39,9 +39,13 @@
     Walk trav[3];
     const rayrs::WalkTree& tree(int which) const { return which == 2 ? flat.gate_hot : which == 1 ? flat.gate : flat.walk; }
     rayrs::DevBuf d_hot;
+    rayrs::DevBuf d_lines, d_line_nodes, d_hot_lines;
     int walk_index(bool exact) const {
         if (!exact) return lab.gate_tree ? 1 : 0;
         return (flat.has_hot && lab.hot_group != 0xffffffffu) ? 2 : 1;
+    }
+    bool lines_route(bool exact) const {
+        return exact && flat.has_lines && lab.no_group_lines == 0u && walk_index(true) == (flat.has_hot ? 2 : 1);
     }
     uint64_t device_bytes = 0;
     struct Pool {
@@ -85,6 +89,8 @@
 CameraDev make_camera_dev(const rayrs_camera* c);
 bool camera_is_far(const rayrs_scene* s, const rayrs_camera* c);
 uint32_t trav_settings(const rayrs_scene* s, bool exact, uint32_t np, RenderDev& rp);
+int launch_trav(const rayrs_scene* s, bool exact, bool count, const SceneDev& sc, const RenderDev& rp, const WfDev& wf,
+                uint32_t blocks, hipStream_t stream);
 constexpr size_t POOL_SLOT_BYTES = sizeof(PathSlot) + 4 * sizeof(double) + 1u;
 WfDev pool_wf(const DevBuf& block, uint32_t np, const DevBuf& ctl, uint32_t trav_blocks, const DevBuf& spill);
 int render_enqueue(rayrs_scene* scene, const rayrs_camera* camera, const rayrs_render_params* params, uint32_t sample0,
diff --git a/rayrs_amd/csrc/selftest.cpp b/rayrs_amd/csrc/selftest.cpp
--- a/rayrs_amd/csrc/selftest.cpp
+++ b/rayrs_amd/csrc/selftest.cpp
@@ -105,7 +105,7 @@
             std::memset(&ctl, 0, sizeof(ctl));
             ctl.live_slots = m;
             HIP_TRY(hipMemcpy(dctl.as<>(), &ctl, sizeof(ctl), hipMemcpyHostToDevice));
-            HIP_TRY(wf_launch_trav(scene->flat.compact, false, sc, rp, wf, trav_blocks, nullptr));
+            RAYRS_TRY(launch_trav(scene, ex, false, sc, rp, wf, trav_blocks, nullptr));
             HIP_TRY(hipDeviceSynchronize());
             HIP_TRY(hipMemcpy(state.data(), wf.state, np, hipMemcpyDeviceToHost));
             bool ready = false;
@@ -140,6 +140,22 @@
     return RAYRS_OK;
 }
 
+int rayrs_test_group_lines(const rayrs_scene* scene, uint64_t sizes[8], uint8_t* lines, uint8_t* line_nodes, uint8_t* nodes,
+                           uint8_t* prims) {
+    if (!scene || !sizes) return RAYRS_INVALID_ARG;
+    const FlatScene& f = scene->flat;
+    if (!f.has_lines) return RAYRS_UNSUPPORTED;
+    const WalkTree& t = f.lines_tree();
+    sizes[0] = f.line_bytes.size(), sizes[1] = f.line_node_bytes.size(), sizes[2] = t.node_bytes.size();
+    sizes[3] = f.prim_bytes.size(), sizes[4] = f.line_root_ref, sizes[5] = f.has_hot ? 1u : 0u;
+    sizes[6] = f.n_line_groups, sizes[7] = f.n_two_line_groups;
+    if (lines) std::memcpy(lines, f.line_bytes.data(), f.line_bytes.size());
+    if (line_nodes) std::memcpy(line_nodes, f.line_node_bytes.data(), f.line_node_bytes.size());
+    if (nodes) std::memcpy(nodes, t.node_bytes.data(), t.node_bytes.size());
+    if (prims) std::memcpy(prims, f.prim_bytes.data(), f.prim_bytes.size());
+    return RAYRS_OK;
+}
+
 int rayrs_test_path_trace(rayrs_scene* scene, const rayrs_camera* camera, uint64_t seed, uint32_t max_bounces,
                           const uint32_t* pixel, const uint32_t* sample, uint64_t n, int exact, uint32_t cap,
                           uint32_t* n_queries, int64_t* object, double* t, double* throughput, uint32_t* draw, double* rgb) {
diff --git a/rayrs_amd/csrc/wavefront.h b/rayrs_amd/csrc/wavefront.h
--- a/rayrs_amd/csrc/wavefront.h
+++ b/rayrs_amd/csrc/wavefront.h
@@ -66,11 +66,15 @@
 hipError_t wf_launch_init(const WfDev& wf, uint32_t live, hipStream_t stream);
 hipError_t wf_launch_gen(bool compact, const SceneDev& sc, const CameraDev& cam, const RenderDev& rp, const WfDev& wf,
                          uint32_t blocks, hipStream_t stream);
-hipError_t wf_launch_trav(bool compact, bool count, const SceneDev& sc, const RenderDev& rp, const WfDev& wf,
+hipError_t wf_launch_trav(bool compact, bool count, bool lines, const SceneDev& sc, const RenderDev& rp, const WfDev& wf,
                           uint32_t blocks, hipStream_t stream);
 uint32_t wf_trav_lds_bytes(bool compact, uint32_t stack_lds, uint32_t leafq, uint32_t hot_records);
-hipError_t wf_trav_occupancy(bool compact, uint32_t lds, int* blocks_per_cu);
-hipError_t wf_trav_raise_lds(bool compact, uint32_t lds);
+hipError_t wf_trav_occupancy(bool compact, bool lines, uint32_t lds, int* blocks_per_cu);
+hipError_t wf_trav_raise_lds(bool compact, bool lines, uint32_t lds);
+hipError_t wf_lines_launch_trav(bool count, const SceneDev& sc, const RenderDev& rp, const WfDev& wf, uint32_t blocks,
+                                uint32_t lds, hipStream_t stream);
+hipError_t wf_lines_occupancy(uint32_t lds, int* blocks_per_cu);
+hipError_t wf_lines_raise_lds(uint32_t lds);
 hipError_t wf_launch_hit(bool compact, bool eager_light, const SceneDev& sc, const CameraDev& cam, const RenderDev& rp, const WfDev& wf,
                          uint32_t blocks, hipStream_t stream);
 hipError_t wf_launch_miss(bool compact, bool eager_light, const SceneDev& sc, const CameraDev& cam, const RenderDev& rp, const WfDev& wf,
diff --git a/rayrs_amd/csrc/wavefront.hip b/rayrs_amd/csrc/wavefront.hip
--- a/rayrs_amd/csrc/wavefront.hip
+++ b/rayrs_amd/csrc/wavefront.hip
@@ -8,78 +8,11 @@
 #include "lab_ticks.h"
 #include "launch_dispatch.h"
 #include "wavefront.h"
+#include "wf_trav_body.h"
 
 namespace rayrs {
 
-constexpr uint32_t SPL = 8;
-constexpr uint32_t WINDOW = 64 * SPL;
 constexpr uint32_t HIT_SURFACES_LDS = 32;
-
-static_assert(SPL == 8, "StateWords/BatchFeed assume two words per lane");
-struct StateWords {
-    uint32_t w[SPL / 4];
-};
-
-RR_DEV StateWords load_state_words(const WfDev& wf, uint32_t win) {
-    const uint32_t* src = reinterpret_cast<const uint32_t*>(wf.state + win * WINDOW) + (threadIdx.x & 63u) * (SPL / 4);
-    StateWords r;
-#pragma unroll
-    for (uint32_t k = 0; k < SPL / 4; k++) r.w[k] = src[k];
-    return r;
-}
-
-RR_DEV uint32_t compact_words(const StateWords& sw, uint8_t want, uint16_t* list) {
-    const uint32_t lane = threadIdx.x & 63u;
-    const unsigned long long lanemask_lt = (1ull << lane) - 1ull;
-    const uint32_t* words = sw.w;
-    uint32_t count = 0;
-#pragma unroll
-    for (int j = 0; j < (int)SPL; j++) {
-        const uint32_t s = (words[j >> 2] >> ((j & 3) * 8)) & 0xffu;
-        const bool m = s == (uint32_t)want;
-        const unsigned long long mask = __ballot(m);
-        if (m) list[count + (uint32_t)__popcll(mask & lanemask_lt)] = (uint16_t)(lane * SPL + (uint32_t)j);
-        count += (uint32_t)__popcll(mask);
-    }
-    return count;
-}
-
-RR_DEV uint32_t compact_window(const WfDev& wf, uint32_t win, uint8_t want, uint16_t* list) {
-    return compact_words(load_state_words(wf, win), want, list);
-}
-
-RR_DEV uint8_t ready_state(V3 d) {
-    const uint32_t key = (d.x < 0.0 ? 1u : 0u) | (d.y < 0.0 ? 2u : 0u) | (d.z < 0.0 ? 4u : 0u);
-    return (uint8_t)(WF_READY | (key << 4));
-}
-RR_DEV uint32_t compact_window_ready(const WfDev& wf, uint32_t win, uint16_t* list) {
-    const StateWords sw = load_state_words(wf, win);
-    uint32_t count = 0;
-#pragma nounroll
-    for (uint32_t key = 0; key < 8u; key++) count += compact_words(sw, (uint8_t)(WF_READY | (key << 4)), list + count);
-    return count;
-}
-
-RR_DEV uint8_t ready_state_pre(uint32_t mask) { return (uint8_t)(WF_READY | (mask << 3)); }
-RR_DEV uint32_t compact_window_ready_pre(const WfDev& wf, uint32_t win, uint16_t* list) {
-    const StateWords sw = load_state_words(wf, win);
-    const uint32_t lane = threadIdx.x & 63u;
-    const unsigned long long lanemask_lt = (1ull << lane) - 1ull;
-    uint32_t count = 0;
-#pragma nounroll
-    for (uint32_t key = 0; key < 4u; key++) {
-#pragma unroll
-        for (int j = 0; j < (int)SPL; j++) {
-            const uint32_t s = (sw.w[j >> 2] >> ((j & 3) * 8)) & 0xffu;
-            const uint32_t m = (s >> 3) & 15u;
-            const bool hit = (s & 7u) == (uint32_t)WF_READY && (m & (0u - m)) == (1u << key);
-            const unsigned long long mask = __ballot(hit);
-            if (hit) list[count + (uint32_t)__popcll(mask & lanemask_lt)] = (uint16_t)((lane * SPL + (uint32_t)j) | (m << 9));
-            count += (uint32_t)__popcll(mask);
-        }
-    }
-    return count;
-}
 
 constexpr uint32_t FEED_LIST = WINDOW + 64;
 
@@ -132,21 +65,6 @@
     return true;
 }
 
-RR_DEV unsigned long long wave_sum(unsigned long long v) {
-#pragma unroll
-    for (int off = 32; off > 0; off >>= 1) {
-        const uint32_t lo = (uint32_t)__shfl_xor((int)(uint32_t)v, off);
-        const uint32_t hi = (uint32_t)__shfl_xor((int)(uint32_t)(v >> 32), off);
-        v += ((unsigned long long)hi << 32) | lo;
-    }
-    return v;
-}
-
-RR_DEV void wave_atomic_add(unsigned long long* dst, unsigned long long v) {
-    const unsigned long long s = wave_sum(v);
-    if ((threadIdx.x & 63u) == 0 && s) atomicAdd(dst, s);
-}
-
 constexpr uint32_t ka_up(uint32_t off, uint32_t a) { return (off + a - 1u) / a * a; }
 constexpr uint32_t KA_SC = 0;
 constexpr uint32_t KA_CAM = ka_up(KA_SC + (uint32_t)sizeof(SceneDev), (uint32_t)alignof(CameraDev));
@@ -159,10 +77,6 @@
     asm volatile("" : "+s"(p));
     return *(const T*)p;
 }
-
-RR_DEV RaySlot* ray_slot(const WfDev& wf, uint32_t slot) { return &wf.slots[slot].ray; }
-RR_DEV TailSlot* tail_slot(const WfDev& wf, uint32_t slot) { return &wf.slots[slot].tail; }
-RR_DEV double* light_slot(const WfDev& wf, uint32_t slot) { return wf.light + (size_t)slot * 4u; }
 
 
 __global__ void __launch_bounds__(256) wf_init_kernel(WfDev wf, uint32_t live) {
@@ -475,198 +389,11 @@
 }
 
 
-
 template <bool COMPACT, bool COUNT, bool EXACT, bool PRE>
 __global__ void __launch_bounds__(256, 5) wf_trav_kernel(SceneDev sc, RenderDev rp, WfDev wf) {
-    static_assert(EXACT || !PRE, "pre-tested rays are the default walk's");
-    extern __shared__ uint32_t lds_dyn[];
-    WfCtl* ctl = wf.ctl;
-    if (ctl->live_slots == 0u) return;
-    const uint32_t lane = threadIdx.x & 63u;
-    const uint32_t wave = threadIdx.x >> 6;
-    const uint32_t stack_words = (sc.stack_lds + 1u + sc.leafq) * 64u;
-    const LaneStack stack{lds_dyn + (size_t)wave * stack_words + lane,
-                          wf.stack_spill + ((size_t)blockIdx.x * 256u + threadIdx.x), sc.stack_lds, wf.trav_threads};
-    uint16_t* list = reinterpret_cast<uint16_t*>(lds_dyn + 4u * (size_t)stack_words) + wave * WINDOW;
-    uint4* hot_lds = reinterpret_cast<uint4*>(lds_dyn + 4u * (size_t)stack_words + 4u * WINDOW / 2u);
-    {
-        constexpr uint32_t G = COMPACT ? 8u : 16u;
-        const uint4* src = reinterpret_cast<const uint4*>(sc.nodes);
-        for (uint32_t i = threadIdx.x; i < sc.hot_records * G; i += 256u)
-            hot_lds[(i / G) * HotNodes::stride<COMPACT>() + i % G] = src[i];
-        __syncthreads();
-    }
-    const HotNodes hot{hot_lds, sc.hot_records};
-    const unsigned long long lanemask_lt = (1ull << lane) - 1ull;
-    uint32_t root_ref0 = 0, root_ref1 = 0, root_ref2 = 0, root_ref3 = 0;
-    if (PRE) {
-        const HotPtr h = hot_ptr(sc);
-        root_ref0 = h->root_ref[0], root_ref1 = h->root_ref[1], root_ref2 = h->root_ref[2], root_ref3 = h->root_ref[3];
-    }
-    const uint32_t root_leaves = (root_ref0 >= REF_LEAF_BASE ? 1u : 0u) | (root_ref1 >= REF_LEAF_BASE ? 2u : 0u) |
-                                 (root_ref2 >= REF_LEAF_BASE ? 4u : 0u) | (root_ref3 >= REF_LEAF_BASE ? 8u : 0u);
-
-    const uint32_t n_windows = wf.np / WINDOW;
-    const uint32_t n_waves = gridDim.x * 4u;
-    const uint32_t static_windows = ctl->live_slots < wf.np / 4u ? n_windows : rp.static_windows;
-    uint32_t static_next = blockIdx.x * 4u + wave;
-    uint32_t list_pos = 0, list_len = 0, list_base = 0;
-    bool no_more = false;
-
-    bool active = false, pending = false;
-    uint32_t slot = 0;
-    V3 o = mk(0, 0, 0), d = mk(0, 0, 1);
-    Trav tv;
-    tv.inv = mk(0, 0, 0), tv.best_t = 0, tv.best_prim = 0xffffffffu, tv.cur = TRAV_DONE, tv.sp = 0;
-    WorkCount wc{0, 0, 0, 0, 0};
-    unsigned long long n_rays = 0;
-    unsigned long long u_int_wave = 0, u_int_lane = 0, u_leaf_wave = 0, u_leaf_lane = 0;
-    unsigned long long tk_int = 0, tk_leaf = 0, tk_refill = 0, tk_last = COUNT ? clock64() : 0ull;
-
-    for (;;) {
-        const bool at_int = EXACT ? (active && tv.cur != TRAV_DONE && defer_has_room(tv)) : (active && trav_at_interior(tv));
-        const bool at_leaf = EXACT ? (active && defer_has_leaf(tv)) : (active && !trav_at_interior(tv));
-        const int n_int = __popcll(__ballot(at_int));
-        const int n_leaf = __popcll(__ballot(at_leaf));
-        const int n_work = EXACT ? __popcll(__ballot(active)) : n_int + n_leaf;
-        if ((n_work < (int)rp.refill_min && !no_more) || n_work == 0) {
-            if (pending) {
-                const bool hit = tv.best_prim != 0xffffffffu;
-                if (hit) {
-                    RaySlot* rs = ray_slot(wf, slot);
-                    rs->t = tv.best_t;
-                    rs->prim = tv.best_prim;
-                }
-                wf.state[slot] = hit ? WF_HIT : WF_MISS;
-                pending = false;
-            }
-            if (no_more) break;
-            bool need = !active;
-            unsigned long long need_mask = __ballot(need);
-            while (need_mask != 0ull) {
-                if (list_pos >= list_len) {
-                    uint32_t w = static_next;
-                    if (w < static_windows) {
-                        static_next += n_waves;
-                    } else {
-                        if (lane == 0) w = static_windows + atomicAdd(&ctl->next_window, 1u);
-                        w = (uint32_t)__builtin_amdgcn_readfirstlane((int)w);
-                    }
-                    if (w >= n_windows) {
-                        no_more = true;
-                        break;
-                    }
-                    list_base = w * WINDOW;
-                    list_len = PRE ? compact_window_ready_pre(wf, w, list) : compact_window_ready(wf, w, list);
-                    list_pos = 0;
-                    continue;
-                }
-                const uint32_t avail = list_len - list_pos;
-                const uint32_t rank = (uint32_t)__popcll(need_mask & lanemask_lt);
-                if (need && rank < avail) {
-                    const uint32_t entry = (uint32_t)list[list_pos + rank];
-                    slot = list_base + (PRE ? (entry & 511u) : entry);
-                    const RaySlot* rs = ray_slot(wf, slot);
-                    o = mk(rs->o[0], rs->o[1], rs->o[2]);
-                    d = mk(rs->d[0], rs->d[1], rs->d[2]);
-                    n_rays++;
-                    if (PRE) {
-                        tv.inv = mk(1.0 / d.x, 1.0 / d.y, 1.0 / d.z);
-                        tv.best_t = rs->t;
-                        tv.best_prim = rs->prim;
-                        const uint32_t m = entry >> 9;
-                        uint32_t r1 = root_ref1, r2 = root_ref2, r3 = root_ref3;
-                        asm volatile("" : "+s"(r1), "+s"(r2), "+s"(r3));
-                        const uint32_t mi = m & ~root_leaves, ml = m & root_leaves;
-                        const int n = (int)__popc(mi);
-                        const uint32_t low = mi & (0u - mi);
-                        tv.cur = mi == 0u ? TRAV_DONE : (low & 1u) ? root_ref0 : (low & 2u) ? r1 : (low & 4u) ? r2 : r3;
-                        tv.sp = n > 0 ? n - 1 : 0;
-                        if ((mi & 2u) && low != 2u) stack.put(n - 1 - (int)__popc(mi & 1u), r1);
-                        if ((mi & 4u) && low != 4u) stack.put(n - 1 - (int)__popc(mi & 3u), r2);
-                        if ((mi & 8u) && low != 8u) stack.put(n - 1 - (int)__popc(mi & 7u), r3);
-                        if (ml != 0u) {
-                            if (ml & 1u) defer_take_ref(stack, tv, root_ref0);
-                            if (ml & 2u) defer_take_ref(stack, tv, r1);
-                            if (ml & 4u) defer_take_ref(stack, tv, r2);
-                            if (ml & 8u) defer_take_ref(stack, tv, r3);
-                        }
-                        active = true;
-                    } else {
-                        trav_init(sc, o, d, tv);
-                        if (tv.cur == TRAV_DONE) {
-                            pending = true;
-                        } else {
-                            active = true;
-                            if (EXACT && tv.cur >= REF_LEAF_BASE) {
-                                const uint32_t ref = tv.cur;
-                                tv.cur = TRAV_DONE;
-                                defer_take_ref(stack, tv, ref);
-                            }
-                        }
-                    }
-                    need = false;
-                }
-                const uint32_t wanted = (uint32_t)__popcll(need_mask);
-                list_pos += wanted < avail ? wanted : avail;
-                need_mask = __ballot(need);
-            }
-            if (COUNT) {
-                const unsigned long long now = clock64();
-                tk_refill += now - tk_last, tk_last = now;
-            }
-            if (__ballot(active || pending) == 0ull && no_more) break;
-            continue;
-        }
-        const bool leaf_phase = n_leaf >= (int)rp.leaf_min || n_int == 0 ||
-                                (EXACT && __popcll(__ballot(at_leaf && !at_int)) >= (int)rp.leaf_wait);
-        if (leaf_phase) {
-            if (COUNT) u_leaf_wave += 1, u_leaf_lane += at_leaf ? 1 : 0;
-            if (at_leaf) {
-                if (EXACT) {
-                    trav_leaf_step_defer<COMPACT, COUNT>(sc, o, d, stack, tv, wc);
-                    if (defer_finished(tv)) active = false, pending = true;
-                } else {
-                    trav_leaf_step<COMPACT, COUNT>(sc, o, d, stack, tv, wc);
-                    if (tv.cur == TRAV_DONE) active = false, pending = true;
-                }
-            }
-            if (COUNT) {
-                const unsigned long long now = clock64();
-                tk_leaf += now - tk_last, tk_last = now;
-            }
-        } else {
-            if (COUNT) u_int_wave += 1, u_int_lane += at_int ? 1 : 0;
-            if (at_int) {
-                if (EXACT) {
-                    trav_interior_step_defer<COMPACT, COUNT>(sc, o, stack, hot, tv, wc);
-                    if (defer_finished(tv)) active = false, pending = true;
-                } else {
-                    trav_interior_step<COMPACT, COUNT, false>(sc, o, stack, hot, tv, wc);
-                    if (tv.cur == TRAV_DONE) active = false, pending = true;
-                }
-            }
-            if (COUNT) {
-                const unsigned long long now = clock64();
-                tk_int += now - tk_last, tk_last = now;
-            }
-        }
-    }
-
-    Counters* c = rp.counters;
-    wave_atomic_add(&c->rays, n_rays);
-    if (COUNT) {
-        wave_atomic_add(&c->interior_visits, wc.interior);
-        wave_atomic_add(&c->tri_tests, wc.tri);
-        wave_atomic_add(&c->sphere_tests, wc.sphere);
-        wave_atomic_add(&c->plane_tests, wc.plane);
-        wave_atomic_add(&c->step_wave, u_int_wave), wave_atomic_add(&c->step_lane, u_int_lane);
-        wave_atomic_add(&c->inner_wave, u_leaf_lane), wave_atomic_add(&c->leaf_wave, u_leaf_wave);
-        if (lane == 0) {
-            atomicAdd(&c->interior_ticks, tk_int), atomicAdd(&c->leaf_ticks, tk_leaf);
-            atomicAdd(&c->refill_ticks, tk_refill);
-        }
-    }
+#define WF_TRAV_LEAF_STEP trav_leaf_step_defer
+#include "wf_trav_loop.h"
+#undef WF_TRAV_LEAF_STEP
 }
 
 
@@ -959,22 +686,31 @@
     return hipGetLastError();
 }
 
-hipError_t wf_launch_trav(bool compact, bool count, const SceneDev& sc, const RenderDev& rp, const WfDev& wf,
+hipError_t wf_launch_trav(bool compact, bool count, bool lines, const SceneDev& sc, const RenderDev& rp, const WfDev& wf,
                           uint32_t blocks, hipStream_t stream) {
     const uint32_t lds = wf_trav_lds_bytes(compact, sc.stack_lds, sc.leafq, sc.hot_records);
+    if (lines) {
+        if (!compact || sc.exact == 0u) return hipErrorInvalidValue;
+        return wf_lines_launch_trav(count, sc, rp, wf, blocks, lds, stream);
+    }
     with_bools([&](auto C, auto N, auto X, auto P) {
         hipLaunchKernelGGL((wf_trav_kernel<C(), N(), X(), X() && P()>), dim3(blocks), dim3(256), lds, stream, sc, rp, wf);
     }, compact, count, sc.exact != 0u, sc.hot != nullptr);
     return hipGetLastError();
 }
 
-hipError_t wf_trav_occupancy(bool compact, uint32_t lds, int* blocks_per_cu) {
+hipError_t wf_trav_occupancy(bool compact, bool lines, uint32_t lds, int* blocks_per_cu) {
+    if (lines) return compact ? wf_lines_occupancy(lds, blocks_per_cu) : hipErrorInvalidValue;
     return with_bools([&](auto C) {
         return hipOccupancyMaxActiveBlocksPerMultiprocessor(blocks_per_cu, wf_trav_kernel<C(), false, false, false>, 256, lds);
     }, compact);
 }
 
-hipError_t wf_trav_raise_lds(bool compact, uint32_t lds) {
+hipError_t wf_trav_raise_lds(bool compact, bool lines, uint32_t lds) {
+    if (lines) {
+        const hipError_t el = compact ? wf_lines_raise_lds(lds) : hipErrorInvalidValue;
+        if (el != hipSuccess) return el;
+    }
     static std::mutex mutex;
     static std::map<std::pair<int, bool>, uint32_t> raised;
     int device = 0;
diff --git a/rayrs_amd/csrc/wavefront_lines.hip b/rayrs_amd/csrc/wavefront_lines.hip
--- /dev/null
+++ b/rayrs_amd/csrc/wavefront_lines.hip
@@ -0,0 +1,58 @@
+#include <hip/hip_runtime.h>
+
+#include <map>
+#include <mutex>
+#include <type_traits>
+
+#include "device_path.h"
+#include "group_lines.h"
+#include "launch_dispatch.h"
+#include "wavefront.h"
+#include "wf_trav_body.h"
+
+namespace rayrs {
+
+struct GroupLines {};
+
+template <bool COUNT, bool PRE, class LEAVES>
+__global__ void __launch_bounds__(256, 5) wf_trav_kernel(SceneDev sc, RenderDev rp, WfDev wf) {
+    static_assert(std::is_same<LEAVES, GroupLines>::value, "this unit's instances read group lines");
+    constexpr bool COMPACT = true, EXACT = true;
+#define WF_TRAV_LEAF_STEP trav_leaf_step_lines
+#include "wf_trav_loop.h"
+#undef WF_TRAV_LEAF_STEP
+}
+
+hipError_t wf_lines_launch_trav(bool count, const SceneDev& sc, const RenderDev& rp, const WfDev& wf, uint32_t blocks,
+                                uint32_t lds, hipStream_t stream) {
+    with_bools([&](auto N, auto P) {
+        hipLaunchKernelGGL((wf_trav_kernel<N(), P(), GroupLines>), dim3(blocks), dim3(256), lds, stream, sc, rp, wf);
+    }, count, sc.hot != nullptr);
+    return hipGetLastError();
+}
+
+hipError_t wf_lines_occupancy(uint32_t lds, int* blocks_per_cu) {
+    return hipOccupancyMaxActiveBlocksPerMultiprocessor(blocks_per_cu, wf_trav_kernel<false, false, GroupLines>, 256, lds);
+}
+
+hipError_t wf_lines_raise_lds(uint32_t lds) {
+    static std::mutex mutex;
+    static std::map<int, uint32_t> raised;
+    int device = 0;
+    hipError_t e = hipGetDevice(&device);
+    if (e != hipSuccess) return e;
+    std::lock_guard<std::mutex> lock(mutex);
+    uint32_t& set = raised[device];
+    if (lds <= set) return hipSuccess;
+    const void* const instances[] = {
+        reinterpret_cast<const void*>(&wf_trav_kernel<false, false, GroupLines>), reinterpret_cast<const void*>(&wf_trav_kernel<true, false, GroupLines>),
+        reinterpret_cast<const void*>(&wf_trav_kernel<false, true, GroupLines>), reinterpret_cast<const void*>(&wf_trav_kernel<true, true, GroupLines>)};
+    for (const void* k : instances) {
+        e = hipFuncSetAttribute(k, hipFuncAttributeMaxDynamicSharedMemorySize, (int)lds);
+        if (e != hipSuccess) return e;
+    }
+    set = lds;
+    return hipSuccess;
+}
+
+}
diff --git a/rayrs_amd/csrc/wf_trav_body.h b/rayrs_amd/csrc/wf_trav_body.h
--- /dev/null
+++ b/rayrs_amd/csrc/wf_trav_body.h
@@ -0,0 +1,97 @@
+#pragma once
+#include <hip/hip_runtime.h>
+
+#include "device_path.h"
+#include "wavefront.h"
+
+namespace rayrs {
+
+constexpr uint32_t SPL = 8;
+constexpr uint32_t WINDOW = 64 * SPL;
+
+static_assert(SPL == 8, "StateWords/BatchFeed assume two words per lane");
+struct StateWords {
+    uint32_t w[SPL / 4];
+};
+
+RR_DEV StateWords load_state_words(const WfDev& wf, uint32_t win) {
+    const uint32_t* src = reinterpret_cast<const uint32_t*>(wf.state + win * WINDOW) + (threadIdx.x & 63u) * (SPL / 4);
+    StateWords r;
+#pragma unroll
+    for (uint32_t k = 0; k < SPL / 4; k++) r.w[k] = src[k];
+    return r;
+}
+
+RR_DEV uint32_t compact_words(const StateWords& sw, uint8_t want, uint16_t* list) {
+    const uint32_t lane = threadIdx.x & 63u;
+    const unsigned long long lanemask_lt = (1ull << lane) - 1ull;
+    const uint32_t* words = sw.w;
+    uint32_t count = 0;
+#pragma unroll
+    for (int j = 0; j < (int)SPL; j++) {
+        const uint32_t s = (words[j >> 2] >> ((j & 3) * 8)) & 0xffu;
+        const bool m = s == (uint32_t)want;
+        const unsigned long long mask = __ballot(m);
+        if (m) list[count + (uint32_t)__popcll(mask & lanemask_lt)] = (uint16_t)(lane * SPL + (uint32_t)j);
+        count += (uint32_t)__popcll(mask);
+    }
+    return count;
+}
+
+RR_DEV uint32_t compact_window(const WfDev& wf, uint32_t win, uint8_t want, uint16_t* list) {
+    return compact_words(load_state_words(wf, win), want, list);
+}
+
+RR_DEV uint8_t ready_state(V3 d) {
+    const uint32_t key = (d.x < 0.0 ? 1u : 0u) | (d.y < 0.0 ? 2u : 0u) | (d.z < 0.0 ? 4u : 0u);
+    return (uint8_t)(WF_READY | (key << 4));
+}
+RR_DEV uint32_t compact_window_ready(const WfDev& wf, uint32_t win, uint16_t* list) {
+    const StateWords sw = load_state_words(wf, win);
+    uint32_t count = 0;
+#pragma nounroll
+    for (uint32_t key = 0; key < 8u; key++) count += compact_words(sw, (uint8_t)(WF_READY | (key << 4)), list + count);
+    return count;
+}
+
+RR_DEV uint8_t ready_state_pre(uint32_t mask) { return (uint8_t)(WF_READY | (mask << 3)); }
+RR_DEV uint32_t compact_window_ready_pre(const WfDev& wf, uint32_t win, uint16_t* list) {
+    const StateWords sw = load_state_words(wf, win);
+    const uint32_t lane = threadIdx.x & 63u;
+    const unsigned long long lanemask_lt = (1ull << lane) - 1ull;
+    uint32_t count = 0;
+#pragma nounroll
+    for (uint32_t key = 0; key < 4u; key++) {
+#pragma unroll
+        for (int j = 0; j < (int)SPL; j++) {
+            const uint32_t s = (sw.w[j >> 2] >> ((j & 3) * 8)) & 0xffu;
+            const uint32_t m = (s >> 3) & 15u;
+            const bool hit = (s & 7u) == (uint32_t)WF_READY && (m & (0u - m)) == (1u << key);
+            const unsigned long long mask = __ballot(hit);
+            if (hit) list[count + (uint32_t)__popcll(mask & lanemask_lt)] = (uint16_t)((lane * SPL + (uint32_t)j) | (m << 9));
+            count += (uint32_t)__popcll(mask);
+        }
+    }
+    return count;
+}
+
+RR_DEV unsigned long long wave_sum(unsigned long long v) {
+#pragma unroll
+    for (int off = 32; off > 0; off >>= 1) {
+        const uint32_t lo = (uint32_t)__shfl_xor((int)(uint32_t)v, off);
+        const uint32_t hi = (uint32_t)__shfl_xor((int)(uint32_t)(v >> 32), off);
+        v += ((unsigned long long)hi << 32) | lo;
+    }
+    return v;
+}
+
+RR_DEV void wave_atomic_add(unsigned long long* dst, unsigned long long v) {
+    const unsigned long long s = wave_sum(v);
+    if ((threadIdx.x & 63u) == 0 && s) atomicAdd(dst, s);
+}
+
+RR_DEV RaySlot* ray_slot(const WfDev& wf, uint32_t slot) { return &wf.slots[slot].ray; }
+RR_DEV TailSlot* tail_slot(const WfDev& wf, uint32_t slot) { return &wf.slots[slot].tail; }
+RR_DEV double* light_slot(const WfDev& wf, uint32_t slot) { return wf.light + (size_t)slot * 4u; }
+
+}
diff --git a/rayrs_amd/csrc/wf_trav_loop.h b/rayrs_amd/csrc/wf_trav_loop.h
--- /dev/null
+++ b/rayrs_amd/csrc/wf_trav_loop.h
@@ -0,0 +1,190 @@
+
+    static_assert(EXACT || !PRE, "pre-tested rays are the default walk's");
+    extern __shared__ uint32_t lds_dyn[];
+    WfCtl* ctl = wf.ctl;
+    if (ctl->live_slots == 0u) return;
+    const uint32_t lane = threadIdx.x & 63u;
+    const uint32_t wave = threadIdx.x >> 6;
+    const uint32_t stack_words = (sc.stack_lds + 1u + sc.leafq) * 64u;
+    const LaneStack stack{lds_dyn + (size_t)wave * stack_words + lane,
+                          wf.stack_spill + ((size_t)blockIdx.x * 256u + threadIdx.x), sc.stack_lds, wf.trav_threads};
+    uint16_t* list = reinterpret_cast<uint16_t*>(lds_dyn + 4u * (size_t)stack_words) + wave * WINDOW;
+    uint4* hot_lds = reinterpret_cast<uint4*>(lds_dyn + 4u * (size_t)stack_words + 4u * WINDOW / 2u);
+    {
+        constexpr uint32_t G = COMPACT ? 8u : 16u;
+        const uint4* src = reinterpret_cast<const uint4*>(sc.nodes);
+        for (uint32_t i = threadIdx.x; i < sc.hot_records * G; i += 256u)
+            hot_lds[(i / G) * HotNodes::stride<COMPACT>() + i % G] = src[i];
+        __syncthreads();
+    }
+    const HotNodes hot{hot_lds, sc.hot_records};
+    const unsigned long long lanemask_lt = (1ull << lane) - 1ull;
+    uint32_t root_ref0 = 0, root_ref1 = 0, root_ref2 = 0, root_ref3 = 0;
+    if (PRE) {
+        const HotPtr h = hot_ptr(sc);
+        root_ref0 = h->root_ref[0], root_ref1 = h->root_ref[1], root_ref2 = h->root_ref[2], root_ref3 = h->root_ref[3];
+    }
+    const uint32_t root_leaves = (root_ref0 >= REF_LEAF_BASE ? 1u : 0u) | (root_ref1 >= REF_LEAF_BASE ? 2u : 0u) |
+                                 (root_ref2 >= REF_LEAF_BASE ? 4u : 0u) | (root_ref3 >= REF_LEAF_BASE ? 8u : 0u);
+
+    const uint32_t n_windows = wf.np / WINDOW;
+    const uint32_t n_waves = gridDim.x * 4u;
+    const uint32_t static_windows = ctl->live_slots < wf.np / 4u ? n_windows : rp.static_windows;
+    uint32_t static_next = blockIdx.x * 4u + wave;
+    uint32_t list_pos = 0, list_len = 0, list_base = 0;
+    bool no_more = false;
+
+    bool active = false, pending = false;
+    uint32_t slot = 0;
+    V3 o = mk(0, 0, 0), d = mk(0, 0, 1);
+    Trav tv;
+    tv.inv = mk(0, 0, 0), tv.best_t = 0, tv.best_prim = 0xffffffffu, tv.cur = TRAV_DONE, tv.sp = 0;
+    WorkCount wc{0, 0, 0, 0, 0};
+    unsigned long long n_rays = 0;
+    unsigned long long u_int_wave = 0, u_int_lane = 0, u_leaf_wave = 0, u_leaf_lane = 0;
+    unsigned long long tk_int = 0, tk_leaf = 0, tk_refill = 0, tk_last = COUNT ? clock64() : 0ull;
+
+    for (;;) {
+        const bool at_int = EXACT ? (active && tv.cur != TRAV_DONE && defer_has_room(tv)) : (active && trav_at_interior(tv));
+        const bool at_leaf = EXACT ? (active && defer_has_leaf(tv)) : (active && !trav_at_interior(tv));
+        const int n_int = __popcll(__ballot(at_int));
+        const int n_leaf = __popcll(__ballot(at_leaf));
+        const int n_work = EXACT ? __popcll(__ballot(active)) : n_int + n_leaf;
+        if ((n_work < (int)rp.refill_min && !no_more) || n_work == 0) {
+            if (pending) {
+                const bool hit = tv.best_prim != 0xffffffffu;
+                if (hit) {
+                    RaySlot* rs = ray_slot(wf, slot);
+                    rs->t = tv.best_t;
+                    rs->prim = tv.best_prim;
+                }
+                wf.state[slot] = hit ? WF_HIT : WF_MISS;
+                pending = false;
+            }
+            if (no_more) break;
+            bool need = !active;
+            unsigned long long need_mask = __ballot(need);
+            while (need_mask != 0ull) {
+                if (list_pos >= list_len) {
+                    uint32_t w = static_next;
+                    if (w < static_windows) {
+                        static_next += n_waves;
+                    } else {
+                        if (lane == 0) w = static_windows + atomicAdd(&ctl->next_window, 1u);
+                        w = (uint32_t)__builtin_amdgcn_readfirstlane((int)w);
+                    }
+                    if (w >= n_windows) {
+                        no_more = true;
+                        break;
+                    }
+                    list_base = w * WINDOW;
+                    list_len = PRE ? compact_window_ready_pre(wf, w, list) : compact_window_ready(wf, w, list);
+                    list_pos = 0;
+                    continue;
+                }
+                const uint32_t avail = list_len - list_pos;
+                const uint32_t rank = (uint32_t)__popcll(need_mask & lanemask_lt);
+                if (need && rank < avail) {
+                    const uint32_t entry = (uint32_t)list[list_pos + rank];
+                    slot = list_base + (PRE ? (entry & 511u) : entry);
+                    const RaySlot* rs = ray_slot(wf, slot);
+                    o = mk(rs->o[0], rs->o[1], rs->o[2]);
+                    d = mk(rs->d[0], rs->d[1], rs->d[2]);
+                    n_rays++;
+                    if (PRE) {
+                        tv.inv = mk(1.0 / d.x, 1.0 / d.y, 1.0 / d.z);
+                        tv.best_t = rs->t;
+                        tv.best_prim = rs->prim;
+                        const uint32_t m = entry >> 9;
+                        uint32_t r1 = root_ref1, r2 = root_ref2, r3 = root_ref3;
+                        asm volatile("" : "+s"(r1), "+s"(r2), "+s"(r3));
+                        const uint32_t mi = m & ~root_leaves, ml = m & root_leaves;
+                        const int n = (int)__popc(mi);
+                        const uint32_t low = mi & (0u - mi);
+                        tv.cur = mi == 0u ? TRAV_DONE : (low & 1u) ? root_ref0 : (low & 2u) ? r1 : (low & 4u) ? r2 : r3;
+                        tv.sp = n > 0 ? n - 1 : 0;
+                        if ((mi & 2u) && low != 2u) stack.put(n - 1 - (int)__popc(mi & 1u), r1);
+                        if ((mi & 4u) && low != 4u) stack.put(n - 1 - (int)__popc(mi & 3u), r2);
+                        if ((mi & 8u) && low != 8u) stack.put(n - 1 - (int)__popc(mi & 7u), r3);
+                        if (ml != 0u) {
+                            if (ml & 1u) defer_take_ref(stack, tv, root_ref0);
+                            if (ml & 2u) defer_take_ref(stack, tv, r1);
+                            if (ml & 4u) defer_take_ref(stack, tv, r2);
+                            if (ml & 8u) defer_take_ref(stack, tv, r3);
+                        }
+                        active = true;
+                    } else {
+                        trav_init(sc, o, d, tv);
+                        if (tv.cur == TRAV_DONE) {
+                            pending = true;
+                        } else {
+                            active = true;
+                            if (EXACT && tv.cur >= REF_LEAF_BASE) {
+                                const uint32_t ref = tv.cur;
+                                tv.cur = TRAV_DONE;
+                                defer_take_ref(stack, tv, ref);
+                            }
+                        }
+                    }
+                    need = false;
+                }
+                const uint32_t wanted = (uint32_t)__popcll(need_mask);
+                list_pos += wanted < avail ? wanted : avail;
+                need_mask = __ballot(need);
+            }
+            if (COUNT) {
+                const unsigned long long now = clock64();
+                tk_refill += now - tk_last, tk_last = now;
+            }
+            if (__ballot(active || pending) == 0ull && no_more) break;
+            continue;
+        }
+        const bool leaf_phase = n_leaf >= (int)rp.leaf_min || n_int == 0 ||
+                                (EXACT && __popcll(__ballot(at_leaf && !at_int)) >= (int)rp.leaf_wait);
+        if (leaf_phase) {
+            if (COUNT) u_leaf_wave += 1, u_leaf_lane += at_leaf ? 1 : 0;
+            if (at_leaf) {
+                if (EXACT) {
+                    WF_TRAV_LEAF_STEP<COMPACT, COUNT>(sc, o, d, stack, tv, wc);
+                    if (defer_finished(tv)) active = false, pending = true;
+                } else {
+                    trav_leaf_step<COMPACT, COUNT>(sc, o, d, stack, tv, wc);
+                    if (tv.cur == TRAV_DONE) active = false, pending = true;
+                }
+            }
+            if (COUNT) {
+                const unsigned long long now = clock64();
+                tk_leaf += now - tk_last, tk_last = now;
+            }
+        } else {
+            if (COUNT) u_int_wave += 1, u_int_lane += at_int ? 1 : 0;
+            if (at_int) {
+                if (EXACT) {
+                    trav_interior_step_defer<COMPACT, COUNT>(sc, o, stack, hot, tv, wc);
+                    if (defer_finished(tv)) active = false, pending = true;
+                } else {
+                    trav_interior_step<COMPACT, COUNT, false>(sc, o, stack, hot, tv, wc);
+                    if (tv.cur == TRAV_DONE) active = false, pending = true;
+                }
+            }
+            if (COUNT) {
+                const unsigned long long now = clock64();
+                tk_int += now - tk_last, tk_last = now;
+            }
+        }
+    }
+
+    Counters* c = rp.counters;
+    wave_atomic_add(&c->rays, n_rays);
+    if (COUNT) {
+        wave_atomic_add(&c->interior_visits, wc.interior);
+        wave_atomic_add(&c->tri_tests, wc.tri);
+        wave_atomic_add(&c->sphere_tests, wc.sphere);
+        wave_atomic_add(&c->plane_tests, wc.plane);
+        wave_atomic_add(&c->step_wave, u_int_wave), wave_atomic_add(&c->step_lane, u_int_lane);
+        wave_atomic_add(&c->inner_wave, u_leaf_lane), wave_atomic_add(&c->leaf_wave, u_leaf_wave);
+        if (lane == 0) {
+            atomicAdd(&c->interior_ticks, tk_int), atomicAdd(&c->leaf_ticks, tk_leaf);
+            atomicAdd(&c->refill_ticks, tk_refill);
+        }
+    }
```

Result: faster. 5781, median of 6 (+1.1%).
